# thepochynsons/MCRay-Tracing

Hardware: AMD Instinct MI355X
Metric: rays/sec (Monte-Carlo sample paths traced + accumulated into whole B-mode frames: PSF, envelope, scan conversion) (higher is better)
Workload: dtype f32; 1 GPU; 1M random triangles (8 meshes, PCG64 12345): 128x1024 rays/GPU, depth 10, 465 rows; scan_lines_total=128, triangles=1000000, parallelism=scanline-shard x1, frames_in_flight=128, last_pass_gather_and_post_exposed=False, gather=none (one GPU), slowest_repeat=0, overlap_gather_psf_with_next_trace=True, bvh_builder=sah, warmup_steps_run=3978

## Files before the change

mcray-tracing_amd/api.py:

```python
import contextlib
import ctypes as C
import math
import numpy as np

from . import _lib
from ._lib import Params, MeshRec, Stats, Bvh, Bvh4, BmodeParams, Focus, Compound, Sweep, VolumeGrid, CompoundOpts, LabelOpts, RenderView, RenderOpts, SpeckleOpts, ReconOpts, NODE_DTYPE, SEGMENT_DTYPE, check, ptr, load_library

DEFAULT_ANGLE = 1.0471975511965976


def host_build_bvh(tri, tri_mesh):
    L = load_library()
    tri = np.ascontiguousarray(tri, np.float32).reshape(-1, 9)
    tm = np.ascontiguousarray(tri_mesh, np.uint32)
    b = Bvh()
    check(L.mcrt_build_bvh(ptr(tri), ptr(tm), tri.shape[0], C.byref(b)))
    try:
        nodes = np.frombuffer(C.string_at(b.nodes, 64 * b.n_nodes), dtype=NODE_DTYPE).copy()
        btri = np.frombuffer(C.string_at(b.tri, 48 * b.n_tri), dtype=np.float32).reshape(-1, 12).copy()
        depth = int(b.max_depth)
    finally:
        L.mcrt_free_bvh(C.byref(b))
    return nodes, btri, depth


def host_build_bvh4(tri, tri_mesh):
    L = load_library()
    tri = np.ascontiguousarray(tri, np.float32).reshape(-1, 9)
    tm = np.ascontiguousarray(tri_mesh, np.uint32)
    b = Bvh(); b4 = Bvh4()
    check(L.mcrt_build_bvh(ptr(tri), ptr(tm), tri.shape[0], C.byref(b)))
    try:
        check(L.mcrt_build_bvh4(C.byref(b), C.byref(b4)))
        nodes = np.frombuffer(C.string_at(b.nodes, 64 * b.n_nodes), dtype=NODE_DTYPE).copy()
        btri = np.frombuffer(C.string_at(b.tri, 48 * b.n_tri), dtype=np.float32).reshape(-1, 12).copy()
        n4 = np.frombuffer(C.string_at(b4.nodes, 128 * b4.n_nodes), dtype=np.uint8).reshape(-1, 128).copy()
        ms = int(b4.max_stack)
    finally:
        L.mcrt_free_bvh(C.byref(b)); L.mcrt_free_bvh4(C.byref(b4))
    return nodes, btri, n4, ms


def host_row_thresholds(row_dt_us, n_rows):
    thr = np.zeros(n_rows + 1, np.float64)
    check(load_library().mcrt_row_thresholds(row_dt_us, n_rows, ptr(thr)))
    return thr


def host_texture(n=256):
    out = np.empty((n, n, n, 2), np.float32)
    check(load_library().mcrt_generate_texture(ptr(out), n))
    return out


def host_psf(freq=4.5, var_x=0.05, var_y=0.2, res_um=145, n_ax=7, n_lat=13):
    ax = np.zeros(n_ax, np.float32); lat = np.zeros(n_lat, np.float32)
    check(load_library().mcrt_psf_kernels(freq, var_x, var_y, res_um, ptr(ax), n_ax, ptr(lat), n_lat))
    return ax, lat


def focus_struct(focus_mm=(), focal_range_mm=20.0):
    f = Focus()
    fm = [float(x) for x in (focus_mm or ())]
    f.n_focus = len(fm)
    for i, x in enumerate(fm[:8]):
        f.focus_mm[i] = x
    f.focal_range_mm = focal_range_mm
    return f


def host_psf_focus(var_y, res_um, n_rows, row_mm, focus_mm, focal_range_mm=20.0, n_lat=13):
    out = np.zeros((n_rows, n_lat), np.float32)
    f = focus_struct(focus_mm, focal_range_mm)
    check(load_library().mcrt_psf_focus_kernels(var_y, res_um, C.byref(f), n_rows, row_mm, ptr(out), n_lat))
    return out


def row_pitch_mm(frequency):
    res_f = np.float32(np.float32(1.45) / np.float32(frequency))
    return int(np.float32(res_f * np.float32(1000.0))) / 1000.0


def _element_tables(fn, n_elements, radius_cm, sep_mm, position, angles_deg, *how):
    pos = np.zeros((n_elements, 3), np.float32); d = np.zeros((n_elements, 3), np.float32)
    p = np.asarray(position, np.float32); a = np.asarray(angles_deg, np.float32)
    check(getattr(load_library(), fn)(n_elements, radius_cm, sep_mm, ptr(p), ptr(a), *how, ptr(pos), ptr(d)))
    return pos, d


def host_transducer(n_elements, radius_cm, sep_mm, position, angles_deg):
    return _element_tables("mcrt_transducer_elements", n_elements, radius_cm, sep_mm, position, angles_deg)


def host_elevation_axis(angles_deg):
    a = np.asarray(angles_deg, np.float32); out = np.zeros(3, np.float32)
    check(load_library().mcrt_transducer_elevation_axis(ptr(a), ptr(out)))
    return out


def host_elevation_planes(pos, dirs, axis, n_planes, pitch_um):
    pos = np.ascontiguousarray(pos, np.float32).reshape(-1, 3); dirs = np.ascontiguousarray(dirs, np.float32).reshape(-1, 3)
    axis = np.ascontiguousarray(axis, np.float32)
    E, K = pos.shape[0], max(int(n_planes), 0)
    po = np.zeros((K, E, 3), np.float32); do = np.zeros((K, E, 3), np.float32); z = np.zeros(K, np.float32)
    check(load_library().mcrt_elevation_planes(ptr(pos), ptr(dirs), E, ptr(axis), n_planes, pitch_um, ptr(po), ptr(do), ptr(z)))
    return po, do, z


def host_psf_elevation(var_z, pitch_um, n_rows, row_mm, focus_mm=(), focal_range_mm=20.0, n_planes=7, normalize=True):
    out = np.zeros((n_rows, max(int(n_planes), 0)), np.float32)
    f = focus_struct(focus_mm, focal_range_mm)
    check(load_library().mcrt_psf_elevation_kernels(var_z, pitch_um, C.byref(f), n_rows, row_mm, 1 if normalize else 0, ptr(out), n_planes))
    return out


def host_scan_maps(n_elements, n_rows, radius_mm=30.0, total_angle=DEFAULT_ANGLE, max_travel_us=100, speed_of_sound=1500, out_rows=400, out_cols=500):
    return _sector_maps("mcrt_scan_maps", n_elements, n_rows, radius_mm, total_angle, max_travel_us, speed_of_sound, out_rows, out_cols)


def _sector_maps(fn, n_elements, n_rows, radius_mm, total_angle, max_travel_us, speed_of_sound, out_rows, out_cols, *steer):
    mr = np.zeros((out_rows, out_cols), np.float32); mc = np.zeros((out_rows, out_cols), np.float32)
    check(getattr(load_library(), fn)(n_elements, n_rows, radius_mm, total_angle, max_travel_us, speed_of_sound, out_rows, out_cols, *steer, ptr(mr), ptr(mc)))
    return mr, mc


def host_transducer_steered(n_elements, radius_cm, sep_mm, position, angles_deg, steer_rad):
    return _element_tables("mcrt_transducer_steered", n_elements, radius_cm, sep_mm, position, angles_deg, steer_rad)


def host_compound_maps(n_elements, n_rows, steer_rad, radius_mm=30.0, total_angle=DEFAULT_ANGLE, max_travel_us=100, speed_of_sound=1500, out_rows=400,
                       out_cols=500):
    return _sector_maps("mcrt_compound_maps", n_elements, n_rows, radius_mm, total_angle, max_travel_us, speed_of_sound, out_rows, out_cols, steer_rad)


def compound_struct(steer_rad):
    st = [float(x) for x in steer_rad]
    cp = Compound()
    cp.n_views = len(st)
    for i, x in enumerate(st[:16]):
        cp.steer_rad[i] = x
    return cp


COMPOUND_MODES = {"mean": 0, "max": 1, "median": 2}


def compound_opts_struct(mode="mean", view_weights=None, feather_lines=0.0):
    o = CompoundOpts()
    check(load_library().mcrt_default_compound_opts(C.byref(o)))
    o.mode = COMPOUND_MODES[mode] if isinstance(mode, str) else int(mode)
    o.feather_lines = float(feather_lines)
    if view_weights is not None:
        w = [float(x) for x in view_weights]
        if len(w) > 16:
            raise ValueError("at most 16 view weights, got %d" % len(w))
        for i, x in enumerate(w):
            o.view_weight[i] = x
    return o


def _compound_defaults(mode, view_weights, feather_lines):
    return mode in ("mean", 0) and view_weights is None and feather_lines == 0.0


def host_compound_weights(n_elements, n_rows, steer_rad, view_weight=1.0, feather_lines=0.0, radius_mm=30.0, total_angle=DEFAULT_ANGLE,
                          max_travel_us=100, speed_of_sound=1500, out_rows=400, out_cols=500):
    w = np.zeros((out_rows, out_cols), np.float32)
    check(load_library().mcrt_compound_weights(n_elements, n_rows, radius_mm, total_angle, max_travel_us, speed_of_sound, out_rows, out_cols, steer_rad,
                                               view_weight, feather_lines, ptr(w)))
    return w


def host_transducer_swept(n_elements, radius_cm, sep_mm, position, angles_deg, tilt_rad, pivot_mm=0.0):
    return _element_tables("mcrt_transducer_swept", n_elements, radius_cm, sep_mm, position, angles_deg, tilt_rad, pivot_mm)


def sweep_struct(n_planes, step_rad, pivot_mm=0.0):
    sw = Sweep()
    sw.n_planes, sw.step_rad, sw.pivot_mm = int(n_planes), float(step_rad), float(pivot_mm)
    return sw


def _as_sweep(sweep):
    return sweep if isinstance(sweep, Sweep) else sweep_struct(*sweep)


def sweep_tilts(n_planes, step_rad):
    step = float(np.float32(step_rad))
    return np.array([(k - (n_planes - 1) / 2.0) * step for k in range(n_planes)], np.float32)


def volume_grid(origin_mm, du, dv, dw, nu, nv, nw=1):
    g = VolumeGrid()
    for dst, src in ((g.origin_mm, origin_mm), (g.du_mm, du), (g.dv_mm, dv), (g.dw_mm, dw)):
        for i in range(3):
            dst[i] = float(src[i])
    g.nu, g.nv, g.nw, g._pad = int(nu), int(nv), int(nw), 0
    return g


def cplane_grid(depth_mm, nu, nv, pitch_mm, x0_mm=None, z0_mm=None):
    x0 = -(nu - 1) * pitch_mm / 2.0 if x0_mm is None else x0_mm
    z0 = -(nv - 1) * pitch_mm / 2.0 if z0_mm is None else z0_mm
    return volume_grid((x0, depth_mm, z0), (pitch_mm, 0, 0), (0, 0, pitch_mm), (0, 0, 0), nu, nv, 1)


def sagittal_grid(x_mm, nu, nv, pitch_mm, y0_mm, z0_mm=None):
    z0 = -(nu - 1) * pitch_mm / 2.0 if z0_mm is None else z0_mm
    return volume_grid((x_mm, y0_mm, z0), (0, 0, pitch_mm), (0, pitch_mm, 0), (0, 0, 0), nu, nv, 1)


def host_volume_maps(n_elements, n_rows, sweep, grid, radius_mm=30.0, total_angle=DEFAULT_ANGLE, max_travel_us=100, speed_of_sound=1500):
    sw = _as_sweep(sweep)
    shape = (grid.nw, grid.nv, grid.nu)
    mz = np.zeros(shape, np.float32); mr = np.zeros(shape, np.float32); mc = np.zeros(shape, np.float32)
    check(load_library().mcrt_volume_maps(n_elements, n_rows, radius_mm, total_angle, max_travel_us, speed_of_sound, C.byref(sw), C.byref(grid), ptr(mz), ptr(mr), ptr(mc)))
    return mz, mr, mc


BMODE_MODES = {"db": 0, "ref_log": 1}


RENDER_MODES = {"mip": 0, "mean": 1, "surface": 2}


def render_view(grid, direction, up=(0, 0, 1), pixel_mm=0.25, step_mm=0.25, nx=500, ny=400):
    v = RenderView()
    d = (C.c_double * 3)(*[float(x) for x in direction]); u = (C.c_double * 3)(*[float(x) for x in up])
    check(load_library().mcrt_render_view_for_grid(C.byref(grid), d, u, float(pixel_mm), float(step_mm), int(nx), int(ny), C.byref(v)))
    return v


def render_opts_struct(in_u8=False, mode=None, lo=None, hi=None, threshold=None, ramp=None, opacity=None, depth_cue=None, t_cut=None):
    o = RenderOpts()
    check(load_library().mcrt_default_render_opts(C.byref(o), 1 if in_u8 else 0))
    if mode is not None:
        o.mode = RENDER_MODES[mode] if isinstance(mode, str) else int(mode)
    for name, val in (("lo", lo), ("hi", hi), ("threshold", threshold), ("ramp", ramp), ("opacity", opacity), ("depth_cue", depth_cue), ("t_cut", t_cut)):
        if val is not None:
            setattr(o, name, float(val))
    return o


def speckle_opts_struct(n_iter=None, q0=None, rho=None, lambda_=None, **kw):
    o = SpeckleOpts()
    check(load_library().mcrt_default_speckle_opts(C.byref(o)))
    for k in ("lambda", "lam"):
        if k in kw:
            lambda_ = kw.pop(k)
    if kw:
        raise TypeError("unknown speckle options: %s" % ", ".join(sorted(kw)))
    if n_iter is not None:
        o.n_iter = int(n_iter)
    for name, val in (("q0", q0), ("rho", rho), ("lambda_", lambda_)):
        if val is not None:
            setattr(o, name, float(val))
    return o


def host_speckle_tables(opts=None, **kw):
    o = opts if opts is not None else speckle_opts_struct(**kw)
    n = min(int(o.n_iter), 256)
    q0sq = np.zeros(n, np.float32); kq = np.zeros(n, np.float32); lam4 = np.zeros(1, np.float32)
    check(load_library().mcrt_speckle_tables(C.byref(o), ptr(q0sq), ptr(kq), ptr(lam4)))
    return q0sq, kq, np.float32(lam4[0])


RECON_MODES = {"mean": 0, "max": 1}


def recon_opts_struct(mode=None, value_max=None, fill_radius=None, fill_min=None, empty=None):
    o = ReconOpts()
    check(load_library().mcrt_default_recon_opts(C.byref(o)))
    if mode is not None:
        o.mode = RECON_MODES[mode] if isinstance(mode, str) else int(mode)
    for name, val, kind in (("value_max", value_max, float), ("fill_radius", fill_radius, int), ("fill_min", fill_min, int), ("empty", empty, float)):
        if val is not None:
            setattr(o, name, kind(val))
    return o


def host_recon_transform(grid, unit_mm=10.0):
    A = np.zeros((3, 3), np.float32); b = np.zeros(3, np.float32)
    check(load_library().mcrt_recon_transform(C.byref(grid), float(unit_mm), ptr(A), ptr(b)))
    return A, b


def _depth_mm_f(depth_cm, speed_of_sound):
    travel = int((depth_cm / float(speed_of_sound)) * 10000.0)
    return float(np.float32(np.float32((travel * int(speed_of_sound)) & 0xffffffff) * np.float32(0.001)))


LABEL_RULES = {"traced": 0, "geometric": 1}
LABEL_NONE = 255
LABEL_MAX_CROSSINGS = 64
LABEL_CAPPED = 1 << 31


def label_opts_struct(rule="traced", start_offset=None):
    o = LabelOpts()
    check(load_library().mcrt_default_label_opts(C.byref(o)))
    o.rule = LABEL_RULES[rule] if isinstance(rule, str) else int(rule)
    if start_offset is not None:
        o.start_offset = float(start_offset)
    return o


def bmode_params(mode="db", dynamic_range_db=60.0, gain_db=0.0, ref=None, persistence=0.0, reset_state=True, radius_mm=30.0,
                 total_angle=DEFAULT_ANGLE, out_rows=400, out_cols=500):
    p = BmodeParams()
    check(load_library().mcrt_default_bmode(C.byref(p)))
    p.mode = BMODE_MODES[mode] if isinstance(mode, str) else int(mode)
    p.dynamic_range_db, p.gain_db, p.ref, p.persistence = dynamic_range_db, gain_db, 0.0 if ref is None else ref, persistence
    p.reset_state = 1 if reset_state else 0
    p.out_rows, p.out_cols, p.radius_mm, p.total_angle_rad = out_rows, out_cols, radius_mm, total_angle
    return p


class Transducer:

    def __init__(self, n_elements=512, frequency=4.5, radius_cm=3.0, amplitude_deg=60.0, position=(0, 0, 0), angles_deg=(0, 0, 0), separation_mm=None):
        self.n_elements = n_elements
        self.frequency = frequency
        self.radius_cm = radius_cm
        self.amplitude_rad = (amplitude_deg * math.pi * 1.0) / 180.0
        if separation_mm is None:
            separation_mm = ((float(np.float32(self.amplitude_rad)) * radius_cm) / n_elements) * 10.0
        self.separation_mm = separation_mm
        self.position = tuple(float(x) for x in position)
        self.angles = tuple(float(x) for x in angles_deg)
        self.update()

    def update(self):
        self.pos, self.dir = host_transducer(self.n_elements, self.radius_cm, self.separation_mm, self.position, self.angles)

    def element(self, i):
        return self.pos[i], self.dir[i]

    def planes(self, n_planes, pitch_um):
        return host_elevation_planes(self.pos, self.dir, host_elevation_axis(self.angles), n_planes, pitch_um)

    def steered(self, steer_rad_list):
        tabs = [host_transducer_steered(self.n_elements, self.radius_cm, self.separation_mm, self.position, self.angles, float(s)) for s in steer_rad_list]
        return np.stack([t[0] for t in tabs]), np.stack([t[1] for t in tabs])

    def swept(self, n_planes, step_rad, pivot_mm=0.0):
        tabs = [host_transducer_swept(self.n_elements, self.radius_cm, self.separation_mm, self.position, self.angles, float(t), pivot_mm)
                for t in sweep_tilts(n_planes, step_rad)]
        return np.stack([t[0] for t in tabs]), np.stack([t[1] for t in tabs])

    def poses(self, positions, angles_deg):
        positions = np.asarray(positions, np.float32).reshape(-1, 3); angles_deg = np.asarray(angles_deg, np.float32).reshape(-1, 3)
        if positions.shape != angles_deg.shape:
            raise ValueError("poses takes one position and one set of angles per frame")
        tabs = [host_transducer(self.n_elements, self.radius_cm, self.separation_mm, p, a) for p, a in zip(positions, angles_deg)]
        return np.stack([t[0] for t in tabs]), np.stack([t[1] for t in tabs])


class Psf:

    def __init__(self, freq=4.5, var_x=0.05, var_y=0.2, var_z=0.1, axial_size=7, lateral_size=13, resolution_um=145, focus_mm=None, focal_range_mm=20.0,
                 elevation_size=7, elevation_pitch_um=None, elevation_focus_mm=None, elevation_normalize=True):
        self.axial_kernel, self.lateral_kernel = host_psf(freq, var_x, var_y, resolution_um, axial_size, lateral_size)
        self.var_y, self.resolution_um = var_y, resolution_um
        self.focus_mm = tuple(float(x) for x in focus_mm) if focus_mm is not None else ()
        self.focal_range_mm = focal_range_mm
        self._rows = {}
        self.var_z, self.elevation_size = var_z, elevation_size
        self.elevation_pitch_um = resolution_um if elevation_pitch_um is None else elevation_pitch_um
        self.elevation_focus_mm = tuple(float(x) for x in elevation_focus_mm) if elevation_focus_mm is not None else ()
        self.elevation_normalize = bool(elevation_normalize)
        self.elevation_kernel = (host_psf_elevation(var_z, self.elevation_pitch_um, 1, 1.0, (), focal_range_mm, elevation_size, False)[0]
                                 if var_z > 0 and math.isfinite(var_z) else np.zeros(elevation_size, np.float32))
        self._elev_rows = {}

    def elevation_rows(self, n_rows, row_mm):
        key = (n_rows, row_mm)
        if key not in self._elev_rows:
            self._elev_rows[key] = host_psf_elevation(self.var_z, self.elevation_pitch_um, n_rows, row_mm, self.elevation_focus_mm, self.focal_range_mm,
                                                      self.elevation_size, self.elevation_normalize)
        return self._elev_rows[key]

    @property
    def has_focus(self):
        return len(self.focus_mm) > 0

    def lateral_rows(self, n_rows, row_mm):
        key = (n_rows, row_mm)
        if key not in self._rows:
            self._rows[key] = host_psf_focus(self.var_y, self.resolution_um, n_rows, row_mm, self.focus_mm, self.focal_range_mm, self.lateral_kernel.size)
        return self._rows[key]


def _scene_tables(sd):
    meshes = (MeshRec * len(sd.meshes))(*[MeshRec(a, b, c, 0) for a, b, c in sd.meshes])
    return meshes, len(sd.meshes), np.asarray(sd.spacing, np.float32)


def _tri9(tri):
    if isinstance(tri, np.ndarray):
        tri = np.ascontiguousarray(tri, np.float32).reshape(-1, 9)
        return tri, tri.shape[0]
    return tri, tri.numel() // 9


def _tgc_rows(tgc_db, n_rows):
    if tgc_db is None:
        return None
    tgc = np.ascontiguousarray(tgc_db, np.float32)
    if tgc.shape != (n_rows,):
        raise ValueError("tgc_db needs one value per RF row: %d, got shape %s" % (n_rows, tgc.shape))
    return tgc


def _pose_tables(what, pos, dirs, n_frames, n_elements):
    if isinstance(pos, np.ndarray):
        pos = np.ascontiguousarray(pos, np.float32); dirs = np.ascontiguousarray(dirs, np.float32)
    if n_frames is None:
        if not hasattr(pos, "shape"):
            raise ValueError("%s: n_frames is required with raw device pointers for pos / dirs" % what)
        n_frames = pos.shape[0]
        assert tuple(pos.shape) == (n_frames, n_elements, 3) and tuple(dirs.shape) == tuple(pos.shape)
    return pos, dirs, n_frames


class _SceneCalls:

    def _call(self, name, *args):
        check(getattr(self.L, self.PREFIX + name)(self.h, *args))

    def _assign_params(self, kw):
        for k, v in kw.items():
            if not hasattr(self.params, k):
                raise AttributeError(k)
            setattr(self.params, k, v)

    def set_bvh_builder(self, builder):
        self._call("set_bvh_builder", {"sah": 0, "lbvh": 1}[builder] if isinstance(builder, str) else int(builder))

    def upload_scene(self, sd):
        meshes, n_mesh, sp = _scene_tables(sd)
        self._call("upload_scene", ptr(sd.tri), ptr(sd.tri_mesh), sd.n_tri, C.cast(meshes, C.c_void_p), n_mesh, ptr(sd.materials), sd.materials.shape[0], sd.start_mat, ptr(sp))

    def upload_texture(self, vox=None, n=256):
        if vox is not None:
            vox = np.ascontiguousarray(vox, np.float32)
        self._call("upload_texture", ptr(vox), n)

    def set_transducer(self, pos, d):
        pos = np.ascontiguousarray(pos, np.float32); d = np.ascontiguousarray(d, np.float32)
        self._call("set_transducer", ptr(pos), ptr(d), pos.shape[0])


class Context(_SceneCalls):
    PREFIX = "mcrt_"

    def __init__(self, device=0, _borrowed=None):
        self.L = load_library()
        self.owned = _borrowed is None
        if self.owned:
            h = C.c_void_p()
            check(self.L.mcrt_create(device, C.byref(h)))
        else:
            h = C.c_void_p(_borrowed)
        self.h = h
        self.params = Params()
        check(self.L.mcrt_default_params(C.byref(self.params)))

    def close(self):
        if getattr(self, "h", None):
            if self.owned:
                self.L.mcrt_destroy(self.h)
            self.h = None

    def __del__(self):
        try:
            self.close()
        except Exception:
            pass

    def set_params(self, **kw):
        self._assign_params(kw)
        check(self.L.mcrt_set_params(self.h, C.byref(self.params)))

    def set_stream(self, stream_ptr):
        check(self.L.mcrt_set_stream(self.h, C.c_void_p(stream_ptr) if stream_ptr else None))

    def synchronize(self):
        check(self.L.mcrt_synchronize(self.h))

    def debug_fast_paths(self):
        out = (C.c_uint32 * 4)()
        check(self.L.mcrt_debug_fast_paths(self.h, out))
        return bool(out[0]), bool(out[1]), int(out[2])

    def debug_set_error(self, bits):
        check(self.L.mcrt_debug_set_error(self.h, int(bits)))

    def update_triangles(self, tri):
        tri, n = _tri9(tri)
        check(self.L.mcrt_update_triangles(self.h, ptr(tri), n))

    def refit_triangles(self, tri):
        tri, n = _tri9(tri)
        check(self.L.mcrt_refit_triangles(self.h, ptr(tri), n))

    def get_bvh(self):
        b = Bvh()
        check(self.L.mcrt_get_bvh(self.h, C.byref(b)))
        nodes = np.frombuffer(C.string_at(b.nodes, 64 * b.n_nodes), dtype=NODE_DTYPE).copy() if b.n_nodes else np.zeros(0, NODE_DTYPE)
        btri = np.frombuffer(C.string_at(b.tri, 48 * b.n_tri), dtype=np.float32).reshape(-1, 12).copy()
        return nodes, btri, int(b.max_depth)

    def get_bvh4(self):
        b = Bvh4()
        check(self.L.mcrt_get_bvh4(self.h, C.byref(b)))
        return np.frombuffer(C.string_at(b.nodes, 128 * b.n_nodes), dtype=np.uint8).reshape(-1, 128).copy(), int(b.max_stack)

    def alloc(self, nbytes):
        p = C.c_void_p()
        check(self.L.mcrt_alloc(self.h, nbytes, C.byref(p)))
        return p.value

    def free(self, dev):
        check(self.L.mcrt_free(self.h, C.c_void_p(dev)))

    @contextlib.contextmanager
    def temp(self, nbytes):
        p = self.alloc(nbytes)
        try:
            yield p
        finally:
            self.free(p)

    def d2h(self, dev, shape, dtype=np.float32):
        out = np.empty(shape, dtype)
        check(self.L.mcrt_memcpy_d2h(self.h, ptr(out), ptr(dev), out.nbytes))
        return out

    def h2d(self, dev, arr):
        arr = np.ascontiguousarray(arr)
        check(self.L.mcrt_memcpy_h2d(self.h, ptr(dev), ptr(arr), arr.nbytes))

    def trace_frame(self, frame_id, rf_dev, e_begin=0, e_end=None):
        e_end = self.params.n_elements if e_end is None else e_end
        check(self.L.mcrt_trace_frame(self.h, frame_id, e_begin, e_end, ptr(rf_dev)))

    def trace_frames(self, frame_id, n_frames, rf_dev, e_begin=0, e_end=None):
        e_end = self.params.n_elements if e_end is None else e_end
        check(self.L.mcrt_trace_frames(self.h, frame_id, n_frames, e_begin, e_end, ptr(rf_dev)))

    def trace_frames_poses(self, frame_id, pos, dirs, rf_dev, e_begin=0, e_end=None, n_frames=None):
        e_end = self.params.n_elements if e_end is None else e_end
        pos, dirs, n_frames = _pose_tables("trace_frames_poses", pos, dirs, n_frames, self.params.n_elements)
        check(self.L.mcrt_trace_frames_poses(self.h, frame_id, n_frames, e_begin, e_end, ptr(pos), ptr(dirs), ptr(rf_dev)))

    def trace_frame_debug(self, frame_id, rf_dev, e_begin=0, e_end=None, want_hits=True, want_segs=False):
        e_end = self.params.n_elements if e_end is None else e_end
        ne, S, B = e_end - e_begin, self.params.n_samples, self.params.max_depth
        hits = np.full((ne, S, B), -3, np.int32) if want_hits else None
        segs = np.zeros((ne, S, B), SEGMENT_DTYPE) if want_segs else None
        cnt = np.zeros((ne, S), np.uint32) if want_segs else None
        check(self.L.mcrt_trace_frame_debug(self.h, frame_id, e_begin, e_end, ptr(rf_dev), ptr(hits), ptr(segs), ptr(cnt)))
        return hits, segs, cnt

    def cast_rays(self, frame_id, e_begin=0, e_end=None, want_hits=True):
        e_end = self.params.n_elements if e_end is None else e_end
        ne, S, B = e_end - e_begin, self.params.n_samples, self.params.max_depth
        segs = np.zeros((ne, S, B), SEGMENT_DTYPE); cnt = np.zeros((ne, S), np.uint32)
        hits = np.full((ne, S, B), -3, np.int32) if want_hits else None
        check(self.L.mcrt_cast_rays(self.h, frame_id, e_begin, e_end, ptr(segs), ptr(cnt), ptr(hits)))
        return segs, cnt, hits

    def convolve_frames(self, rf_dev, n_frames, n_elements, n_rows, axial, lateral):
        ax = np.ascontiguousarray(axial, np.float32); lat = np.ascontiguousarray(lateral, np.float32)
        check(self.L.mcrt_convolve_frames(self.h, ptr(rf_dev), n_frames, n_elements, n_rows, ptr(ax), ax.size, ptr(lat), lat.size))

    def convolve_frames_depth(self, rf_dev, n_frames, n_elements, n_rows, axial, lat_rows):
        ax = np.ascontiguousarray(axial, np.float32); lat = np.ascontiguousarray(lat_rows, np.float32)
        if lat.ndim != 2 or lat.shape[0] != n_rows:
            raise ValueError("lat_rows needs one row of taps per RF row: (%d, n_lat), got shape %s" % (n_rows, lat.shape))
        check(self.L.mcrt_convolve_frames_depth(self.h, ptr(rf_dev), n_frames, n_elements, n_rows, ptr(ax), ax.size, ptr(lat), lat.shape[1]))

    def elevation_frames(self, planes_dev, n_frames, n_planes, n_elements, n_rows, w_rows, rf_dev):
        w = np.ascontiguousarray(w_rows, np.float32)
        if w.shape != (n_rows, n_planes):
            raise ValueError("w_rows needs one row of weights per RF row: (%d, %d), got shape %s" % (n_rows, n_planes, w.shape))
        check(self.L.mcrt_elevation_frames(self.h, ptr(planes_dev), n_frames, n_planes, n_elements, n_rows, ptr(w), ptr(rf_dev)))

    def convolve(self, rf_dev, n_elements, n_rows, axial, lateral):
        ax =np.ascontiguousarray(axial, np.float32); lat = np.ascontiguousarray(lateral, np.float32)
        check(self.L.mcrt_convolve(self.h, ptr(rf_dev), n_elements, n_rows, ptr(ax), ax.size, ptr(lat), lat.size))

    def envelope(self, rf_dev, n_elements, n_rows):
        check(self.L.mcrt_envelope(self.h, ptr(rf_dev), n_elements, n_rows))

    def envelope_frames(self, rf_dev, n_frames, n_elements, n_rows):
        check(self.L.mcrt_envelope_frames(self.h, ptr(rf_dev), n_frames, n_elements, n_rows))

    def scan_convert_frames(self, rf_dev, n_frames, n_elements, n_rows, out_dev, radius_mm=30.0, total_angle=DEFAULT_ANGLE, out_rows=400, out_cols=500):
        check(self.L.mcrt_scan_convert_frames(self.h, ptr(rf_dev), n_frames, n_elements, n_rows, radius_mm, total_angle, ptr(out_dev), out_rows, out_cols))

    def scan_convert(self, rf_dev, n_elements, n_rows, out_dev, radius_mm=30.0, total_angle=DEFAULT_ANGLE, out_rows=400, out_cols=500):
        check(self.L.mcrt_scan_convert(self.h, ptr(rf_dev), n_elements, n_rows, radius_mm, total_angle, ptr(out_dev), out_rows, out_cols))

    def bmode_frames(self, rf_dev, n_frames, n_elements, n_rows, out_dev, *, mode="db", dynamic_range_db=60.0, gain_db=0.0, ref=None, tgc_db=None,
                     persistence=0.0, state_dev=None, reset_state=True, peak_dev=None, radius_mm=30.0, total_angle=DEFAULT_ANGLE,
                     out_rows=400, out_cols=500):
        p = bmode_params(mode=mode, dynamic_range_db=dynamic_range_db, gain_db=gain_db, ref=ref, persistence=persistence, reset_state=reset_state,
                         radius_mm=radius_mm, total_angle=total_angle, out_rows=out_rows, out_cols=out_cols)
        tgc = _tgc_rows(tgc_db, n_rows)
        check(self.L.mcrt_bmode_frames(self.h, ptr(rf_dev), n_frames, n_elements, n_rows, C.byref(p), ptr(tgc), ptr(state_dev), ptr(peak_dev), ptr(out_dev)))

    def compound_frames(self, rf_dev, n_frames, n_elements, n_rows, steer_rad, out_dev, radius_mm=30.0, total_angle=DEFAULT_ANGLE, out_rows=400, out_cols=500,
                        mode="mean", view_weights=None, feather_lines=0.0):
        cp = compound_struct(steer_rad)
        if _compound_defaults(mode, view_weights, feather_lines):
            check(self.L.mcrt_compound_frames(self.h, ptr(rf_dev), n_frames, n_elements, n_rows, radius_mm, total_angle, C.byref(cp), ptr(out_dev), out_rows, out_cols))
            return
        o = compound_opts_struct(mode, view_weights, feather_lines)
        check(self.L.mcrt_compound_frames_opts(self.h, ptr(rf_dev), n_frames, n_elements, n_rows, radius_mm, total_angle, C.byref(cp), ptr(out_dev), out_rows, out_cols,
                                               C.byref(o)))

    def bmode_compound_frames(self, rf_dev, n_frames, n_elements, n_rows, steer_rad, out_dev, *, mode="db", dynamic_range_db=60.0, gain_db=0.0, ref=None,
                              tgc_db=None, persistence=0.0, state_dev=None, reset_state=True, peak_dev=None, radius_mm=30.0,
                              total_angle=DEFAULT_ANGLE, out_rows=400, out_cols=500, compound_mode="mean", view_weights=None, feather_lines=0.0):
        p = bmode_params(mode=mode, dynamic_range_db=dynamic_range_db, gain_db=gain_db, ref=ref, persistence=persistence, reset_state=reset_state,
                         radius_mm=radius_mm, total_angle=total_angle, out_rows=out_rows, out_cols=out_cols)
        cp = compound_struct(steer_rad)
        tgc = _tgc_rows(tgc_db, n_rows)
        if _compound_defaults(compound_mode, view_weights, feather_lines):
            check(self.L.mcrt_bmode_compound_frames(self.h, ptr(rf_dev), n_frames, n_elements, n_rows, C.byref(p), C.byref(cp), ptr(tgc), ptr(state_dev),
                                                    ptr(peak_dev), ptr(out_dev)))
            return
        o = compound_opts_struct(compound_mode, view_weights, feather_lines)
        check(self.L.mcrt_bmode_compound_frames_opts(self.h, ptr(rf_dev), n_frames, n_elements, n_rows, C.byref(p), C.byref(cp), ptr(tgc), ptr(state_dev),
                                                     ptr(peak_dev), ptr(out_dev), C.byref(o)))

    def volume_frames(self, rf_dev, n_frames, n_elements, n_rows, sweep, grid, out_dev, radius_mm=30.0, total_angle=DEFAULT_ANGLE):
        sw = _as_sweep(sweep)
        check(self.L.mcrt_volume_frames(self.h, ptr(rf_dev), n_frames, n_elements, n_rows, radius_mm, total_angle, C.byref(sw), C.byref(grid), ptr(out_dev)))

    def bmode_volume_frames(self, rf_dev, n_frames, n_elements, n_rows, sweep, grid, out_dev, *, mode="db", dynamic_range_db=60.0, gain_db=0.0, ref=None,
                            tgc_db=None, persistence=0.0, peak_dev=None, radius_mm=30.0, total_angle=DEFAULT_ANGLE):
        p = bmode_params(mode=mode, dynamic_range_db=dynamic_range_db, gain_db=gain_db, ref=ref, persistence=persistence, radius_mm=radius_mm,
                         total_angle=total_angle, out_rows=0, out_cols=0)
        sw = _as_sweep(sweep)
        tgc = _tgc_rows(tgc_db, n_rows)
        check(self.L.mcrt_bmode_volume_frames(self.h, ptr(rf_dev), n_frames, n_elements, n_rows, C.byref(p), C.byref(sw), C.byref(grid), ptr(tgc), ptr(peak_dev),
                                              ptr(out_dev)))

    def render_frames(self, vol_dev, n_frames, shape, view, out_dev=None, out8_dev=None, depth_dev=None, in_u8=False, **opts):
        nw, nv, nu = shape
        o = render_opts_struct(in_u8, **opts)
        check(self.L.mcrt_render_frames(self.h, ptr(vol_dev), 1 if in_u8 else 0, n_frames, nu, nv, nw, C.byref(view), C.byref(o), ptr(out_dev), ptr(out8_dev),
                                        ptr(depth_dev)))

    def speckle_frames(self, in_dev, n_frames, height, width, out_dev=None, **opts):
        o = speckle_opts_struct(**opts)
        check(self.L.mcrt_speckle_frames(self.h, ptr(in_dev), n_frames, height, width, C.byref(o), ptr(in_dev if out_dev is None else out_dev)))

    def recon_frames(self, stack_dev, pos, dirs, n_frames, n_elements, n_rows, grid, out_dev, count_dev=None, stats_dev=None, row_mm=None, unit_mm=10.0,
                     **opts):
        o = recon_opts_struct(**opts)
        if row_mm is None:
            row_mm = _depth_mm_f(self.params.depth_cm, self.params.speed_of_sound) / n_rows
        pos, dirs, n_frames = _pose_tables("recon_frames", pos, dirs, n_frames, n_elements)
        check(self.L.mcrt_recon_frames(self.h, ptr(stack_dev), n_frames, n_elements, n_rows, ptr(pos), ptr(dirs), float(row_mm), float(unit_mm), C.byref(grid),
                                       C.byref(o), ptr(out_dev), ptr(count_dev), ptr(stats_dev)))

    def label_frames(self, pos=None, dirs=None, *, rule="traced", start_offset=None, e_begin=0, e_end=None, n_frames=None, tissue_dev=None,
                     interface_dev=None, crossings_dev=None):
        e_end = self.params.n_elements if e_end is None else e_end
        if pos is None:
            n_frames = 1 if n_frames is None else n_frames
        else:
            pos, dirs, n_frames = _pose_tables("label_frames", pos, dirs, n_frames, self.params.n_elements)
        o = label_opts_struct(rule, start_offset)
        check(self.L.mcrt_label_frames(self.h, n_frames, e_begin, e_end, ptr(pos), ptr(dirs), C.byref(o), ptr(tissue_dev), ptr(interface_dev), ptr(crossings_dev)))

    def label_scan_convert_frames(self, tissue_dev, n_frames, n_elements, n_rows, out_dev, radius_mm=30.0, total_angle=DEFAULT_ANGLE, out_rows=400, out_cols=500):
        check(self.L.mcrt_label_scan_convert_frames(self.h, ptr(tissue_dev), n_frames, n_elements, n_rows, radius_mm, total_angle, ptr(out_dev), out_rows, out_cols))

    def label_volume_frames(self, tissue_dev, n_frames, n_elements, n_rows, sweep, grid, out_dev, radius_mm=30.0, total_angle=DEFAULT_ANGLE):
        sw = _as_sweep(sweep)
        check(self.L.mcrt_label_volume_frames(self.h, ptr(tissue_dev), n_frames, n_elements, n_rows, radius_mm, total_angle, C.byref(sw), C.byref(grid), ptr(out_dev)))

    def export_rf(self, rf_dev, n_elements, n_rows):
        out = np.empty((n_rows, n_elements), np.float32)
        check(self.L.mcrt_export_rf(self.h, ptr(rf_dev), n_elements, n_rows, ptr(out)))
        return out

    def enable_stats(self, on=True):
        check(self.L.mcrt_enable_stats(self.h, int(on)))

    def get_stats(self, reset=True):
        s = Stats()
        check(self.L.mcrt_get_stats(self.h, C.byref(s), int(reset)))
        return s.as_dict()

    def enable_timing(self, on=True):
        check(self.L.mcrt_enable_timing(self.h, int(on)))

    def kernel_times(self, reset=True):
        ms = (C.c_double * 3)(); n = (C.c_uint32 * 3)()
        check(self.L.mcrt_get_kernel_times(self.h, ms, n, int(reset)))
        return {k: (ms[i], n[i]) for i, k in enumerate(("walk", "shade", "march"))}

    def kernel_time(self, reset=True):
        ms = C.c_double(); n = C.c_uint32()
        check(self.L.mcrt_get_kernel_time(self.h, C.byref(ms), C.byref(n), int(reset)))
        return ms.value, n.value

    def debug_math(self, op, x, y=None):
        x = np.ascontiguousarray(x, np.float64); out = np.empty_like(x)
        if y is not None:
            y = np.ascontiguousarray(y, np.float64)
        check(self.L.mcrt_debug_math(self.h, op, ptr(x), ptr(y), ptr(out), x.size))
        return out

    def debug_philox(self, ctr, key):
        c = np.asarray(ctr, np.uint32); k = np.asarray(key, np.uint32); o = np.zeros(4, np.uint32)
        check(self.L.mcrt_debug_philox(self.h, ptr(c), ptr(k), ptr(o)))
        return o


def shard_range(rank, n_ranks, n_elements):
    b = C.c_uint32(); e = C.c_uint32()
    check(load_library().mcrt_group_shard(rank, n_ranks, n_elements, C.byref(b), C.byref(e)))
    return int(b.value), int(e.value)


class Group(_SceneCalls):
    PREFIX = "mcrt_group_"

    def __init__(self, devices):
        self.L = load_library()
        devs = (C.c_int * len(devices))(*devices)
        h = C.c_void_p()
        check(self.L.mcrt_group_create(C.cast(devs, C.c_void_p), len(devices), C.byref(h)))
        self.h = h
        self.size = int(self.L.mcrt_group_size(self.h))
        self.root = Context(_borrowed=self.L.mcrt_group_root(self.h))
        self.members = [Context(_borrowed=self.L.mcrt_group_member(self.h, r)) for r in range(self.size)]
        self.params = Params()
        check(self.L.mcrt_default_params(C.byref(self.params)))

    def close(self):
        if getattr(self, "h", None):
            self.L.mcrt_group_destroy(self.h)
            self.h = None
            self.root.h = None
            for m in self.members:
                m.h = None

    def __del__(self):
        try:
            self.close()
        except Exception:
            pass

    def set_params(self, **kw):
        self._assign_params(kw)
        try:
            check(self.L.mcrt_group_set_params(self.h, C.byref(self.params)))
        finally:
            for c in [self.root] + self.members:
                check(self.L.mcrt_get_params(c.h, C.byref(c.params)))
            check(self.L.mcrt_get_params(self.root.h, C.byref(self.params)))

    def update_triangles(self, tri):
        tri = np.ascontiguousarray(tri, np.float32).reshape(-1, 9)
        check(self.L.mcrt_group_update_triangles(self.h, ptr(tri), tri.shape[0]))

    def refit_triangles(self, tri):
        tri = np.ascontiguousarray(tri, np.float32).reshape(-1, 9)
        check(self.L.mcrt_group_refit_triangles(self.h, ptr(tri), tri.shape[0]))

    def trace_frames(self, frame_id, n_frames, rf_dev):
        check(self.L.mcrt_group_trace_frames(self.h, frame_id, n_frames, ptr(rf_dev)))

    def trace_frames_poses(self, frame_id, pos, dirs, rf_dev):
        pos = np.ascontiguousarray(pos, np.float32); dirs = np.ascontiguousarray(dirs, np.float32)
        assert tuple(pos.shape) == (pos.shape[0], self.params.n_elements, 3) and tuple(dirs.shape) == tuple(pos.shape)
        check(self.L.mcrt_group_trace_frames_poses(self.h, frame_id, pos.shape[0], ptr(pos), ptr(dirs), ptr(rf_dev)))

    def synchronize(self):
        check(self.L.mcrt_group_synchronize(self.h))

    def last_scene_seconds(self):
        b, u = C.c_double(), C.c_double()
        check(self.L.mcrt_group_last_scene_seconds(self.h, C.byref(b), C.byref(u)))
        return b.value, u.value

    def last_pass_ms(self):
        t = np.zeros(self.size, np.float32); c = np.zeros(self.size, np.float32)
        check(self.L.mcrt_group_last_pass_ms(self.h, ptr(t), ptr(c)))
        return t, c


class Simulator:

    def __init__(self, scene_data, transducer, n_samples=5, n_rows=None, device=0, seed=0x5EED, psf=None, texture=None,
                 max_depth=10, sanitize_tir=0, tex_n=256, bvh_builder="sah", elevation=False, compound=None, compound_mode="mean", compound_weights=None,
                 compound_feather=0.0, sweep=None, sweep_pivot_mm=0.0, speckle=None):
        if sweep is not None and (compound is not None or elevation):
            raise ValueError("sweep= does not combine with compound= or elevation=")
        if compound is not None and not 1 <= len(tuple(compound)) <= 16:
            raise ValueError("compound takes 1..16 steering angles, got %d" % len(tuple(compound)))
        self.speckle = None if speckle is None or speckle is False else speckle_opts_struct(**({} if speckle is True else dict(speckle)))
        self.ctx = Context(device)
        self.ctx.set_bvh_builder(bvh_builder)
        self.tr = transducer
        E = transducer.n_elements
        self.ctx.set_params(n_elements=E, n_samples=n_samples, frequency=transducer.frequency, seed=seed, max_depth=max_depth,
                            sanitize_tir=sanitize_tir, tex_n=tex_n, **({"n_rows": n_rows} if n_rows else {}))
        self.E, self.R, self.S = E, self.ctx.params.n_rows, n_samples
        self.ctx.upload_scene(scene_data)
        self.ctx.upload_texture(texture, tex_n)
        self.ctx.set_transducer(transducer.pos, transducer.dir)
        self.psf = psf or Psf(freq=transducer.frequency)
        self.rf_dev = self.ctx.alloc(E * self.R * 4)
        self.elevation, self.planes_dev, self.views_dev, self.sweep, self.sweep_dev = bool(elevation), None, None, None, None
        self.steers = tuple(float(x) for x in compound) if compound is not None else None
        self.N = len(self.steers) if self.steers is not None else 1
        if compound_weights is not None and (self.steers is None or len(tuple(compound_weights)) != len(self.steers)):
            raise ValueError("compound_weights takes one weight per steering angle of compound=")
        if self.steers is None and not _compound_defaults(compound_mode, None, compound_feather):
            raise ValueError("compound_mode and compound_feather need compound=")
        self.compound_opts = dict(mode=compound_mode, view_weights=tuple(float(x) for x in compound_weights) if compound_weights is not None else None,
                                  feather_lines=float(compound_feather))
        self._stack, self._pass = (self.rf_dev, 1), None
        if self.steers is not None:
            self.view_pos, self.view_dir = transducer.steered(self.steers)
            self.views_dev = self.ctx.alloc(self.N * E * self.R * 4)
            self._stack, self._pass = (self.views_dev, self.N), (self.view_pos, self.view_dir, self.views_dev, self.N)
        if sweep is not None:
            self.sweep = sweep_struct(sweep[0], sweep[1], sweep_pivot_mm)
            self.sweep_pos, self.sweep_dir = transducer.swept(self.sweep.n_planes, self.sweep.step_rad, self.sweep.pivot_mm)
            self.sweep_dev = self.ctx.alloc(self.sweep.n_planes * E * self.R * 4)
            self._stack, self._pass = (self.sweep_dev, self.sweep.n_planes), (self.sweep_pos, self.sweep_dir, self.sweep_dev, self.sweep.n_planes)
        if self.elevation:
            self.K = self.psf.elevation_size
            self.plane_pos, self.plane_dir, self.plane_z_mm = transducer.planes(self.K, self.psf.elevation_pitch_um)
            if self.steers is not None:
                axis = host_elevation_axis(transducer.angles)
                tabs = [host_elevation_planes(self.view_pos[n], self.view_dir[n], axis, self.K, self.psf.elevation_pitch_um) for n in range(self.N)]
                self.plane_pos = np.concatenate([t[0] for t in tabs]); self.plane_dir = np.concatenate([t[1] for t in tabs])
            self.planes_dev = self.ctx.alloc(self.N * self.K * E * self.R * 4)
            self._pass = (self.plane_pos, self.plane_dir, self.planes_dev, self.N * self.K)

    def close(self):
        if self.ctx.h:
            for d in (self.rf_dev, self.planes_dev, self.views_dev, self.sweep_dev):
                if d:
                    self.ctx.free(d)
            self.ctx.close()

    def trace(self, frame_id=0):
        if self._pass is None:
            self.ctx.trace_frame(frame_id, self.rf_dev)
            return
        pos, dirs, dest, per_frame = self._pass
        self.ctx.trace_frames_poses(frame_id * per_frame, pos, dirs, dest)
        if self.elevation:
            self.ctx.elevation_frames(self.planes_dev, self._stack[1], self.K, self.E, self.R, self.psf.elevation_rows(self.R, self.row_mm), self._stack[0])

    @property
    def row_mm(self):
        return row_pitch_mm(self.ctx.params.frequency)

    def convolve(self):
        if self.psf.has_focus:
            self.ctx.convolve_frames_depth(*self._stack, self.E, self.R, self.psf.axial_kernel, self.psf.lateral_rows(self.R, self.row_mm))
        else:
            self.ctx.convolve_frames(*self._stack, self.E, self.R, self.psf.axial_kernel, self.psf.lateral_kernel)

    def envelope(self):
        self.ctx.envelope_frames(*self._stack, self.E, self.R)

    def despeckle(self):
        o = self.speckle if self.speckle is not None else speckle_opts_struct()
        self.ctx.speckle_frames(*self._stack, self.E, self.R, n_iter=o.n_iter, q0=o.q0, rho=o.rho, lambda_=o.lambda_)

    def _run(self, frame_id, convolve=True, envelope=True):
        self.trace(frame_id)
        if convolve:
            self.convolve()
        if envelope:
            self.envelope()
            if self.speckle is not None:
                self.despeckle()

    def compound_image(self, frame_id=0, convolve=True, envelope=True, radius_mm=30.0, total_angle=DEFAULT_ANGLE, out_rows=400, out_cols=500):
        if self.steers is None:
            raise RuntimeError("compound_image() needs Simulator(compound=...)")
        self._run(frame_id, convolve, envelope)
        with self.ctx.temp(out_rows * out_cols * 4) as out:
            self.ctx.compound_frames(self.views_dev, 1, self.E, self.R, self.steers, out, radius_mm=radius_mm, total_angle=total_angle, out_rows=out_rows,
                                     out_cols=out_cols, **self.compound_opts)
            return self.ctx.d2h(out, (out_rows, out_cols), np.float32)

    def volume(self, frame_id, grid, convolve=True, envelope=True, radius_mm=30.0, total_angle=DEFAULT_ANGLE):
        if self.sweep is None:
            raise RuntimeError("volume() needs Simulator(sweep=...)")
        self._run(frame_id, convolve, envelope)
        shape = (grid.nw, grid.nv, grid.nu)
        with self.ctx.temp(shape[0] * shape[1] * shape[2] * 4) as out:
            self.ctx.volume_frames(self.sweep_dev, 1, self.E, self.R, self.sweep, grid, out, radius_mm=radius_mm, total_angle=total_angle)
            return self.ctx.d2h(out, shape, np.float32)

    def bmode_volume(self, frame_id, grid, **display):
        if self.sweep is None:
            raise RuntimeError("bmode_volume() needs Simulator(sweep=...)")
        self._run(frame_id)
        shape = (grid.nw, grid.nv, grid.nu)
        with self.ctx.temp(shape[0] * shape[1] * shape[2]) as out:
            self.ctx.bmode_volume_frames(self.sweep_dev, 1, self.E, self.R, self.sweep, grid, out, **display)
            return self.ctx.d2h(out, shape, np.uint8)

    def render(self, frame_id, grid, direction, up=(0, 0, 1), size=(500, 400), pixel_mm=0.25, step_mm=0.25, mode="surface", **opts):
        if self.sweep is None:
            raise RuntimeError("render() needs Simulator(sweep=...)")
        ropts = {k: opts.pop(k) for k in ("lo", "hi", "threshold", "ramp", "opacity", "depth_cue", "t_cut") if k in opts}
        if "bmode_mode" in opts:
            opts["mode"] = opts.pop("bmode_mode")
        view = render_view(grid, direction, up, pixel_mm, step_mm, size[0], size[1])
        self._run(frame_id)
        shape = (grid.nw, grid.nv, grid.nu)
        with self.ctx.temp(shape[0] * shape[1] * shape[2]) as vox, self.ctx.temp(size[0] * size[1]) as out:
            self.ctx.bmode_volume_frames(self.sweep_dev, 1, self.E, self.R, self.sweep, grid, vox, **opts)
            self.ctx.render_frames(vox, 1, shape, view, out8_dev=out, in_u8=True, mode=mode, **ropts)
            return self.ctx.d2h(out, (size[1], size[0]), np.uint8)

    def freehand(self, frame_id, pos, dirs, grid, convolve=True, envelope=True, counts=False, row_mm=None, unit_mm=10.0, **opts):
        if self.steers is not None or self.sweep is not None or self.elevation:
            raise RuntimeError("freehand() does not combine with compound=, sweep= or elevation=")
        pos, dirs, F = _pose_tables("freehand", np.asarray(pos), np.asarray(dirs), None, self.E)
        shape = (grid.nw, grid.nv, grid.nu)
        n = shape[0] * shape[1] * shape[2]
        with self.ctx.temp(F * self.E * self.R * 4) as stack_dev, self.ctx.temp(n * 4) as out, self.ctx.temp(n * 4) as cnt:
            self.ctx.trace_frames_poses(frame_id * F, pos, dirs, stack_dev)
            held, self._stack = self._stack, (stack_dev, F)
            try:
                if convolve:
                    self.convolve()
                if envelope:
                    self.envelope()
                    if self.speckle is not None:
                        self.despeckle()
            finally:
                self._stack = held
            self.ctx.recon_frames(stack_dev, pos, dirs, F, self.E, self.R, grid, out, count_dev=cnt if counts else None, row_mm=row_mm, unit_mm=unit_mm, **opts)
            vox = self.ctx.d2h(out, shape, np.float32)
            return (vox, self.ctx.d2h(cnt, shape, np.uint32)) if counts else vox

    @contextlib.contextmanager
    def _label_pass(self, rule, start_offset, want_rows=True):
        F = self.sweep.n_planes if self.sweep is not None else 1
        n = F * self.E * self.R
        with contextlib.ExitStack() as held:
            sizes = (n, 4 * n, 4 * F * self.E) if want_rows else (n, 0, 0)
            bufs = [held.enter_context(self.ctx.temp(size)) if size else None for size in sizes]
            pos, dirs = (self.sweep_pos, self.sweep_dir) if self.sweep is not None else (None, None)
            self.ctx.label_frames(pos, dirs, rule=rule, start_offset=start_offset, tissue_dev=bufs[0], interface_dev=bufs[1], crossings_dev=bufs[2])
            yield F, bufs

    def labels(self, rule="traced", start_offset=None, picture=True, radius_mm=30.0, total_angle=DEFAULT_ANGLE, out_rows=400, out_cols=500):
        with self._label_pass(rule, start_offset) as (F, bufs):
            lead = (F,) if self.sweep is not None else ()
            out = dict(tissue=self.ctx.d2h(bufs[0], lead + (self.E, self.R), np.uint8), interface=self.ctx.d2h(bufs[1], lead + (self.E, self.R), np.int32),
                       crossings=self.ctx.d2h(bufs[2], lead + (self.E,), np.uint32), picture=None)
            if picture and self.sweep is None:
                with self.ctx.temp(out_rows * out_cols) as pic_dev:
                    self.ctx.label_scan_convert_frames(bufs[0], 1, self.E, self.R, pic_dev, radius_mm=radius_mm, total_angle=total_angle, out_rows=out_rows, out_cols=out_cols)
                    out["picture"] = self.ctx.d2h(pic_dev, (out_rows, out_cols), np.uint8)
            return out

    def label_volume(self, grid, rule="traced", start_offset=None, radius_mm=30.0, total_angle=DEFAULT_ANGLE):
        if self.sweep is None:
            raise RuntimeError("label_volume() needs Simulator(sweep=...)")
        shape = (grid.nw, grid.nv, grid.nu)
        with self._label_pass(rule, start_offset, want_rows=False) as (F, bufs), self.ctx.temp(shape[0] * shape[1] * shape[2]) as out:
            self.ctx.label_volume_frames(bufs[0], 1, self.E, self.R, self.sweep, grid, out, radius_mm=radius_mm, total_angle=total_angle)
            return self.ctx.d2h(out, shape, np.uint8)

    def bmode(self, frame_id=0, **display):
        if self.sweep is not None:
            raise RuntimeError("a swept probe has K planes and meets only at a grid's points: use volume() or bmode_volume()")
        rows, cols = display.get("out_rows", 400), display.get("out_cols", 500)
        self._run(frame_id)
        with self.ctx.temp(rows * cols) as out:
            if self.steers is not None:
                o = self.compound_opts
                self.ctx.bmode_compound_frames(self.views_dev, 1, self.E, self.R, self.steers, out, compound_mode=o["mode"], view_weights=o["view_weights"],
                                               feather_lines=o["feather_lines"], **display)
            else:
                self.ctx.bmode_frames(self.rf_dev, 1, self.E, self.R, out, **display)
            return self.ctx.d2h(out, (rows, cols), np.uint8)

    def frame(self, frame_id=0, convolve=True):
        if self.sweep is not None:
            raise RuntimeError("a swept probe has K planes and meets only at a grid's points: use volume() or bmode_volume()")
        if self.steers is not None:
            raise RuntimeError("frame() returns one RF image; a compounded frame has N views and meets only as a picture: use compound_image() or bmode()")
        self._run(frame_id, convolve, envelope=False)
        return self.ctx.export_rf(self.rf_dev, self.E, self.R)
```

mcray-tracing_amd/csrc/mcrt_api.cpp:

```cpp
#include "mcrt_ctx.h"
#include "mcrt_kernels.h"
#include "mcrt_lbvh.h"

#include <hip/hip_runtime.h>
#include <cmath>
#include <cstdlib>
#include <cstring>
#include <vector>
#include <algorithm>
#include <memory>
#include <utility>

using mcrt::set_error;

static Consts derive_consts(const mcrt_params &p)
{
    Consts c;
    c.axial_res_f = 1.45f / p.frequency;
    c.axial_res_mm = (double)c.axial_res_f;
    c.axial_res_um = (uint32_t)(c.axial_res_f * 1000.0f);
    c.time_step_us = (c.axial_res_mm * 1000.0) / (double)p.speed_of_sound;
    c.row_dt_us = (double)c.axial_res_um / (double)p.speed_of_sound;
    c.max_travel_us = (p.depth_cm / (double)p.speed_of_sound) * 10000.0;
    c.max_rows = (uint32_t)((p.speed_of_sound * (uint32_t)c.max_travel_us) / c.axial_res_um);
    return c;
}

static Knobs read_knobs()
{
    using mcrt::tuning_env;
    Knobs k;
    if (const char *e = tuning_env("MCRT_KSPLIT_LIMIT")) { long v = atol(e); if (v >= 0 && v <= MCRT_KSPLIT_MAX) k.ksplit_limit = (uint32_t)v; }
    if (const char *e = tuning_env("MCRT_TRACE_BLOCKS")) { int v = atoi(e); if (v >= 1) k.trace_blocks = (uint32_t)v; }
    if (const char *e = tuning_env("MCRT_TRACE_BLOCKS_WIDE")) { int v = atoi(e); if (v >= 1) k.trace_blocks_wide = (uint32_t)v; }
    if (const char *e = tuning_env("MCRT_WIDE_MAX_TREE_MB")) { long long v = atoll(e); if (v >= 0 && v <= 0xffffffffll) k.wide_max_tree_mb = (uint32_t)v; }
    if (const char *e = tuning_env("MCRT_WIDE_FROM")) { long long v = atoll(e); if (v >= 1 && v <= 0xffffffffll) k.wide_from = (uint32_t)v; }
    if (const char *e = tuning_env("MCRT_GROUPS")) { int v = atoi(e); if (v >= 1 && v <= 16) k.groups = (uint32_t)v; }
    if (const char *e = tuning_env("MCRT_PACKET_BOUNCES")) { long v = strtol(e, nullptr, 0); if (v >= 0) k.packet_mask = (uint32_t)v; }
    if (const char *e = tuning_env("MCRT_PATH_GROUPS")) { int v = atoi(e); if (v >= 1 && v <= 16) k.path_groups = (uint32_t)v; }
    if (const char *e = tuning_env("MCRT_PATH_MAX")) { long long v = atoll(e); if (v >= 0 && v <= 0xffffffffll) k.path_max = (uint32_t)v; }
    if (const char *e = tuning_env("MCRT_PACKET_FROM")) { long long v = atoll(e); if (v >= 0 && v <= 0xffffffffll) k.packet_from = (uint32_t)v; }
    if (const char *e = tuning_env("MCRT_MARCH_STREAMS")) { int v = atoi(e); if (v >= 1 && v <= MCRT_SIDE_STREAMS) k.march_streams = (uint32_t)v; }
    if (const char *e = tuning_env("MCRT_MARCH_BLOCKS")) { int v = atoi(e); if (v >= 1) k.march_blocks = (uint32_t)v; }
    k.no_overlap = tuning_env("MCRT_NO_OVERLAP") != nullptr; k.no_priority = tuning_env("MCRT_NO_PRIORITY") != nullptr;
    k.no_fast_div = tuning_env("MCRT_NO_FAST_DIV") != nullptr; k.no_lean = tuning_env("MCRT_NO_LEAN") != nullptr;
    k.test_hooks = tuning_env("MCRT_TEST_HOOKS") != nullptr;
    if (const char *e = tuning_env("MCRT_RETIRE_LATE")) k.retire_late = atoi(e) != 0;
    if (const char *e = tuning_env("MCRT_FOLD_B0")) k.fold_b0 = atoi(e) != 0;
    if (const char *e = tuning_env("MCRT_RENDER_ROW_TILE")) k.render_row_tile = atoi(e) != 0;
    if (const char *e = tuning_env("MCRT_SPECKLE_FUSE")) { int v = atoi(e); if (v == 2 || v == 4) k.speckle_fuse = (uint32_t)v; }
    return k;
}

static int prepare_tables(mcrt_ctx *c)
{
    if (c->tab.thr_rows != c->p.n_rows || c->tab.thr_dt != c->c.row_dt_us || !c->tab.d_row_thr) {
        std::vector<double> thr((size_t)c->p.n_rows + 1);
        MCRT_TRY(mcrt_row_thresholds(c->c.row_dt_us, c->p.n_rows, thr.data()));
        HIP_TRY(hipStreamSynchronize(c->stream));
        c->tab.thr_rows = 0;
        HIP_TRY(c->tab.d_row_thr.alloc(thr.size()));
        HIP_TRY(hipMemcpy(c->tab.d_row_thr, thr.data(), thr.size() * 8, hipMemcpyHostToDevice));
        c->tab.thr_rows = c->p.n_rows; c->tab.thr_dt = c->c.row_dt_us; c->tab.thr_end = thr.back();
    }
    if (c->tab.verified_res != c->p.tex_res) {
        Buf<unsigned long long> d_bad; unsigned long long bad = 1;
        HIP_TRY(d_bad.alloc(1));
        HIP_TRY(hipMemsetAsync(d_bad, 0, 8, c->stream));
        HIP_TRY(mcrt::launch_verify_div(c->p.tex_res, 1.0f / c->p.tex_res, d_bad, c->stream));
        HIP_TRY(hipStreamSynchronize(c->stream));
        HIP_TRY(hipMemcpy(&bad, d_bad, 8, hipMemcpyDeviceToHost));
        c->tab.fast_div = (bad == 0) && !c->knobs.no_fast_div;
        c->tab.fast_div_all = c->tab.fast_div && c->p.tex_res > 1e-16f && !c->knobs.no_lean;
        c->tab.verified_res = c->p.tex_res;
    }
    if (c->scene.have && (!c->tab.mtab_valid || c->tab.mtab_key[0] != c->c.axial_res_f || c->tab.mtab_key[1] != c->p.frequency)) {
        c->tab.mtab_valid = false;
        if (c->tab.d_mtab.cap < c->scene.n_mat) {
            HIP_TRY(hipStreamSynchronize(c->stream));
            HIP_TRY(c->tab.d_mtab.alloc(c->scene.n_mat));
        }
        HIP_TRY(mcrt::launch_material_table(c->scene.d_mats, c->scene.n_mat, c->c.axial_res_f, c->p.frequency, c->tab.d_mtab, c->stream));
        c->tab.mtab_key[0] = c->c.axial_res_f; c->tab.mtab_key[1] = c->p.frequency; c->tab.mtab_valid = true;
    }
    return MCRT_OK;
}

extern "C" int mcrt_version(void) { return MCRT_VERSION; }
extern "C" int mcrt_device_count(void)
{
    int n = 0;
    if (hipGetDeviceCount(&n) != hipSuccess) return 0;
    return n;
}

extern "C" int mcrt_default_params(mcrt_params *p)
{
    if (!p) return set_error(MCRT_ERR_INVALID, "null params");
    memset(p, 0, sizeof *p);
    p->n_elements = 512; p->n_samples = 5; p->max_depth = 10; p->n_rows = 465;
    p->frequency = 4.5f; p->intensity_epsilon = 1e-10f; p->initial_intensity = 1.0f; p->ray_start_offset = 0.1f;
    p->speed_of_sound = 1500; p->depth_cm = 15.0; p->seed = 0x5EED; p->sanitize_tir = 0; p->tex_n = 256; p->tex_res = 0.145f;
    return MCRT_OK;
}

extern "C" int mcrt_create(int device, mcrt_ctx **out)
{
    if (!out) return set_error(MCRT_ERR_INVALID, "null out pointer");
    *out = nullptr;
    int n = 0;
    if (hipGetDeviceCount(&n) != hipSuccess || n <= 0)
        return set_error(MCRT_ERR_NO_DEVICE, "no HIP device visible: libmcrt_hip has no CPU fallback");
    if (device < 0 || device >= n) return set_error(MCRT_ERR_INVALID, "device %d out of range (0..%d)", device, n - 1);
    HIP_TRY(hipSetDevice(device));
    hipDeviceProp_t prop;
    HIP_TRY(hipGetDeviceProperties(&prop, device));
    if (!strstr(prop.gcnArchName, "gfx950"))
        return set_error(MCRT_ERR_NO_DEVICE, "device %d is %s; this library carries gfx950 (MI355X) code only", device, prop.gcnArchName);
    std::unique_ptr<mcrt_ctx> c(new (std::nothrow) mcrt_ctx());
    if (!c) return set_error(MCRT_ERR_NOMEM, "out of host memory");
    c->device = device;
    c->knobs = read_knobs();
    if (prop.multiProcessorCount > 0) c->n_cu = (uint32_t)prop.multiProcessorCount;
    HIP_TRY(hipStreamCreateWithFlags(&c->own_stream.h, hipStreamNonBlocking));
    c->stream = c->own_stream;
    HIP_TRY(ensure_event(c->ev_start));
    c->work.reserve(16);
    mcrt_default_params(&c->p);
    c->c = derive_consts(c->p);
    HIP_TRY(c->ins.d_stats.alloc(MCRT_STATS_WORDS));
    HIP_TRY(hipMemsetAsync(c->ins.d_stats, 0, MCRT_STATS_WORDS * sizeof(unsigned long long), c->stream));
    HIP_TRY(c->d_error.alloc(1));
    HIP_TRY(hipMemsetAsync(c->d_error, 0, 4, c->stream));
    HIP_TRY(hipStreamSynchronize(c->stream));
    MCRT_TRY(prepare_tables(c.get()));
    *out = c.release();
    return MCRT_OK;
}

static int refresh_soa(mcrt_ctx *c)
{
    c->scene.walked_stale = true;
    if (c->scene.bvh4.n_nodes == 0) { c->scene.d_nodes_walk.reset(); return MCRT_OK; }
    if (c->scene.d_nodes_walk.cap != 4 * (size_t)c->scene.bvh4.n_nodes) {
        HIP_TRY(hipStreamSynchronize(c->stream));
        HIP_TRY(c->scene.d_nodes_walk.alloc(4 * (size_t)c->scene.bvh4.n_nodes));
    }
    HIP_TRY(mcrt::launch_nodes_walk(c->scene.d_nodes, c->scene.bvh4.n_nodes, c->scene.d_nodes_walk, c->stream));
    if (c->scene.d_tris_id.cap != MCRT_TRI_PIECES * (size_t)c->scene.bvh.n_tri) {
        HIP_TRY(hipStreamSynchronize(c->stream));
        HIP_TRY(c->scene.d_tris_id.alloc(MCRT_TRI_PIECES * (size_t)c->scene.bvh.n_tri));
    }
    HIP_TRY(mcrt::launch_tris_by_id((const float4 *)c->scene.d_tris, c->scene.bvh.n_tri, c->scene.d_tris_id, c->stream));
    HIP_TRY(ensure_event(c->scene.ev_update));
    HIP_TRY(hipEventRecord(c->scene.ev_update, c->stream));
    c->scene.update_stream = c->stream; c->scene.update_pending = true;
    return MCRT_OK;
}

extern "C" int mcrt_destroy(mcrt_ctx *c)
{
    if (!c) return MCRT_OK;
    hipSetDevice(c->device);
    hipDeviceSynchronize();
    delete c;
    return MCRT_OK;
}

namespace mcrt { hipStream_t ctx_stream(mcrt_ctx *c) { return c->stream; } }
extern "C" int mcrt_set_stream(mcrt_ctx *c, void *s) { CTX_TRY(c); c->stream = s ? (hipStream_t)s : c->own_stream; return MCRT_OK; }
int mcrt::check_device_error(mcrt_ctx *c)
{
    uint32_t e = 0;
    HIP_TRY(hipMemcpy(&e, c->d_error, 4, hipMemcpyDeviceToHost));
    if (e) { HIP_TRY(hipMemsetAsync(c->d_error, 0, 4, c->stream)); HIP_TRY(hipStreamSynchronize(c->stream)); return set_error(MCRT_ERR_LIMIT, "device error flag 0x%x:%s%s", e, (e & 1u) ? " BVH traversal stack overflow" : "", (e & 2u) ? " kernel watchdog expired (a persistent kernel ran for more than its time limit and was abandoned)" : ""); }
    return MCRT_OK;
}
extern "C" int mcrt_synchronize(mcrt_ctx *c) { CTX_TRY(c); HIP_TRY(hipStreamSynchronize(c->stream)); return mcrt::check_device_error(c); }

extern "C" int mcrt_set_params(mcrt_ctx *c, const mcrt_params *p)
{
    CTX_TRY(c);
    if (!p) return set_error(MCRT_ERR_INVALID, "null params");
    if (p->n_elements == 0 || p->n_samples == 0) return set_error(MCRT_ERR_INVALID, "n_elements and n_samples must be positive");
    if (p->max_depth == 0 || p->max_depth > MCRT_MAX_BOUNCES) return set_error(MCRT_ERR_LIMIT, "max_depth must be 1..%d", MCRT_MAX_BOUNCES);
    if (p->n_rows == 0 || p->n_rows > MCRT_MAX_ROWS) return set_error(MCRT_ERR_LIMIT, "n_rows must be 1..%d", MCRT_MAX_ROWS);
    if (!(p->frequency > 0.f) || p->speed_of_sound == 0 || !(p->depth_cm > 0.0)) return set_error(MCRT_ERR_INVALID, "frequency, speed_of_sound and depth must be positive");
    if (p->tex_n == 0 || !(p->tex_res > 0.f)) return set_error(MCRT_ERR_INVALID, "texture size/resolution must be positive");
    Consts k = derive_consts(*p);
    if (k.axial_res_um == 0) return set_error(MCRT_ERR_INVALID, "axial resolution rounds to 0 um at %g MHz", (double)p->frequency);
    c->p = *p; c->c = k;
    return prepare_tables(c);
}

extern "C" int mcrt_get_params(mcrt_ctx *c, mcrt_params *out)
{
    if (!c || !out) return set_error(MCRT_ERR_INVALID, "null argument");
    *out = c->p;
    return MCRT_OK;
}

static int copy_tree(const mcrt::HostTree &src, mcrt_bvh *bvh, mcrt_bvh4 *bvh4)
{
    *bvh = *src.bvh; *bvh4 = *src.bvh4;
    bvh->nodes = nullptr; bvh->tri = nullptr; bvh4->nodes = nullptr;
    const size_t nb = sizeof(mcrt_bvh_node) * (size_t)src.bvh->n_nodes, tb = 48 * (size_t)src.bvh->n_tri, n4 = sizeof(mcrt_bvh4_node) * (size_t)src.bvh4->n_nodes;
    bvh->nodes = (mcrt_bvh_node *)malloc(nb ? nb : 1); bvh->tri = (float *)malloc(tb ? tb : 1); bvh4->nodes = (mcrt_bvh4_node *)malloc(n4 ? n4 : 1);
    if (!bvh->nodes || !bvh->tri || !bvh4->nodes) { mcrt_free_bvh(bvh); mcrt_free_bvh4(bvh4); return set_error(MCRT_ERR_NOMEM, "out of host memory"); }
    memcpy(bvh->nodes, src.bvh->nodes, nb); memcpy(bvh->tri, src.bvh->tri, tb); memcpy(bvh4->nodes, src.bvh4->nodes, n4);
    return MCRT_OK;
}

static int index_triangles(mcrt_ctx *c, const float *tri, uint32_t n_tri, const mcrt::HostTree *pre = nullptr)
{
    if (n_tri >= (1u << 25)) return set_error(MCRT_ERR_LIMIT, "%u triangles: the walk addresses at most 2^25 (32-bit byte offsets into 64-byte nodes and records)", n_tri);
    c->scene.d_nodes.reset(); c->scene.d_tris.reset(); c->scene.d_tri_slot.reset();
    mcrt_free_bvh(&c->scene.bvh); mcrt_free_bvh4(&c->scene.bvh4);
    c->scene.host_bvh_stale = false;
    const bool on_device = c->scene.builder == MCRT_BVH_DEVICE_LBVH;
    Buf<float4> leaf;
    if (on_device) {
        mcrt::LbvhResult r;
        {
            Buf<float> d_tri; Buf<uint32_t> d_mesh;
            HIP_TRY(d_tri.alloc(9 * (size_t)n_tri));
            HIP_TRY(d_mesh.alloc(n_tri));
            if (hipMemcpyAsync(d_tri, tri, 36 * (size_t)n_tri, hipMemcpyDefault, c->stream) != hipSuccess ||
                hipMemcpyAsync(d_mesh, c->scene.tri_mesh.data(), 4 * (size_t)n_tri, hipMemcpyHostToDevice, c->stream) != hipSuccess)
                return set_error(MCRT_ERR_HIP, "triangle upload failed");
            MCRT_TRY(mcrt::lbvh_build(d_tri, d_mesh, n_tri, c->stream, &r));
        }
        c->scene.d_nodes = std::move(r.nodes); c->scene.d_tri_slot = std::move(r.tri_slot); leaf = std::move(r.tris);
        c->scene.bvh.n_nodes = 0; c->scene.bvh.n_tri = n_tri; c->scene.bvh.max_depth = r.max_depth; c->scene.bvh.pad_abs = r.pad_abs; c->scene.bvh.nodes = nullptr; c->scene.bvh.tri = nullptr;
        c->scene.bvh4.n_nodes = r.n_nodes4; c->scene.bvh4.max_stack = r.max_stack; c->scene.bvh4.nodes = nullptr;
        c->scene.host_bvh_stale = true;
        for (int i = 0; i < 3; i++) { c->scene.lo[i] = r.lo[i]; c->scene.hi[i] = r.hi[i]; }
    } else if (pre) {
        if (pre->bvh->n_tri != n_tri) return set_error(MCRT_ERR_INVALID, "prebuilt tree has %u triangles, the scene %u", pre->bvh->n_tri, n_tri);
        MCRT_TRY(copy_tree(*pre, &c->scene.bvh, &c->scene.bvh4));
    } else {
        std::vector<float> host_copy;
        if (is_device_pointer(tri)) {
            host_copy.resize((size_t)n_tri * 9);
            HIP_TRY(hipMemcpy(host_copy.data(), tri, 36 * (size_t)n_tri, hipMemcpyDeviceToHost));
            tri = host_copy.data();
        }
        MCRT_TRY(mcrt_build_bvh(tri, c->scene.tri_mesh.data(), n_tri, &c->scene.bvh));
        MCRT_TRY(mcrt_build_bvh4(&c->scene.bvh, &c->scene.bvh4));
    }
    if (c->scene.bvh4.max_stack > MCRT_STACK)
        return set_error(MCRT_ERR_LIMIT, "%sBVH4 needs a %u-entry traversal stack, the kernel has %d", on_device ? "device-built " : "", c->scene.bvh4.max_stack, MCRT_STACK);
    if (c->scene.bvh4.n_nodes >= (1u << 25)) return set_error(MCRT_ERR_LIMIT, "%u BVH4 nodes: the walk addresses at most 2^25", c->scene.bvh4.n_nodes);
    if (!on_device) {
        for (int i = 0; i < 3; i++) { c->scene.lo[i] = INFINITY; c->scene.hi[i] = -INFINITY; }
        for (int k = 0; k < 4; k++) {
            const mcrt_bvh4_child &ch = c->scene.bvh4.nodes[0].c[k];
            if (ch.ref == MCRT_BVH4_EMPTY) continue;
            const float hi[3] = { ch.hi_x, ch.hi_y, ch.hi_z };
            for (int i = 0; i < 3; i++) { c->scene.lo[i] = std::min(c->scene.lo[i], ch.lo[i]); c->scene.hi[i] = std::max(c->scene.hi[i], hi[i]); }
        }
        HIP_TRY(c->scene.d_nodes.alloc(sizeof(mcrt_bvh4_node) / 16 * (size_t)c->scene.bvh4.n_nodes));
        HIP_TRY(hipMemcpy(c->scene.d_nodes, c->scene.bvh4.nodes, sizeof(mcrt_bvh4_node) * (size_t)c->scene.bvh4.n_nodes, hipMemcpyHostToDevice));
        HIP_TRY(leaf.alloc(3 * (size_t)n_tri));
        HIP_TRY(hipMemcpy(leaf, c->scene.bvh.tri, 48 * (size_t)n_tri, hipMemcpyHostToDevice));
        std::vector<uint32_t> slot(n_tri);
        for (uint32_t k = 0; k < n_tri; k++) { uint32_t id; memcpy(&id, &c->scene.bvh.tri[(size_t)k * 12 + 3], 4); slot[id] = k; }
        HIP_TRY(c->scene.d_tri_slot.alloc(n_tri));
        HIP_TRY(hipMemcpy(c->scene.d_tri_slot, slot.data(), 4 * (size_t)n_tri, hipMemcpyHostToDevice));
    }
    HIP_TRY(c->scene.d_tris.alloc(MCRT_TRI_PIECES * (size_t)n_tri));
    HIP_TRY(mcrt::launch_expand_tris(leaf, n_tri, c->scene.d_tris, c->stream));
    HIP_TRY(hipStreamSynchronize(c->stream));
    return MCRT_OK;
}

static int download_bvh(mcrt_ctx *c)
{
    if (!c->scene.host_bvh_stale) return MCRT_OK;
    HIP_TRY(hipStreamSynchronize(c->stream));
    c->scene.bvh.tri = (float *)malloc(48 * (size_t)c->scene.bvh.n_tri);
    c->scene.bvh4.nodes = (mcrt_bvh4_node *)malloc(sizeof(mcrt_bvh4_node) * (size_t)c->scene.bvh4.n_nodes);
    if (!c->scene.bvh.tri || !c->scene.bvh4.nodes) return set_error(MCRT_ERR_NOMEM, "out of memory");
    {
        const size_t W = 4 * MCRT_TRI_PIECES;
        std::vector<float> rec((size_t)c->scene.bvh.n_tri * W);
        HIP_TRY(hipMemcpy(rec.data(), c->scene.d_tris, 4 * W * (size_t)c->scene.bvh.n_tri, hipMemcpyDeviceToHost));
        for (size_t t = 0; t < c->scene.bvh.n_tri; t++) {
            const float *r = &rec[t * W]; float *o = &c->scene.bvh.tri[t * 12];
            memcpy(o, r, 32);
            o[8] = r[8]; o[9] = r[9]; o[10] = r[10]; o[11] = 0.0f;
        }
    }
    HIP_TRY(hipMemcpy(c->scene.bvh4.nodes, c->scene.d_nodes, sizeof(mcrt_bvh4_node) * (size_t)c->scene.bvh4.n_nodes, hipMemcpyDeviceToHost));
    c->scene.host_bvh_stale = false;
    return MCRT_OK;
}

extern "C" int mcrt_set_bvh_builder(mcrt_ctx *c, int builder)
{
    CTX_TRY(c);
    if (builder != MCRT_BVH_HOST_SAH && builder != MCRT_BVH_DEVICE_LBVH) return set_error(MCRT_ERR_INVALID, "unknown BVH builder %d", builder);
    c->scene.builder = builder;
    return MCRT_OK;
}

static int check_new_positions(mcrt_ctx *c, const float *tri, uint32_t n_tri)
{
    CTX_TRY(c);
    if (!c->scene.have) return set_error(MCRT_ERR_INVALID, "no scene uploaded");
    if (!tri) return set_error(MCRT_ERR_INVALID, "null triangles");
    if (n_tri != c->scene.bvh.n_tri || n_tri == 0) return set_error(MCRT_ERR_INVALID, "the scene has %u triangles, the update has %u", c->scene.bvh.n_tri, n_tri);
    HIP_TRY(hipStreamSynchronize(c->stream));
    return MCRT_OK;
}

static int update_triangles(mcrt_ctx *c, const float *tri, uint32_t n_tri, const mcrt::HostTree *pre)
{
    MCRT_TRY(check_new_positions(c, tri, n_tri));
    c->scene.have = false;
    MCRT_TRY(index_triangles(c, tri, n_tri, pre));
    MCRT_TRY(refresh_soa(c));
    c->scene.have = true;
    return MCRT_OK;
}
extern "C" int mcrt_update_triangles(mcrt_ctx *c, const float *tri, uint32_t n_tri) { return update_triangles(c, tri, n_tri, nullptr); }

extern "C" int mcrt_refit_triangles(mcrt_ctx *c, const float *tri, uint32_t n_tri)
{
    MCRT_TRY(check_new_positions(c, tri, n_tri));
    Buf<float> d_tri;
    HIP_TRY(d_tri.alloc(9 * (size_t)n_tri));
    int rc = MCRT_OK;
    if (hipMemcpyAsync(d_tri, tri, 36 * (size_t)n_tri, hipMemcpyDefault, c->stream) != hipSuccess) rc = set_error(MCRT_ERR_HIP, "triangle upload failed");
    float pad = 0.0f, lo[3], hi[3];
    if (!rc) rc = mcrt::bvh_refit(d_tri, n_tri, c->scene.d_nodes, c->scene.bvh4.n_nodes, c->scene.d_tris, c->stream, &pad, lo, hi);
    d_tri.reset();
    if (!rc) rc = refresh_soa(c);
    if (rc) { c->scene.have = false; return rc; }
    c->scene.bvh.pad_abs = pad;
    for (int i = 0; i < 3; i++) { c->scene.lo[i] = lo[i]; c->scene.hi[i] = hi[i]; }
    free(c->scene.bvh.nodes); c->scene.bvh.nodes = nullptr; c->scene.bvh.n_nodes = 0;
    free(c->scene.bvh.tri); c->scene.bvh.tri = nullptr;
    free(c->scene.bvh4.nodes); c->scene.bvh4.nodes = nullptr;
    c->scene.host_bvh_stale = true;
    return MCRT_OK;
}

static int upload_scene(mcrt_ctx *c, const float *tri, const uint32_t *tri_mesh, uint32_t n_tri,
                        const mcrt_mesh *meshes, uint32_t n_mesh, const float *mats, uint32_t n_mat,
                        uint32_t start_mat, const float spacing[3], const mcrt::HostTree *pre)
{
    CTX_TRY(c);
    if (!meshes || !mats || n_mesh == 0 || n_mat == 0 || !spacing) return set_error(MCRT_ERR_INVALID, "mcrt_upload_scene: missing tables");
    if (n_tri && (!tri || !tri_mesh)) return set_error(MCRT_ERR_INVALID, "mcrt_upload_scene: missing triangles");
    if (start_mat >= n_mat) return set_error(MCRT_ERR_INVALID, "startingMaterial index %u out of range", start_mat);
    for (uint32_t i = 0; i < n_mesh; i++)
        if (meshes[i].mat_inside >= n_mat || meshes[i].mat_outside >= n_mat) return set_error(MCRT_ERR_INVALID, "mesh %u references a material out of range", i);
    for (uint32_t i = 0; i < n_tri; i++)
        if (tri_mesh[i] >= n_mesh) return set_error(MCRT_ERR_INVALID, "triangle %u references mesh %u out of range", i, tri_mesh[i]);
    HIP_TRY(hipStreamSynchronize(c->stream));
    free(c->scene.walked_nodes); c->scene.walked_nodes = nullptr; c->scene.walked_stale = true;
    mcrt_free_bvh(&c->scene.bvh); mcrt_free_bvh4(&c->scene.bvh4);
    c->scene.have = false;
    if (n_tri) {
        c->scene.tri_mesh.assign(tri_mesh, tri_mesh + n_tri);
        MCRT_TRY(index_triangles(c, tri, n_tri, pre));
        MCRT_TRY(refresh_soa(c));
    } else {
        c->scene.d_nodes.reset(); c->scene.d_tris.reset(); c->scene.d_tri_slot.reset(); c->scene.d_nodes_walk.reset(); c->scene.d_tris_id.reset();
    }
    HIP_TRY(c->scene.d_mats.alloc(2 * (size_t)n_mat));
    HIP_TRY(hipMemcpy(c->scene.d_mats, mats, 32 * (size_t)n_mat, hipMemcpyHostToDevice));
    HIP_TRY(c->scene.d_meshes.alloc(n_mesh));
    HIP_TRY(hipMemcpy(c->scene.d_meshes, meshes, sizeof(mcrt_mesh) * (size_t)n_mesh, hipMemcpyHostToDevice));
    c->scene.n_mesh = n_mesh; c->scene.n_mat = n_mat; c->scene.start_mat = start_mat;
    c->scene.start_silent = mats[8 * (size_t)start_mat + 2] == 0.0f && mats[8 * (size_t)start_mat + 4] == 0.0f;
    for (int i = 0; i < 3; i++) c->scene.spacing[i] = spacing[i];
    c->scene.have = true; c->tab.mtab_valid = false;
    return prepare_tables(c);
}
extern "C" int mcrt_upload_scene(mcrt_ctx *c, const float *tri, const uint32_t *tri_mesh, uint32_t n_tri,
                                 const mcrt_mesh *meshes, uint32_t n_mesh, const float *mats, uint32_t n_mat,
                                 uint32_t start_mat, const float spacing[3])
{
    return upload_scene(c, tri, tri_mesh, n_tri, meshes, n_mesh, mats, n_mat, start_mat, spacing, nullptr);
}
namespace mcrt {
int ctx_bvh_builder(const mcrt_ctx *c) { return c ? c->scene.builder : MCRT_BVH_HOST_SAH; }
int upload_scene_with_tree(mcrt_ctx *c, const float *tri, const uint32_t *tri_mesh, uint32_t n_tri, const mcrt_mesh *meshes, uint32_t n_mesh,
                           const float *mats, uint32_t n_mat, uint32_t start_mat, const float spacing[3], const HostTree *pre)
{
    return upload_scene(c, tri, tri_mesh, n_tri, meshes, n_mesh, mats, n_mat, start_mat, spacing, pre);
}
int update_triangles_with_tree(mcrt_ctx *c, const float *tri, uint32_t n_tri, const HostTree *pre) { return update_triangles(c, tri, n_tri, pre); }
}

extern "C" int mcrt_get_bvh(mcrt_ctx *c, mcrt_bvh *out)
{
    if (!c || !out) return set_error(MCRT_ERR_INVALID, "null argument");
    if (!c->scene.have) return set_error(MCRT_ERR_INVALID, "no scene uploaded");
    MCRT_TRY(download_bvh(c));
    *out = c->scene.bvh;
    return MCRT_OK;
}

extern "C" int mcrt_get_bvh4(mcrt_ctx *c, mcrt_bvh4 *out)
{
    if (!c || !out) return set_error(MCRT_ERR_INVALID, "null argument");
    if (!c->scene.have) return set_error(MCRT_ERR_INVALID, "no scene uploaded");
    HIP_TRY(hipSetDevice(c->device));
    if (c->scene.d_nodes_walk) {
        if (c->scene.walked_stale || !c->scene.walked_nodes) {
            const size_t bytes = sizeof(mcrt_bvh4_node) * (size_t)c->scene.bvh4.n_nodes;
            Buf<float4> d_tmp;
            HIP_TRY(d_tmp.alloc(bytes / 16));
            hipError_t e = mcrt::launch_nodes_walk_decode(c->scene.d_nodes_walk, c->scene.bvh4.n_nodes, d_tmp, c->stream);
            if (e == hipSuccess) e = hipStreamSynchronize(c->stream);
            free(c->scene.walked_nodes);
            c->scene.walked_nodes = (mcrt_bvh4_node *)malloc(bytes);
            if (e == hipSuccess && c->scene.walked_nodes) e = hipMemcpy(c->scene.walked_nodes, d_tmp, bytes, hipMemcpyDeviceToHost);
            d_tmp.reset();
            if (!c->scene.walked_nodes) return set_error(MCRT_ERR_NOMEM, "out of memory");
            if (e != hipSuccess) return set_error(MCRT_ERR_HIP, "mcrt_get_bvh4: %s", hipGetErrorString(e));
            c->scene.walked_stale = false;
        }
        out->n_nodes = c->scene.bvh4.n_nodes; out->max_stack = c->scene.bvh4.max_stack; out->nodes = c->scene.walked_nodes;
        return MCRT_OK;
    }
    MCRT_TRY(download_bvh(c));
    *out = c->scene.bvh4;
    return MCRT_OK;
}

extern "C" int mcrt_upload_texture(mcrt_ctx *c, const float *vox, uint32_t n)
{
    CTX_TRY(c);
    if (n == 0) return set_error(MCRT_ERR_INVALID, "texture size 0");
    const size_t total = (size_t)n * n * n;
    std::vector<float> gen;
    bool finite = true;
    if (!vox) {
        gen.resize(total * 2);
        MCRT_TRY(mcrt_generate_texture(gen.data(), n));
        vox = gen.data();
    } else {
        for (size_t i = 0; i < total * 2; i++) if (!std::isfinite(vox[i])) { finite = false; break; }
    }
    HIP_TRY(hipStreamSynchronize(c->stream));
    c->tex_n = 0;
    HIP_TRY(c->d_tex.alloc(total));
    HIP_TRY(hipMemcpy(c->d_tex, vox, total * 8, hipMemcpyHostToDevice));
    c->tex_n = n; c->tex_finite = finite;
    return MCRT_OK;
}

extern "C" int mcrt_set_transducer(mcrt_ctx *c, const float *pos, const float *dir, uint32_t n)
{
    CTX_TRY(c);
    if (!pos || !dir || n == 0) return set_error(MCRT_ERR_INVALID, "mcrt_set_transducer: bad arguments");
    if (n != c->n_el) {
        HIP_TRY(hipStreamSynchronize(c->stream));
        c->n_el = 0;
        HIP_TRY(c->d_pos.alloc(3 * (size_t)n));
        HIP_TRY(c->d_dir.alloc(3 * (size_t)n));
        c->n_el = n;
    }
    HIP_TRY(hipMemcpyAsync(c->d_pos, pos, 12 * (size_t)n, hipMemcpyHostToDevice, c->stream));
    HIP_TRY(hipMemcpyAsync(c->d_dir, dir, 12 * (size_t)n, hipMemcpyHostToDevice, c->stream));
    HIP_TRY(hipStreamSynchronize(c->stream));
    return MCRT_OK;
}

extern "C" int mcrt_alloc(mcrt_ctx *c, size_t bytes, void **dev)
{
    CTX_TRY(c);
    if (!dev) return set_error(MCRT_ERR_INVALID, "null out pointer");
    HIP_TRY(hipMalloc(dev, bytes ? bytes : 1));
    return MCRT_OK;
}
extern "C" int mcrt_free(mcrt_ctx *c, void *dev) { CTX_TRY(c); HIP_TRY(hipStreamSynchronize(c->stream)); HIP_TRY(hipFree(dev)); return MCRT_OK; }
extern "C" int mcrt_memcpy_d2h(mcrt_ctx *c, void *host, const void *dev, size_t bytes)
{
    CTX_TRY(c);
    HIP_TRY(hipMemcpyAsync(host, dev, bytes, hipMemcpyDeviceToHost, c->stream));
    HIP_TRY(hipStreamSynchronize(c->stream));
    return MCRT_OK;
}
extern "C" int mcrt_memcpy_h2d(mcrt_ctx *c, void *dev, const void *host, size_t bytes)
{
    CTX_TRY(c);
    HIP_TRY(hipMemcpyAsync(dev, host, bytes, hipMemcpyHostToDevice, c->stream));
    HIP_TRY(hipStreamSynchronize(c->stream));
    return MCRT_OK;
}

extern "C" int mcrt_enable_stats(mcrt_ctx *c, int on) { CTX_TRY(c); c->ins.stats_on = on != 0; return MCRT_OK; }
static int read_stats(mcrt_ctx *c, size_t first, size_t n, void *out, int reset)
{
    CTX_TRY(c);
    HIP_TRY(hipStreamSynchronize(c->stream));
    HIP_TRY(hipMemcpy(out, c->ins.d_stats + first, n * 8, hipMemcpyDeviceToHost));
    if (reset) { HIP_TRY(hipMemsetAsync(c->ins.d_stats + first, 0, n * 8, c->stream)); HIP_TRY(hipStreamSynchronize(c->stream)); }
    return MCRT_OK;
}
extern "C" int mcrt_get_stats(mcrt_ctx *c, mcrt_stats *out, int reset)
{
    unsigned long long v[6];
    MCRT_TRY(read_stats(c, 0, 6, v, reset));
    if (out) { out->queries = v[0]; out->nodes_visited = v[1]; out->tris_tested = v[2]; out->segments = v[3]; out->rf_steps = v[4]; out->hits = v[5]; }
    return MCRT_OK;
}

extern "C" int mcrt_debug_stamps(mcrt_ctx *c, uint64_t out[200], int reset) { return read_stats(c, 8, 200, out, reset); }

extern "C" int mcrt_debug_tail_histograms(mcrt_ctx *c, uint64_t out[2560], int reset)
{
    CTX_TRY(c);
    if (!out) return set_error(MCRT_ERR_INVALID, "null out pointer");
    return read_stats(c, 256, 2560, out, reset);
}

extern "C" int mcrt_debug_fast_paths(mcrt_ctx *c, uint32_t out[4])
{
    CTX_TRY(c);
    if (!out) return set_error(MCRT_ERR_INVALID, "null out pointer");
    out[0] = c->tab.fast_div ? 1u : 0u; out[1] = c->ins.last_lean_bound > 0.0f ? 1u : 0u; out[2] = c->ins.last_march_rows; out[3] = 0u;
    return MCRT_OK;
}

extern "C" int mcrt_debug_set_error(mcrt_ctx *c, uint32_t bits)
{
    CTX_TRY(c);
    if (!c->knobs.test_hooks) return set_error(MCRT_ERR_INVALID, "mcrt_debug_set_error is a test hook: create the context with MCRT_TEST_HOOKS set in the environment");
    uint32_t e = 0;
    HIP_TRY(hipStreamSynchronize(c->stream));
    HIP_TRY(hipMemcpy(&e, c->d_error, 4, hipMemcpyDeviceToHost));
    e |= bits;
    HIP_TRY(hipMemcpy(c->d_error, &e, 4, hipMemcpyHostToDevice));
    return MCRT_OK;
}

extern "C" int mcrt_enable_timing(mcrt_ctx *c, int on) { CTX_TRY(c); c->ins.timing_on = on != 0; c->ins.timing_level = on; return MCRT_OK; }
extern "C" int mcrt_get_kernel_times(mcrt_ctx *c, double avg_ms[3], uint32_t n[3], int reset)
{
    CTX_TRY(c);
    double sum[3] = { 0, 0, 0 }; uint32_t cnt[3] = { 0, 0, 0 };
    for (size_t i = 0; i < c->ins.ev_used; i++) {
        const TimedLaunch &t = c->ins.ev[i];
        float ms = 0;
        HIP_TRY(hipEventSynchronize(t.end));
        HIP_TRY(hipEventElapsedTime(&ms, t.start, t.end));
        sum[t.kind] += ms; cnt[t.kind]++;
    }
    for (int k = 0; k < 3; k++) { if (avg_ms) avg_ms[k] = cnt[k] ? sum[k] / (double)cnt[k] : 0.0; if (n) n[k] = cnt[k]; }
    if (reset) c->ins.ev_used = 0;
    return MCRT_OK;
}
extern "C" int mcrt_get_kernel_time(mcrt_ctx *c, double *avg_ms, uint32_t *n, int reset)
{
    double a[3]; uint32_t k[3];
    MCRT_TRY(mcrt_get_kernel_times(c, a, k, reset));
    if (avg_ms) *avg_ms = a[0];
    if (n) *n = k[0];
    return MCRT_OK;
}

extern "C" int mcrt_debug_math(mcrt_ctx *c, int op, const double *x, const double *y, double *out, uint32_t n)
{
    CTX_TRY(c);
    if (!x || !out || n == 0) return set_error(MCRT_ERR_INVALID, "mcrt_debug_math: bad arguments");
    Buf<double> dx, dy, dout;
    HIP_TRY(dx.alloc(n)); HIP_TRY(dout.alloc(n));
    HIP_TRY(hipMemcpy(dx, x, 8 * (size_t)n, hipMemcpyHostToDevice));
    if (y) { HIP_TRY(dy.alloc(n)); HIP_TRY(hipMemcpy(dy, y, 8 * (size_t)n, hipMemcpyHostToDevice)); }
    HIP_TRY(mcrt::launch_math_probe(op, dx, dy, dout, n, c->stream));
    HIP_TRY(hipStreamSynchronize(c->stream));
    HIP_TRY(hipMemcpy(out, dout, 8 * (size_t)n, hipMemcpyDeviceToHost));
    return MCRT_OK;
}

extern "C" int mcrt_debug_philox(mcrt_ctx *c, const uint32_t ctr[4], const uint32_t key[2], uint32_t out[4])
{
    CTX_TRY(c);
    Buf<uint32_t> d;
    HIP_TRY(d.alloc(4));
    HIP_TRY(mcrt::launch_philox_probe(ctr, key, d, c->stream));
    HIP_TRY(hipStreamSynchronize(c->stream));
    HIP_TRY(hipMemcpy(out, d, 16, hipMemcpyDeviceToHost));
    return MCRT_OK;
}
```

mcray-tracing_amd/csrc/mcrt_ctx.h:

```cpp
#pragma once
#include "../../include/mcrt.h"
#include "mcrt_internal.h"
#include "mcrt_hip.h"

#include <cstdlib>
#include <cstring>
#include <vector>

#define CTX_TRY(ctx) do { if (!(ctx)) return mcrt::set_error(MCRT_ERR_INVALID, "null context"); HIP_TRY(hipSetDevice((ctx)->device)); } while (0)

struct Consts {
    float axial_res_f; double axial_res_mm, time_step_us, row_dt_us, max_travel_us; uint32_t axial_res_um, max_rows;
};

struct PathBufs {
    Buf<float4> st0, st1, st2, mrec;
    Buf<unsigned long long> key0, key1;
    Buf<uint32_t> q, counts, seg_count, cursors;
    size_t paths = 0; uint32_t depth = 0;
};
struct Work {
    Stream stream, side[MCRT_SIDE_STREAMS];
    Event ev_bounce[MCRT_MAX_BOUNCES], ev_join[MCRT_SIDE_STREAMS], ev_done;
    Buf<int> stack_ovf;
    Buf<mcrt_segment> segs;
    Buf<int32_t> hits;
    PathBufs b;
};

#define MCRT_SPECKLE_FUSE_DEFAULT 2u
struct Knobs {
    uint32_t ksplit_limit = MCRT_KSPLIT_DEFAULT, trace_blocks = 0, trace_blocks_wide = 0, wide_from = 0 , wide_max_tree_mb = 128, groups = MCRT_GROUPS_DEFAULT, march_streams = MCRT_SIDE_STREAMS_DEFAULT, march_blocks = 0;
    bool no_overlap = false, no_priority = false, no_fast_div = false, no_lean = false;
    uint32_t path_groups = MCRT_PATH_GROUPS_DEFAULT;
    uint32_t path_max = MCRT_PATH_MAX_DEFAULT;
    uint32_t packet_mask = MCRT_PACKET_MASK_DEFAULT, packet_from = MCRT_PACKET_FROM;
    bool retire_late = true;
    bool fold_b0 = false;
    bool render_row_tile = false;
    uint32_t speckle_fuse = MCRT_SPECKLE_FUSE_DEFAULT;
    bool test_hooks = false;
};

struct StagedTable : Staging {
    std::vector<float> on_dev; uint32_t key[2] = { 0, 0 };
    int put(const float *src, uint32_t R, uint32_t n, size_t room, hipStream_t st)
    {
        const size_t len = (size_t)n * R;
        if (key[0] == R && key[1] == n && !memcmp(src, on_dev.data(), 4 * len)) return MCRT_OK;
        float *h = nullptr;
        MCRT_TRY(begin(room, st, &h));
        on_dev.resize(room);
        for (uint32_t r = 0; r < R; r++)
            for (uint32_t k = 0; k < n; k++) h[(size_t)k * R + r] = src[(size_t)r * n + k];
        key[0] = key[1] = 0;
        MCRT_TRY(commit(len, st));
        memcpy(on_dev.data(), src, 4 * len);
        key[0] = R; key[1] = n;
        return MCRT_OK;
    }
};

struct MapCache {
    struct Key {
        std::vector<unsigned char> bytes;
        template <class T> Key &add(const T &v) { return add(&v, sizeof v); }
        Key &add(const void *p, size_t n) { bytes.insert(bytes.end(), (const unsigned char *)p, (const unsigned char *)p + n); return *this; }
    };
    struct Slot { Buf<float> d; std::vector<unsigned char> key; uint64_t used = 0; };
    std::vector<Slot> slot; uint64_t clock = 0;
    explicit MapCache(size_t slots) : slot(slots) {}
    static size_t pad(size_t n) { return (n + 255u) & ~(size_t)255u; }
    template <class Fill> int get(const Key &key, size_t n, hipStream_t st, Fill fill, const float **maps)
    {
        Slot *lru = &slot[0];
        for (Slot &s : slot) {
            if (s.used && s.key == key.bytes) { s.used = ++clock; *maps = s.d; return MCRT_OK; }
            if (s.used < lru->used) lru = &s;
        }
        std::vector<float> m(n, 0.0f);
        MCRT_TRY(fill(m));
        HIP_TRY(hipStreamSynchronize(st));
        lru->used = 0;
        HIP_TRY(lru->d.grow(n));
        HIP_TRY(hipMemcpy(lru->d, m.data(), n * 4, hipMemcpyHostToDevice));
        lru->key = key.bytes; lru->used = ++clock;
        *maps = lru->d;
        return MCRT_OK;
    }
};

struct TimedLaunch { Event start, end; int kind = 0; };

struct Scene {
    bool have = false;
    mcrt_bvh bvh{};
    mcrt_bvh4 bvh4{};
    Buf<float4> d_nodes, d_tris, d_mats;
    mcrt_bvh4_node *walked_nodes = nullptr; bool walked_stale = true;
    Buf<uint4> d_nodes_walk;
    Buf<uint4> d_meshes;
    Buf<uint32_t> d_tri_slot;
    Buf<float4> d_tris_id;
    uint32_t n_mesh = 0, n_mat = 0, start_mat = 0;
    bool start_silent = false;
    int builder = MCRT_BVH_HOST_SAH; bool host_bvh_stale = false;
    std::vector<uint32_t> tri_mesh;
    float lo[3] = { 0, 0, 0 }, hi[3] = { 0, 0, 0 };
    float spacing[3] = { 1, 1, 1 };
    Event ev_update; hipStream_t update_stream = nullptr; bool update_pending = false;
    ~Scene() { free(walked_nodes); mcrt_free_bvh(&bvh); mcrt_free_bvh4(&bvh4); }
};
struct Tables {
    Buf<double> d_row_thr; uint32_t thr_rows = 0; double thr_dt = 0.0, thr_end = 0.0;
    float verified_res = 0.0f; bool fast_div = false, fast_div_all = false;
    Buf<float4> d_mtab; float mtab_key[2] = { 0.0f, 0.0f }; bool mtab_valid = false;
};
struct Accumulators {
    Buf<long long> d_acc; Buf<uint32_t> d_flags;
    uint32_t clean_ne = 0, clean_rows = 0;
};
struct ImageStages {
    MapCache maps{ 1 }, cmaps{ 1 }, vmaps{ 4 };
    Buf<float> d_tmp;
    Buf<float> d_disp; StagedTable tgc;
    StagedTable lat_rows, elev_rows;
    Buf<unsigned long long> d_recon;
};
struct Instrumentation {
    Buf<unsigned long long> d_stats; bool stats_on = false;
    bool timing_on = false; int timing_level = 0;
    std::vector<TimedLaunch> ev; size_t ev_used = 0;
    float last_lean_bound = 0.0f; uint32_t last_march_rows = 0;
};

struct mcrt_ctx {
    int device = 0; uint32_t n_cu = 256;
    Knobs knobs;
    Stream own_stream; hipStream_t stream = nullptr;
    std::vector<Work> work;
    Event ev_start;
    mcrt_params p{};
    Consts c{};
    Buf<uint32_t> d_error;
    Scene scene;
    Buf<float2> d_tex; uint32_t tex_n = 0; bool tex_finite = false;
    Buf<float> d_pos, d_dir; uint32_t n_el = 0;
    Buf<int> label_ovf;
    Staging pose_stage[2];
    Tables tab;
    Accumulators acc;
    ImageStages img;
    Instrumentation ins;
};

namespace mcrt {
int check_device_error(mcrt_ctx *c);
}
```

mcray-tracing_amd/csrc/mcrt_kernels.h:

```cpp
#pragma once
#include <hip/hip_runtime.h>
#include <stdint.h>
#include "../../include/mcrt.h"
#include "mcrt_internal.h"

namespace mcrt {

struct FrameArgs {
    const uint4 *nodes_walk;
    int *stack_ovf;
    const float4 *tris;
    const float4 *tris_id;
    const uint4 *meshes;
    const float4 *mats;
    const float2 *tex;
    const float *el_pos;
    const float *el_dir;
    const double *row_thr;
    float4 *st0, *st1, *st2;
    uint32_t *queue;
    unsigned long long *key0, *key1;
    const uint32_t *tri_slot;
    uint32_t *counts;
    uint32_t *cursors;
    mcrt_segment *segs;
    int32_t *hits;
    float4 *mrec;
    const float4 *mtab;
    uint32_t *seg_count;
    long long *acc;
    uint32_t *flags;
    unsigned long long *stats;
    uint32_t *error_flag;
    unsigned long long *stamps;
    uint32_t n_nodes, S, B, R, e_begin, ne, ne_frame, pose_stride, acc_stride, acc_off, trace_blocks, trace_blocks_wide, wide_from, packet_mask, march_blocks, ksplit_limit, frame, seed, start_mat, tex_n, tex_mask, sanitize, tex_finite, fast_div, want_segs, tex_shift, march_rows, n_mat, n_mesh;
    float scene_lo[3], scene_hi[3];
    float freq, eps, I0, offs, sx, sy, sz, tex_res, axial_res_f, pad_abs, tex_rcp, lean_bound;
    double axial_res_mm, time_step, row_dt, max_travel, sos_d, inv_row_dt;
    double thr_end;
    uint32_t retire_late;
    uint32_t fold_b0;
};

constexpr uint32_t MCRT_ALL_BOUNCES = 0xffffffffu;

struct ConvTaps { float ax[16]; float lat[32]; uint32_t n_ax, n_lat; };

struct PixelPass { uint32_t n, n_pad, F, frames_per_chunk, vec; };

struct BmodeArgs {
    const float *grey;
    const float *map_col, *map_row;
    float *state;
    uint8_t *out;
    float alpha;
    uint32_t E, R, reset;
    PixelPass pass;
};

struct CompoundArgs {
    const float *src;
    const float *maps;
    float *state;
    void *out;
    float alpha;
    uint32_t E, R;
    PixelPass pass;
    uint32_t N, reset;
    uint32_t mode;
    float feather;
    float weight[16];
};
enum { COMPOUND_PLAIN = 0, COMPOUND_WEIGHTED = 1, COMPOUND_MAX = 2, COMPOUND_MEDIAN = 3 };

struct VolumeArgs {
    const float *src;
    const float *maps;
    void *out;
    uint32_t E, R, K;
    PixelPass pass;
};

struct RenderArgs {
    const void *vol;
    float *out;
    uint8_t *out8;
    float *depth;
    float origin[3], di[3], dj[3], ds[3];
    uint32_t nx, ny, n_steps, F, nu, nv, nw;
    uint32_t mode;
    uint32_t row_tile;
    float lo, inv_range, threshold, inv_ramp, opacity, depth_cue, t_cut, inv_steps;
};

#ifndef SRAD_TH
#define SRAD_TH 16
#endif
#ifndef SRAD_TW
#define SRAD_TW 64
#endif
#define SRAD_FUSE_MAX 4
struct SpeckleArgs {
    const float *src;
    float *dst;
    uint32_t H, W;
    uint32_t n;
    uint32_t first;
    uint32_t tx, ty;
    float lam4;
    float q0sq[SRAD_FUSE_MAX], kq[SRAD_FUSE_MAX];
};

#define RECON_TU 32
#define RECON_TV 8
#define RECON_TW 8
#define RECON_MAX_FILL 3
#define RECON_MAX_TILES (1u << 24)
struct ReconArgs {
    const float *stack;
    const float *pos, *dir;
    unsigned long long *sum;
    uint32_t *count;
    float *out;
    uint32_t *count_out;
    uint32_t *stats;
    uint32_t R, n_samples;
    uint32_t nu, nv, nw;
    uint32_t mode, fill_radius, fill_min;
    uint32_t tu, tv;
    float A[9], b[3];
    float row_u, value_max, empty;
    double qscale;
};

struct LabelArgs {
    uint8_t *tissue;
    int32_t *interface;
    uint32_t *crossings;
    uint32_t rule;
    float Ls;
};

struct LabelGatherArgs {
    const uint8_t *src;
    const float *map_plane, *map_col, *map_row;
    uint8_t *out;
    uint32_t E, R, K;
    PixelPass pass;
};

hipError_t launch_init(const FrameArgs &a, hipStream_t st);
hipError_t launch_trace(const FrameArgs &a, uint32_t b, bool stats, hipStream_t st);
hipError_t launch_nodes_walk(const float4 *nodes, uint32_t n_nodes, uint4 *out, hipStream_t st);
hipError_t launch_nodes_walk_decode(const uint4 *walk, uint32_t n_nodes, float4 *out, hipStream_t st);
uint32_t lane_stack_entries();
uint32_t lane_wide_from();
hipError_t launch_shade(const FrameArgs &a, uint32_t b, bool stats, hipStream_t st);
uint32_t path_blocks(size_t np);
hipError_t launch_path(const FrameArgs &a, hipStream_t st);
hipError_t launch_march(const FrameArgs &a, uint32_t b, bool stats, hipStream_t st);
hipError_t launch_finalize(long long *acc, uint32_t *flags, float *rf, uint32_t ne, uint32_t R, const uint32_t *error_flag, hipStream_t st);
hipError_t launch_convolve(float *img, float *tmp, uint32_t n_img, uint32_t E, uint32_t R, const ConvTaps &taps, hipStream_t st);
hipError_t launch_convolve_depth(float *img, float *tmp, uint32_t n_img, uint32_t E, uint32_t R, const ConvTaps &taps, const float *lat, hipStream_t st);
hipError_t launch_elevation(const float *planes, float *rf, uint32_t F, uint32_t K, uint32_t E, uint32_t R, const float *w, hipStream_t st);
hipError_t launch_envelope(float *img, uint32_t E, uint32_t R, hipStream_t st);
hipError_t launch_remap(const float *img, uint32_t n_img, uint32_t E, uint32_t R, const float *map_col, const float *map_row, float *out, uint32_t n, hipStream_t st);
hipError_t launch_bmode_peak(const float *rf, uint32_t F, uint32_t E, uint32_t R, const float *tgc, float *peak, hipStream_t st);
hipError_t launch_bmode_grey(const float *rf, uint32_t F, uint32_t E, uint32_t R, const float *tgc, const float *peak , float ref,
                             float *peak_out , uint32_t mode, float gain, float dr, float *grey, hipStream_t st);
hipError_t launch_bmode(const BmodeArgs &a, hipStream_t st);
hipError_t launch_compound(const CompoundArgs &a, bool out8, hipStream_t st);
hipError_t launch_volume(const VolumeArgs &a, bool out8, hipStream_t st);
hipError_t launch_render(const RenderArgs &a, bool in8, hipStream_t st);
hipError_t launch_srad(SpeckleArgs a, uint32_t F, uint32_t fuse, hipStream_t st);
hipError_t launch_recon_splat(const ReconArgs &a, hipStream_t st);
hipError_t launch_recon_resolve(ReconArgs a, hipStream_t st);
uint32_t label_blocks(size_t lines);
uint32_t label_stack_entries();
hipError_t launch_label(const FrameArgs &a, const LabelArgs &l, hipStream_t st);
hipError_t launch_label_gather(const LabelGatherArgs &a, hipStream_t st);
hipError_t launch_blocks_to_frames(const float *blocks, float *frames, uint32_t F, uint32_t E, uint32_t R, uint32_t G, const uint32_t *off , hipStream_t st);
hipError_t launch_transpose(const float *in, float *out, uint32_t E, uint32_t R, hipStream_t st);
hipError_t launch_math_probe(int op, const double *x, const double *y, double *out, uint32_t n, hipStream_t st);
hipError_t launch_verify_div(float res, float rcp, unsigned long long *bad, hipStream_t st);
hipError_t launch_tris_by_id(const float4 *tris, uint32_t n_tri, float4 *out, hipStream_t st);
hipError_t launch_expand_tris(const float4 *in48, uint32_t n_tri, float4 *out, hipStream_t st);
hipError_t launch_material_table(const float4 *mats, uint32_t n_mat, float axial_res_f, float freq, float4 *mtab, hipStream_t st);
hipError_t launch_philox_probe(const uint32_t c[4], const uint32_t k[2], uint32_t *out, hipStream_t st);

}
```

mcray-tracing_amd/csrc/mcrt_march.hip:

```cpp
#include "mcrt_device.h"

#ifndef MCRT_MARCH_PAIRS_FROM
#define MCRT_MARCH_PAIRS_FROM 1048576
#endif
#ifndef MCRT_MARCH_WAVES
#define MCRT_MARCH_WAVES 6
#endif
#ifndef MCRT_MARCH_TILE
#define MCRT_MARCH_TILE 256
#endif
#ifndef MCRT_MARCH_MTAB
#define MCRT_MARCH_MTAB 32
#endif

namespace mcrt {

MCRT_DEV uint32_t vox_index(float q, uint32_t n, uint32_t mask)
{
    long long i;
    if (!(fabsf(q) < 9.2233720368547758e18f)) i = (long long)0x8000000000000000ull;
    else if (fabsf(q) < 2147483648.0f) i = (long long)(int)q;
    else i = (long long)q;
    return mask ? ((uint32_t)i & mask) : ((uint32_t)i) % n;
}

template <int CTRL> MCRT_DEV int dpp_i(int v) { return __builtin_amdgcn_mov_dpp(v, CTRL, 0xF, 0xF, true); }

#define QP_BCAST(k) ((k) * 0x55)

struct RowBin { double thr; long long bin; };

MCRT_DEV int row_of(double t, const RowBin *rb, uint32_t R, double inv_dt, double thr_end)
{
    if (!(t < thr_end) || !(t >= 0.0)) return -1;
    int r = (int)(t * inv_dt);
    r = r < 0 ? 0 : (r > (int)R - 1 ? (int)R - 1 : r);
    const double lo = rb[r].thr, hi = rb[r + 1].thr;
    if ((t < lo) | !(t < hi)) {
        while (t < rb[r].thr) r--;
        while (t >= rb[r + 1].thr) r++;
    }
    return r;
}

template <bool PADDED>
MCRT_DEV int row_near(double t, int guess, const RowBin *rb, uint32_t R, double inv_dt, double thr_end)
{
    const int r = PADDED ? guess : (guess < 0 ? 0 : (guess > (int)R - 1 ? (int)R - 1 : guess));
    const double lo = rb[r].thr, hi = rb[r + 1].thr;
    if ((t >= lo) & (t < hi)) return r;
    return row_of(t, rb, R, inv_dt, thr_end);
}

MCRT_DEV float div_res(float x, const FrameArgs &a)
{
    const float ax = fabsf(x);
    if (a.fast_div && ((ax > 1e-18f && ax < 1e18f) || x == 0.0f)) {
        const float q0 = x * a.tex_rcp;
        const float r = fmaf(-q0, a.tex_res, x);
        return fmaf(r, a.tex_rcp, q0);
    }
    return x / a.tex_res;
}

MCRT_DEV size_t vox_cell(f3 p, const FrameArgs &a)
{
    const uint32_t vx = vox_index(div_res(p.x, a), a.tex_n, a.tex_mask), vy = vox_index(div_res(p.y, a), a.tex_n, a.tex_mask), vz = vox_index(div_res(p.z, a), a.tex_n, a.tex_mask);
    return ((size_t)vx * a.tex_n + vy) * a.tex_n + vz;
}
MCRT_DEV uint32_t vox_lean1(float x, const FrameArgs &a)
{
    const float q0 = x * a.tex_rcp;
    const float r = fmaf(-q0, a.tex_res, x);
    return (uint32_t)(int)fmaf(r, a.tex_rcp, q0) & a.tex_mask;
}
MCRT_DEV uint32_t vox_cell_lean(f3 p, const FrameArgs &a)
{
    return (((vox_lean1(p.x, a) << a.tex_shift) | vox_lean1(p.y, a)) << a.tex_shift) | vox_lean1(p.z, a);
}
MCRT_DEV uint32_t vox_q(float x, const FrameArgs &a)
{
    const float q0 = x * a.tex_rcp;
    const float r = fmaf(-q0, a.tex_res, x);
    return (uint32_t)(int)fmaf(r, a.tex_rcp, q0);
}
MCRT_DEV uint32_t vox_cell_lean256(f3 p, const FrameArgs &a)
{
    const uint32_t yz = __builtin_amdgcn_perm(vox_q(p.y, a), vox_q(p.z, a), 0x0c0c0400u);
    return __builtin_amdgcn_perm(vox_q(p.x, a), yz, 0x0c040100u);
}
MCRT_DEV float vgpr(float s) { float v = s; asm volatile("" : "+v"(v)); return v; }
MCRT_DEV uint32_t vox_q_v(float x, float rcp_v, float res_v)
{
    const float q0 = x * rcp_v;
    const float r = fmaf(-q0, res_v, x);
    return (uint32_t)(int)fmaf(r, rcp_v, q0);
}
MCRT_DEV uint32_t vox_cell_lean256_v(f3 p, float rcp_v, float res_v)
{
    const uint32_t yz = __builtin_amdgcn_perm(vox_q_v(p.y, rcp_v, res_v), vox_q_v(p.z, rcp_v, res_v), 0x0c0c0400u);
    return __builtin_amdgcn_perm(vox_q_v(p.x, rcp_v, res_v), yz, 0x0c040100u);
}
MCRT_DEV float abs_sum(f3 p) { return (fabsf(p.x) + fabsf(p.y)) + fabsf(p.z); }

MCRT_DEV void rf_add(RowBin *rb, uint32_t *lflags, int row, float echo)
{
    if (row < 0) return;
    if (!(fabsf(echo) < 1024.0f)) { atomicOr(&lflags[row >> 5], 1u << (row & 31)); return; }
    const long long v = fix40(echo);
    if (v != 0) atomicAdd((unsigned long long *)&rb[row].bin, (unsigned long long)v);
}

template <bool STATS, int G, bool FAST>
__global__ void __launch_bounds__(256, MCRT_MARCH_WAVES) k_march(FrameArgs a, uint32_t b, uint32_t chunks)
{
    constexpr int H = 8 / G;
#ifndef MCRT_MARCH_REFILL_DIV
#define MCRT_MARCH_REFILL_DIV 4
#endif
    constexpr int REFILL = (64 / G) / MCRT_MARCH_REFILL_DIV;
    extern __shared__ __attribute__((aligned(16))) unsigned char smem[];
    const int tid = threadIdx.x, nthr = blockDim.x, lane = tid & 63, wv = tid >> 6, j = tid & (G - 1);
    const uint32_t R = a.R, nf = (R + 31u) >> 5, nrt = FAST ? a.march_rows : R + 1u;
    RowBin *rb = (RowBin *)smem;
    uint32_t *lflags = (uint32_t *)(rb + nrt);
    uint32_t *sort_cnt = lflags + ((nf + 3u) & ~3u) + wv * 64;
    unsigned char *sort_list = (unsigned char *)(lflags + ((nf + 3u) & ~3u) + 4 * 64) + wv * MCRT_MARCH_TILE;
    unsigned char *sort_cls = (unsigned char *)(lflags + ((nf + 3u) & ~3u) + 4 * 64) + 4 * MCRT_MARCH_TILE + wv * MCRT_MARCH_TILE;
    float4 *mtab_l = (float4 *)((unsigned char *)(lflags + ((nf + 3u) & ~3u) + 4 * 64) + 8 * MCRT_MARCH_TILE);
    const bool mtab_in_lds = a.n_mat <= (uint32_t)MCRT_MARCH_MTAB;
    for (uint32_t r = tid; r < nrt; r += nthr) { rb[r].thr = r <= R ? a.row_thr[r] : -__builtin_inf(); rb[r].bin = 0; }
    for (uint32_t r = tid; r < nf; r += nthr) lflags[r] = 0u;
    if (mtab_in_lds) for (uint32_t r = tid; r < a.n_mat; r += nthr) mtab_l[r] = a.mtab[r];
    __syncthreads();
    auto mtab_row = [&](int m) -> float4 { float4 v; if (mtab_in_lds) { v = mtab_l[m]; asm volatile("" : "+v"(v.x), "+v"(v.y), "+v"(v.z), "+v"(v.w)); } else v = a.mtab[m]; return v; };
#define MCRT_MTAB(m) mtab_row(m)

    uint32_t bid = blockIdx.x;
    if (gridDim.x % MCRT_XCDS == 0u) bid = (blockIdx.x % MCRT_XCDS) * (gridDim.x / MCRT_XCDS) + blockIdx.x / MCRT_XCDS;
    const uint32_t F = a.ne / a.ne_frame, ol = bid / chunks, chunk = bid % chunks;
    const uint32_t line = (ol % F) * a.ne_frame + ol / F;
    const uint32_t per = (a.S + chunks * 4u - 1u) / (chunks * 4u);
    const uint32_t s_begin = min(a.S, (chunk * 4u + (uint32_t)wv) * per), s_end = min(a.S, s_begin + per);
    const size_t pid0 = (size_t)line * a.S;
    unsigned long long st_steps = 0;

    uint32_t tile0 = s_begin, list_base = s_begin, list_n = 0, list_pos = 0;
    bool tiles_left = s_begin < s_end;
    const double thr_end = a.row_thr[R];
    bool busy = false;
    f3 point = mk(0, 0, 0), delta = mk(0, 0, 0);
    double t = 0.0, t_start = 0.0;
    float inten = 0.0f, k_att = 0.0f, seg_refl = 0.0f, m_dens = 0.0f, m_sigma = 0.0f, m_mu = 0.0f;
    uint32_t sidx = 0, steps = 0;
    bool more = false;
    const bool all_b = b == MCRT_ALL_BOUNCES;
    uint32_t seg_b = all_b ? 0u : b, seg_n = 0; size_t seg_pid = 0;
    const float rcp_v = vgpr(a.tex_rcp), res_v = vgpr(a.tex_res);
#define MCRT_LOAD_SEGMENT() { \
        const float4 *mr = a.mrec + 3 * ((size_t)seg_b * a.ne * a.S + seg_pid); \
        const float4 g0 = mr[0], g1 = mr[1], g2 = mr[2]; \
        const float4 mt = MCRT_MTAB(__float_as_int(g2.w)); \
        point = mk(g0.x, g0.y, g0.z); seg_refl = g0.w; \
        delta = mk(g1.x, g1.y, g1.z); inten = g1.w; \
        t_start = __hiloint2double(__float_as_int(g2.y), __float_as_int(g2.x)); \
        steps = __float_as_uint(g2.z); \
        m_mu = mt.x; m_dens = mt.y; m_sigma = mt.z; k_att = mt.w; \
        t = t_start; sidx = (uint32_t)j; \
         \
        const bool silent = a.tex_finite && m_mu == 0.0f && m_sigma == 0.0f; \
        more = !silent && steps > 0u && t < a.max_travel; \
        _Pragma("unroll") for (int u = 1; u < G; u++) if (j >= u) MCRT_ADVANCE() \
        busy = true; }
#define MCRT_ADVANCE() { point = point + delta; t = t + a.time_step; inten *= k_att; }
    for (;;) {
        const bool fin = busy && !more;
        if (popc_mask(__ballot((!busy || fin) && j == 0)) >= (uint32_t)REFILL || !__any(busy && more)) {
            if (fin) {
                if (j == 0) {
                    const double te = t_start + a.time_step * (double)(uint32_t)(steps - 1u);
                    rf_add(rb, lflags, row_of(te, rb, R, a.inv_row_dt, thr_end), seg_refl / (float)a.S);
                }
                busy = false;
                if (all_b && seg_b + 1u < seg_n) { seg_b++; MCRT_LOAD_SEGMENT() }
            }
            while (list_pos < list_n || tiles_left) {
                if (list_pos >= list_n) {
                    const uint32_t t1 = min(s_end, tile0 + (uint32_t)MCRT_MARCH_TILE);
                    sort_cnt[lane] = 0u;
                    __builtin_amdgcn_fence(__ATOMIC_RELEASE, "wavefront"); __builtin_amdgcn_wave_barrier();
                    auto slot_class = [&](uint32_t slot) -> uint32_t {
                        if (slot >= t1) return 0xffffffffu;
                        const uint32_t sn = a.seg_count[pid0 + slot], sb0 = all_b ? 0u : b;
                        if (sb0 >= sn) return 0xffffffffu;
                        uint32_t its = 0u;
                        if (!all_b) {
                            const float4 g2 = a.mrec[3 * ((size_t)sb0 * a.ne * a.S + pid0 + slot) + 2];
                            const float4 mt = MCRT_MTAB(__float_as_int(g2.w));
                            const bool silent = a.tex_finite && mt.x == 0.0f && mt.z == 0.0f;
                            its = silent ? 0u : (__float_as_uint(g2.z) + 7u) >> 3;
                        }
                        return 63u - (its < 63u ? its : 63u);
                    };
                    for (int k = 0; k < MCRT_MARCH_TILE / 64; k++) {
                        const uint32_t c = slot_class(tile0 + (uint32_t)(k * 64 + lane));
                        sort_cls[k * 64 + lane] = (unsigned char)c;
                        if (c != 0xffffffffu) atomicAdd(&sort_cnt[c], 1u);
                    }
                    __builtin_amdgcn_fence(__ATOMIC_ACQ_REL, "wavefront"); __builtin_amdgcn_wave_barrier();
                    const uint32_t mine_cnt = sort_cnt[lane];
                    uint32_t incl = mine_cnt;
#pragma unroll
                    for (int d = 1; d < 64; d <<= 1) { const uint32_t o = (uint32_t)__shfl_up((int)incl, d, 64); if (lane >= d) incl += o; }
                    __builtin_amdgcn_fence(__ATOMIC_ACQ_REL, "wavefront"); __builtin_amdgcn_wave_barrier();
                    sort_cnt[lane] = incl - mine_cnt;
                    __builtin_amdgcn_fence(__ATOMIC_ACQ_REL, "wavefront"); __builtin_amdgcn_wave_barrier();
                    for (int k = 0; k < MCRT_MARCH_TILE / 64; k++) {
                        const uint32_t c = (uint32_t)sort_cls[k * 64 + lane];
                        if (c != 0xffu) sort_list[atomicAdd(&sort_cnt[c], 1u)] = (unsigned char)(k * 64 + lane);
                    }
                    __builtin_amdgcn_fence(__ATOMIC_ACQ_REL, "wavefront"); __builtin_amdgcn_wave_barrier();
                    list_n = (uint32_t)__shfl((int)incl, 63, 64); list_pos = 0u;
                    list_base = tile0; tile0 = t1; tiles_left = t1 < s_end;
                    continue;
                }
                const unsigned long long want = __ballot(!busy && j == 0);
                if (popc_mask(want) < (uint32_t)REFILL) break;
                const uint32_t mine = list_pos + (uint32_t)__popcll(want & ((1ull << (lane & ~(G - 1))) - 1ull));
                if (!busy && mine < list_n) {
                    seg_pid = pid0 + list_base + (uint32_t)sort_list[mine];
                    seg_b = all_b ? 0u : b;
                    seg_n = all_b ? a.seg_count[seg_pid] : b + 1u;
                    if (seg_b < seg_n) MCRT_LOAD_SEGMENT()
                }
                const uint32_t nw = (uint32_t)__popcll(want);
                list_pos = (list_pos + nw < list_n) ? list_pos + nw : list_n;
            }
        }
        if (!__any(busy)) { if (list_pos >= list_n && !tiles_left) break; else continue; }

        if (busy && more) {
            f3 myp[H]; double myt[H]; float myin[H]; bool myv[H];
            float reach = 0.0f;
#pragma unroll
            for (int h = 0; h < H; h++) {
                myp[h] = point; myt[h] = t; myin[h] = inten; myv[h] = sidx < steps && t < a.max_travel;
                if (h == 0 || h == H - 1) reach += abs_sum(point);
#pragma unroll
                for (int u = 0; u < G; u++) MCRT_ADVANCE()
                sidx += (uint32_t)G;
            }
            more = dpp_i<G == 4 ? QP_BCAST(0) : 0xA0>((sidx < steps && t < a.max_travel) ? 1 : 0) != 0;
            float2 vox[H];
            if (reach < a.lean_bound) {
#pragma unroll
                for (int h = 0; h < H; h++) vox[h] = a.tex[FAST ? vox_cell_lean256_v(myp[h], rcp_v, res_v) : vox_cell_lean(myp[h], a)];
            } else {
#pragma unroll
                for (int h = 0; h < H; h++) vox[h] = myv[h] ? a.tex[vox_cell(myp[h], a)] : make_float2(0.0f, 0.0f);
            }
            int rows[H];
#pragma unroll
            for (int h = 0; h < H; h++)
                rows[h] = myv[h] ? row_near<FAST>(myt[h], (int)(myt[h] * a.inv_row_dt), rb, R, a.inv_row_dt, thr_end) : -1;
#pragma unroll
            for (int h = 0; h < H; h++) {
                if (myv[h]) {
                    const float scattering = vox[h].y >= m_dens ? vox[h].x * m_sigma + m_mu : 0.0f;
                    rf_add(rb, lflags, rows[h], myin[h] * scattering);
                    if (STATS) st_steps++;
                }
            }
        }
    }
#undef MCRT_ADVANCE
#undef MCRT_LOAD_SEGMENT
#undef MCRT_MTAB
    if (STATS) {
        long long x = wave_sum_i64((long long)st_steps);
        if (lane == 0 && x) atomicAdd(&a.stats[4], (unsigned long long)x);
    }
    __syncthreads();
    const size_t row = (size_t)(line / a.ne_frame) * a.acc_stride + a.acc_off + line % a.ne_frame;
    for (uint32_t r = tid; r < R; r += nthr) {
        const long long v = rb[r].bin;
        if (v != 0) atomicAdd((unsigned long long *)&a.acc[row * R + r], (unsigned long long)v);
    }
    for (uint32_t r = tid; r < nf; r += nthr) { const uint32_t f = lflags[r]; if (f) atomicOr(&a.flags[row * nf + r], f); }
}

__global__ void k_material_table(const float4 *mats, uint32_t n_mat, float axial_res_f, float freq, float4 *mtab)
{
    const uint32_t m = blockIdx.x * blockDim.x + threadIdx.x;
    if (m >= n_mat) return;
    const float4 s0 = mats[2 * m], s1 = mats[2 * m + 1];
    mtab[m] = make_float4(s0.z, s0.w, s1.x, det_expf(-s0.y * axial_res_f * 0.01f * freq * 1.0f));
}

size_t march_lds_bytes(uint32_t R, uint32_t rows)
{
    const size_t img = (size_t)rows * 16, flg = (size_t)((((R + 31u) >> 5) + 3u) & ~3u) * 4;
    return img + flg + 4 * (64 * 4 + 2 * MCRT_MARCH_TILE) + 16 * MCRT_MARCH_MTAB;
}

hipError_t launch_march(const FrameArgs &a, uint32_t b, bool stats, hipStream_t st)
{
    uint32_t target = a.march_blocks;
    if (!target) { target = (uint32_t)(1024.0 * sqrt((double)a.ne * a.S / 131072.0)); if (target < 1024u) target = 1024u; }
    uint32_t chunks = a.ne >= target ? 1u : (a.march_blocks ? (target + a.ne - 1u) / a.ne : target / a.ne);
    const uint32_t max_chunks = (a.S + 63u) / 64u;
    if (chunks > max_chunks) chunks = max_chunks;
    if (chunks < 1u) chunks = 1u;
    const dim3 grid(a.ne * chunks), blk(256);
    const bool fast = !stats && a.march_rows != 0u;
    const size_t lds = march_lds_bytes(a.R, fast ? a.march_rows : a.R + 1u);
    const bool pairs = (size_t)a.ne * a.S >= (size_t)MCRT_MARCH_PAIRS_FROM;
    if (stats) { if (pairs) hipLaunchKernelGGL((k_march<true, 2, false>), grid, blk, lds, st, a, b, chunks); else hipLaunchKernelGGL((k_march<true, 4, false>), grid, blk, lds, st, a, b, chunks); }
    else if (fast) { if (pairs) hipLaunchKernelGGL((k_march<false, 2, true>), grid, blk, lds, st, a, b, chunks); else hipLaunchKernelGGL((k_march<false, 4, true>), grid, blk, lds, st, a, b, chunks); }
    else { if (pairs) hipLaunchKernelGGL((k_march<false, 2, false>), grid, blk, lds, st, a, b, chunks); else hipLaunchKernelGGL((k_march<false, 4, false>), grid, blk, lds, st, a, b, chunks); }
    return hipGetLastError();
}

hipError_t launch_material_table(const float4 *mats, uint32_t n_mat, float axial_res_f, float freq, float4 *mtab, hipStream_t st)
{
    hipLaunchKernelGGL(k_material_table, dim3((n_mat + 63u) / 64u), dim3(64), 0, st, mats, n_mat, axial_res_f, freq, mtab);
    return hipGetLastError();
}

}
```

mcray-tracing_amd/csrc/mcrt_path.hip:

```cpp
#include "mcrt_device.h"
#include "mcrt_walk.h"
#include "mcrt_shade.h"

namespace mcrt {

#ifndef MCRT_PATH_WAVES
#define MCRT_PATH_WAVES 4
#endif
#ifndef MCRT_PATH_ADOPT_STEPS
#define MCRT_PATH_ADOPT_STEPS 1
#endif
#ifndef MCRT_PATH_LEAF_BATCH
#define MCRT_PATH_LEAF_BATCH MCRT_LANE_LEAF_BATCH
#endif
#ifndef MCRT_PATH_LEAF_GATE
#define MCRT_PATH_LEAF_GATE 16
#endif
static_assert(MCRT_PATH_LEAF_GATE <= MCRT_PATH_LEAF_BATCH, "k_path: with more parked lanes than MCRT_PATH_LEAF_BATCH the inner-node phase stops stepping, so the leaf phase must have started by then");
#ifndef MCRT_PATH_OWNERS
#define MCRT_PATH_OWNERS 32
#endif
__global__ void __launch_bounds__(256, MCRT_PATH_WAVES) k_path(FrameArgs a)
{
    __shared__ int stack[MCRT_LANE_STACK * 256];
    __shared__ unsigned long long wbest[256];
    __shared__ unsigned char donor_of[256];
    __shared__ float4 mats_l[2 * MCRT_SHADE_TABLE];
    __shared__ uint4 meshes_l[MCRT_SHADE_TABLE];
    const int tid = threadIdx.x, lane = tid & 63;
    const uint32_t np = a.ne * a.S, pos = (blockIdx.x * 4u + (uint32_t)(tid >> 6)) * (uint32_t)MCRT_PATH_OWNERS + (uint32_t)lane;
    const bool tables_in_lds = a.n_mat <= (uint32_t)MCRT_SHADE_TABLE && a.n_mesh <= (uint32_t)MCRT_SHADE_TABLE;
    if (tables_in_lds) {
        for (uint32_t r = tid; r < 2u * a.n_mat; r += blockDim.x) mats_l[r] = a.mats[r];
        for (uint32_t r = tid; r < a.n_mesh; r += blockDim.x) meshes_l[r] = a.meshes[r];
        __syncthreads();
    }
    const ShadeTables tb = { a.mats, a.meshes, mats_l, meshes_l, tables_in_lds };
    const LaneStackT<MCRT_LANE_STACK> S = { stack, a.stack_ovf + ((size_t)blockIdx.x * 256 + tid), (size_t)gridDim.x * 256, tid };
    bool alive = lane < MCRT_PATH_OWNERS && pos < np;
    uint32_t pid = 0; float Ls = 0.0f;
    PathState ps; ps.from = mk(0, 0, 0); ps.dir = mk(0, 0, 1); ps.intensity = 0.0f; ps.media = 0; ps.outside = OUT_NONE; ps.dist_mm = 0.0;
    if (alive) {
        pid = a.queue[pos];
        const uint32_t p0 = MCRT_STATE0_AT(pos, a.S);
        const float4 s0 = a.st0[p0], s1 = a.st1[p0], s2 = a.st2[p0];
        ps.from = mk(s0.x, s0.y, s0.z); Ls = s0.w; ps.dir = mk(s1.x, s1.y, s1.z); ps.media = __float_as_int(s1.w);
        ps.dist_mm = __hiloint2double(__float_as_int(s2.y), __float_as_int(s2.x)); ps.outside = __float_as_int(s2.z); ps.intensity = s2.w;
    }
#define MCRT_WORD(bst) (((unsigned long long)__float_as_uint((bst).frac) << 32) | (unsigned long long)(uint32_t)(bst).tri)
    MCRT_WATCHDOG_DECL()
    bool abandoned = false;
    for (uint32_t b = 0; b < a.B && !abandoned; b++) {
        if (!__any(alive)) break;
        f3 f2 = mk(0, 0, 0), to = mk(1, 1, 1), inv = mk(1, 1, 1);
        float t_lo = 0.0f;
        Best best; best.frac = 1.0f; best.tri = -1;
        int sp = 0, sb = 0, cur = CUR_IDLE, owner = tid;
        bool fresh = true, shared = false, helper = false;
        unsigned long long poll_old = 0; int poll_owner = -1; bool poll_pending = false;
        wbest[tid] = MCRT_KEY_MISS;
        const bool leads = b != 0u || lane == 0 || pos % a.S == 0u;
        const unsigned long long lead_mask = __ballot(alive && leads);
        if (alive && leads) {
            const Ray ry = ray_of(ps.from, ps.dir, Ls, a);
            f2 = ry.f2; to = ry.to;
            const f3 d = to - f2;
            inv = mk(rcp_dir(d.x), rcp_dir(d.y), rcp_dir(d.z));
            cur = a.n_nodes != 0u ? 0 : CUR_IDLE; fresh = false;
        }
        __builtin_amdgcn_fence(__ATOMIC_RELEASE, "wavefront"); __builtin_amdgcn_wave_barrier();
        for (;;) {
            { if ((++wd_iter & 4095u) == 0u && wall_clock64() - wd_start > (unsigned long long)MCRT_WATCHDOG_SECONDS * 100000000ull) { if (lane == 0) atomicOr(a.error_flag, 2u); abandoned = true; break; } }
            if (cur == CUR_IDLE && !fresh) {
                if (best.tri >= 0) atomicMin(&wbest[owner], MCRT_WORD(best));
                fresh = true; shared = false; helper = false;
            }
            if (MCRT_WALKING(cur) == 0ull) break;
            {
                const bool thief = cur == CUR_IDLE && fresh;
                const bool donor = cur != CUR_IDLE && sp > sb && sb < MCRT_LANE_STACK;
                const unsigned long long tm = __ballot(thief), dm = __ballot(donor);
                if (tm != 0ull && dm != 0ull) {
                    const unsigned long long below = (1ull << lane) - 1ull;
                    const uint32_t pairs = (uint32_t)min(__popcll(tm), __popcll(dm));
                    const uint32_t trank = (uint32_t)__popcll(tm & below), drank = (uint32_t)__popcll(dm & below);
                    const bool take = thief && trank < pairs, give = donor && drank < pairs;
                    if (give) donor_of[(tid & ~63) + (int)drank] = (unsigned char)lane;
                    __builtin_amdgcn_fence(__ATOMIC_ACQ_REL, "wavefront"); __builtin_amdgcn_wave_barrier();
                    const int src = take ? (int)donor_of[(tid & ~63) + (int)trank] : lane;
                    const int d_sb = __shfl(sb, src, 64);
                    const float c0 = __shfl(f2.x, src, 64), c1 = __shfl(f2.y, src, 64), c2 = __shfl(f2.z, src, 64);
                    const float c3 = __shfl(to.x, src, 64), c4 = __shfl(to.y, src, 64), c5 = __shfl(to.z, src, 64);
                    const float c6 = __shfl(inv.x, src, 64), c7 = __shfl(inv.y, src, 64), c8 = __shfl(inv.z, src, 64);
                    const float c10 = __shfl(best.frac, src, 64);
                    const int c11 = __shfl(owner, src, 64);
                    const int c12 = __shfl(best.tri, src, 64), c13 = __shfl((int)helper, src, 64);
                    if (take) {
                        cur = stack[d_sb * 256 + (tid & ~63) + src];
                        f2 = mk(c0, c1, c2); to = mk(c3, c4, c5); inv = mk(c6, c7, c8);
                        best.frac = c10; best.tri = -1; owner = c11;
                        sp = 0; sb = 0; fresh = false; shared = true;
                        helper = c12 >= 0 || c13 != 0;
                    }
                    if (give) { sb++; shared = true; }
                }
            }
            const float tcap = fminf(1.0f, best.frac);
            const int thieves_wait = __builtin_amdgcn_readfirstlane(__any(cur == CUR_IDLE && fresh) ? 1 : 0);
            int steps_left = thieves_wait ? MCRT_PATH_ADOPT_STEPS : 0x7fffffff;
            const f3 rc = ray_c(f2, inv);
            const LaneRay lr = { rc.x, rc.y, rc.z, inv.x, inv.y, inv.z, inv.x < 0.0f, inv.y < 0.0f, inv.z < 0.0f };
            for (;;) {
                const unsigned long long inner = MCRT_ON_INNER(cur);
                if (inner == 0ull) break;
                if (popc_mask(MCRT_ON_LEAF(cur)) >= (uint32_t)MCRT_PATH_LEAF_BATCH) break;
                if (--steps_left < 0) break;
                if (cur >= 0) lane_node_step(a, S, lr, t_lo, tcap, cur, sp, sb);
            }
            if (popc_mask(MCRT_ON_LEAF(cur)) >= (uint32_t)MCRT_PATH_LEAF_GATE || MCRT_ON_INNER(cur) == 0ull)
            if ((uint32_t)cur > 0x80000000u) lane_leaf_test(a, S, f2, to, inv, rc, t_lo, helper, best, cur, sp, sb);
            if (poll_pending) {
                poll_pending = false;
                const unsigned long long mine = MCRT_WORD(best);
                if (poll_owner == owner && cur != CUR_IDLE && poll_old < mine) {
                    best.frac = __uint_as_float((uint32_t)(poll_old >> 32)); best.tri = (int)(uint32_t)poll_old; helper = false;
                }
            }
            if (shared && cur != CUR_IDLE) {
                const unsigned long long word = (best.tri >= 0) ? MCRT_WORD(best) : ~0ull;
                poll_old = atomicMin(&wbest[owner], word); poll_owner = owner; poll_pending = true;
            }
        }
        __builtin_amdgcn_fence(__ATOMIC_ACQ_REL, "wavefront"); __builtin_amdgcn_wave_barrier();
        if (abandoned) break;
        if (alive) {
            const int leader = 63 - __clzll((long long)(lead_mask & ((2ull << lane) - 1ull)));
            const unsigned long long key = wbest[(tid & ~63) + leader];
            const Ray ry = ray_of(ps.from, ps.dir, Ls, a);
            bool reflected = false; unsigned long long st_seg = 0, st_hits = 0;
            alive = shade_path<false>(a, tb, b, pid, ps, ry.f2, ry.to, key, reflected, st_seg, st_hits);
            if (alive) Ls = ray_len(ps.intensity, tb.mat(2 * ps.media).y, a);
        }
    }
#undef MCRT_WORD
}

uint32_t path_blocks(size_t np) { return (uint32_t)((np + 4u * MCRT_PATH_OWNERS - 1u) / (4u * MCRT_PATH_OWNERS)); }
hipError_t launch_path(const FrameArgs &a, hipStream_t st)
{
    hipLaunchKernelGGL(k_path, dim3(path_blocks((size_t)a.ne * a.S)), dim3(256), 0, st, a);
    return hipGetLastError();
}

}
```

mcray-tracing_amd/csrc/mcrt_shade.h:

```cpp
#pragma once
#include "mcrt_device.h"

namespace mcrt {

struct Hit { float frac; int tri; int mesh; f3 n; float da; };

struct PathState { f3 from, dir; float intensity; int media, outside; double dist_mm; };

struct ShadeTables {
    const float4 *mats_g; const uint4 *meshes_g; const float4 *mats_l; const uint4 *meshes_l; bool lds;
    MCRT_DEV float4 mat(uint32_t r) const { float4 v; if (lds) { v = mats_l[r]; asm volatile("" : "+v"(v.x), "+v"(v.y), "+v"(v.z), "+v"(v.w)); } else v = mats_g[r]; return v; }
    MCRT_DEV uint4 mesh(uint32_t r) const { uint4 v; if (lds) { v = meshes_l[r]; asm volatile("" : "+v"(v.x), "+v"(v.y), "+v"(v.z), "+v"(v.w)); } else v = meshes_g[r]; return v; }
};
struct FoldEcho { float refl; uint32_t steps; double t_start; };
template <bool STATS, bool FOLD = false>
MCRT_DEV bool shade_path(const FrameArgs &a, const ShadeTables &tb, uint32_t b, uint32_t pid, PathState &ps, f3 f2, f3 to, unsigned long long key, bool &reflected,
                         unsigned long long &st_seg, unsigned long long &st_hits, FoldEcho *fo = nullptr)
{
    bool alive = false;
    f3 from = ps.from, dir = ps.dir;
    float intensity = ps.intensity; int media = ps.media, outside = ps.outside; double dist_mm = ps.dist_mm;
    reflected = false;
    {
        Hit best; best.frac = __uint_as_float((uint32_t)(key >> 32)); best.tri = (int)(uint32_t)key; best.da = 0.0f; best.mesh = 0; best.n = mk(0, 0, 0);
        if (best.tri >= 0) {
            const float4 *T = a.tris_id + MCRT_TRI_PIECES * (size_t)best.tri;
            const float4 t2 = T[1];
            const float4 P = tri_plane(xyz(T[0]), xyz(t2), xyz(T[2]));
            best.n = xyz(P);
            best.da = dot(best.n, f2) - P.w;
            best.mesh = __float_as_int(t2.w);
        }
        const uint32_t line = pid / a.S, fr = line / a.ne_frame;
        const uint32_t e_abs = a.e_begin + (line - fr * a.ne_frame);
        Rng g; g.k0 = a.seed; g.k1 = a.frame + fr; g.element = e_abs; g.sample = pid - line * a.S; g.bounce = b;
        const float4 m0 = tb.mat(2 * media);
        const float att = m0.y;

        f3 seg_to = to;
        float seg_refl = 0.0f; const float seg_init = intensity; const double seg_dist = dist_mm;
        const f3 seg_from = from, seg_dir = dir; const int seg_media = media; int seg_tri = -1;
        if (best.tri >= 0) {
            if (STATS) st_hits++;
            f3 nn = normalized(best.n);
            if (best.da <= 0.0f) nn = neg(nn);
            const float sfr = 1.0f - best.frac;
            const f3 hp = mk(sfr * f2.x + best.frac * to.x, sfr * f2.y + best.frac * to.y, sfr * f2.z + best.frac * to.z);
            const uint4 organ = tb.mesh(best.mesh);
            const float sigma_t = tb.mat(2 * organ.x + 1).w;
            float qpen = 0.0f;
            if (sigma_t != 0.0f) {
                double n1, n2, sn, cs;
                rng_block(g, 0u, n1, n2);
                det_sincos(n2 * 2 * PI_D, sn, cs);
                const double z = sqrt(-2.0 * det_log(1.0 - n1)) * cs;
                qpen = (float)fabs(z * (double)sigma_t + 0.0);
            }
            const f3 inside = mk(qpen * dir.x + hp.x, qpen * dir.y + hp.y, qpen * dir.z + hp.z);
            const float xd = fabsf(from.x - inside.x) * a.sx, yd = fabsf(from.y - inside.y) * a.sy, zd = fabsf(from.z - inside.z) * a.sz;
            const double mm = sqrt((double)xd * (double)xd + (double)yd * (double)yd + (double)zd * (double)zd) * 10;
            dist_mm = dist_mm + mm;
            intensity = intensity * det_expf(-att * ((float)mm * 0.01f) * a.freq);

            int after_vasc, mat_after;
            if (outside != OUT_NONE) {
                if (organ.z) { after_vasc = OUT_NONE; mat_after = (outside == OUT_SELF) ? media : outside; }
                else { after_vasc = (outside == (int)organ.x) ? (int)organ.y : (int)organ.x; mat_after = media; }
            } else {
                if (organ.z) { after_vasc = OUT_SELF; mat_after = (int)organ.x; }
                else { after_vasc = OUT_NONE; mat_after = (int)organ.x; }
            }
            const float4 a0 = tb.mat(2 * mat_after), a1 = tb.mat(2 * mat_after + 1);
            double u_pc, u_x;
            rng_block(g, 1u, u_pc, u_x);
            const int indice = (int)a1.z + 1;
            const float exponente = (float)((double)1.0 / indice);
            const float random_angle = (float)det_pow_pos(u_pc, (double)exponente);
            const f3 rn = random_unit_vector(nn, random_angle, g);

            float inc = dot(dir, neg(rn));
            if (inc < 0) inc = dot(dir, rn);
            const float rr = m0.x / a0.x;
            float refa = 1 - rr * rr * (1 - inc * inc);
            const bool tir = refa < 0;
            refa = sqrtf(refa);
            const float kk = rr * inc - refa;
            f3 refr = mk(rr * dir.x + kk * rn.x, rr * dir.y + kk * rn.y, rr * dir.z + kk * rn.z);
            refr = normalized(refr);
            const float two_c = 2 * inc;
            f3 refl = mk(dir.x + two_c * rn.x, dir.y + two_c * rn.y, dir.z + two_c * rn.z);
            refl = normalized(refl);

            float i_refl;
            if (tir) i_refl = intensity;
            else {
                const float num = m0.x * inc - a0.x * refa;
                const float den = m0.x * inc + a0.x * refa;
                const float qq = num / den;
                i_refl = (float)((double)intensity * ((double)qq * (double)qq));
            }
            const float i_refr = intensity - i_refl;

            const float ra = dot(dir, refr);
            float refraction_factor = det_powf(ra, a1.y);
            const float rb = dot(dir, refl);
            const float reflection_factor = det_powf(rb, a1.y);
            if (a.sanitize && tir) refraction_factor = 0.0f;
            seg_refl = (std_max(refraction_factor, 0.0f) + std_max(reflection_factor, 0.0f)) * random_angle;
            seg_to = inside;
            seg_tri = best.tri;

            const float x = (float)u_x;
            const float prob = i_refl / intensity;
            float i_new;
            from = hp;
            if (prob > x) { dir = refl; i_new = i_refl > a.eps ? i_refl : 0.0f; reflected = true; }
            else { dir = refr; media = mat_after; outside = after_vasc; i_new = i_refr > a.eps ? i_refr : 0.0f; }
            if (i_new > a.eps) { intensity = i_new; alive = true; }
        }
        if (STATS) st_seg++;

        {
            const f3 df = seg_to - seg_from;
            const float dist_f = sqrtf(dot(df, df)) * 10.0f;
            const uint32_t steps = steps_from((double)dist_f / a.axial_res_mm);
            const double t_start = (seg_dist * 1000.0) / a.sos_d;
            if (FOLD) { fo->refl = seg_refl; fo->steps = steps; fo->t_start = t_start; }
            else {
                float4 *mr = a.mrec + 3 * ((size_t)b * a.ne * a.S + pid);
                mr[0] = make_float4(seg_from.x, seg_from.y, seg_from.z, seg_refl);
                mr[1] = make_float4(a.axial_res_f * seg_dir.x, a.axial_res_f * seg_dir.y, a.axial_res_f * seg_dir.z, seg_init);
                mr[2] = make_float4(__int_as_float(__double2loint(t_start)), __int_as_float(__double2hiint(t_start)), __uint_as_float(steps), __int_as_float(seg_media));
            }
        }
        if (a.want_segs) {
            mcrt_segment sg;
            sg.from[0] = seg_from.x; sg.from[1] = seg_from.y; sg.from[2] = seg_from.z;
            sg.to[0] = seg_to.x; sg.to[1] = seg_to.y; sg.to[2] = seg_to.z;
            sg.dir[0] = seg_dir.x; sg.dir[1] = seg_dir.y; sg.dir[2] = seg_dir.z;
            sg.reflected_intensity = seg_refl; sg.initial_intensity = seg_init; sg.attenuation = att;
            sg.distance_traveled = seg_dist; sg.media = seg_media; sg.tri = seg_tri;
            a.segs[(size_t)pid * a.B + b] = sg;
        }
        if (a.hits) a.hits[(size_t)pid * a.B + b] = seg_tri;
        a.seg_count[pid] = b + 1u;
        alive = alive && (b + 1u < a.B);
        if (alive && a.retire_late) {
            const double t_next = (dist_mm * 1000.0) / a.sos_d;
            if (!(t_next < a.max_travel) && !(t_next < a.thr_end) && t_next == t_next) alive = false;
        }
    }
    ps.from = from; ps.dir = dir; ps.intensity = intensity; ps.media = media; ps.outside = outside; ps.dist_mm = dist_mm;
    return alive;
}

}
```

mcray-tracing_amd/csrc/mcrt_shade.hip:

```cpp
#include "mcrt_device.h"
#include "mcrt_shade.h"

#ifndef MCRT_SHADE_WAVES
#define MCRT_SHADE_WAVES 5
#endif

namespace mcrt {


__global__ void __launch_bounds__(256) k_init(FrameArgs a)
{
    const uint32_t pos = blockIdx.x * blockDim.x + threadIdx.x;
    const uint32_t np = a.ne * a.S;
    if (pos == 0) { a.counts[0] = np; for (uint32_t b = 1; b <= a.B; b++) a.counts[b] = 0u; }
    if (pos < MCRT_MAX_BOUNCES * MCRT_XCDS) a.cursors[(size_t)pos * MCRT_CURSOR_STRIDE] = 0u;
    if (pos >= np) return;
    const uint32_t F = a.ne / a.ne_frame;
    const uint32_t qline = pos / a.S, sample = pos % a.S;
    const uint32_t scan = qline / F, fr = qline % F;
    const uint32_t pid = (fr * a.ne_frame + scan) * a.S + sample;
    const size_t pe = (size_t)fr * a.pose_stride + a.e_begin + scan;
    const f3 from = mk(a.el_pos[3 * pe], a.el_pos[3 * pe + 1], a.el_pos[3 * pe + 2]);
    const f3 dir = mk(a.el_dir[3 * pe], a.el_dir[3 * pe + 1], a.el_dir[3 * pe + 2]);
    const float intensity = a.I0 / (float)a.S;
    if (sample == 0u) {
        a.st0[pos] = make_float4(from.x, from.y, from.z, ray_len(intensity, a.mats[2 * a.start_mat].y, a));
        a.st1[pos] = make_float4(dir.x, dir.y, dir.z, __int_as_float((int)a.start_mat));
        a.st2[pos] = make_float4(0.0f, 0.0f, __int_as_float(OUT_NONE), intensity);
    }
    a.queue[pos] = pid;
    a.seg_count[pid] = 0u;
    if (pos < a.ne) a.key0[pos] = MCRT_KEY_MISS;
}

template <bool STATS, bool FOLD>
MCRT_DEV void shade_bounce(const FrameArgs &a, uint32_t b)
{
    const uint32_t n = a.counts[b];
    const uint32_t i = blockIdx.x * blockDim.x + threadIdx.x;
    if (blockIdx.x * blockDim.x >= n) return;
    const int lane = threadIdx.x & 63;
    __shared__ float4 mats_l[2 * MCRT_SHADE_TABLE];
    __shared__ uint4 meshes_l[MCRT_SHADE_TABLE];
    const bool tables_in_lds = a.n_mat <= (uint32_t)MCRT_SHADE_TABLE && a.n_mesh <= (uint32_t)MCRT_SHADE_TABLE;
    if (tables_in_lds) {
        for (uint32_t r = threadIdx.x; r < 2u * a.n_mat; r += blockDim.x) mats_l[r] = a.mats[r];
        for (uint32_t r = threadIdx.x; r < a.n_mesh; r += blockDim.x) meshes_l[r] = a.meshes[r];
        __syncthreads();
    }
    __shared__ long long fold_bin[FOLD ? MCRT_MAX_ROWS : 1];
    __shared__ uint32_t fold_flag[FOLD ? MCRT_MAX_ROWS / 32 : 1];
    if (FOLD) {
        for (uint32_t r = threadIdx.x; r < a.R; r += blockDim.x) fold_bin[r] = 0;
        for (uint32_t r = threadIdx.x; r < (a.R + 31u) >> 5; r += blockDim.x) fold_flag[r] = 0u;
        __syncthreads();
    }
    const ShadeTables tb = { a.mats, a.meshes, mats_l, meshes_l, tables_in_lds };
    const uint32_t *q_in = a.queue + (size_t)(b & 1u) * a.ne * a.S;
    uint32_t *q_out = a.queue + (size_t)((b + 1u) & 1u) * a.ne * a.S;
    const bool valid = i < n;
    bool alive = false, reflected = false;
    uint32_t pid = 0;
    PathState ps; ps.from = mk(0, 0, 0); ps.dir = mk(0, 0, 1); ps.intensity = 0.0f; ps.media = 0; ps.outside = OUT_NONE; ps.dist_mm = 0.0;
    unsigned long long st_seg = 0, st_hits = 0;
    if (valid) {
        pid = q_in[i];
        const size_t sin = (size_t)(b & 1u) * a.ne * a.S + (b == 0u ? MCRT_STATE0_AT(i, a.S) : i);
        const float4 s0 = a.st0[sin], s1 = a.st1[sin], s2 = a.st2[sin];
        ps.from = mk(s0.x, s0.y, s0.z); ps.intensity = s2.w;
        ps.dir = mk(s1.x, s1.y, s1.z); ps.media = __float_as_int(s1.w);
        ps.dist_mm = __hiloint2double(__float_as_int(s2.y), __float_as_int(s2.x));
        ps.outside = __float_as_int(s2.z);
        const Ray ry = ray_of(ps.from, ps.dir, s0.w, a);
        const f3 f2 = ry.f2, to = ry.to;
        const size_t hi = (b == 0u) ? (size_t)(i / a.S) : (size_t)i;
        const unsigned long long key = ((b & 1u) ? a.key1 : a.key0)[hi];
        FoldEcho fo;
        alive = shade_path<STATS, FOLD>(a, tb, b, pid, ps, f2, to, key, reflected, st_seg, st_hits, &fo);
        if (FOLD) {
            const double te = fo.t_start + a.time_step * (double)(uint32_t)(fo.steps - 1u);
            const int row = row_of_thr(te, a.row_thr, a.R, a.inv_row_dt, a.thr_end);
            if (row >= 0) {
                const float echo = fo.refl / (float)a.S;
                if (!(fabsf(echo) < 1024.0f)) atomicOr(&fold_flag[row >> 5], 1u << (row & 31));
                else { const long long v = fix40(echo); if (v != 0) atomicAdd((unsigned long long *)&fold_bin[row], (unsigned long long)v); }
            }
        }
    }
    const f3 from = ps.from, dir = ps.dir; const float intensity = ps.intensity; const int media = ps.media, outside = ps.outside; const double dist_mm = ps.dist_mm;

    __shared__ uint32_t wave_live[4], wave_refl[4], block_base;
    const unsigned long long live = __ballot(alive);
    const unsigned long long live_refl = __ballot(alive && reflected);
    const int wv = threadIdx.x >> 6;
    if (lane == 0) { wave_live[wv] = (uint32_t)__popcll(live); wave_refl[wv] = (uint32_t)__popcll(live_refl); }
    __syncthreads();
    if (threadIdx.x == 0) {
        const uint32_t total = wave_live[0] + wave_live[1] + wave_live[2] + wave_live[3];
        block_base = total ? atomicAdd(&a.counts[b + 1u], total) : 0u;
    }
    __syncthreads();
    if (live) {
        const uint32_t refl_all = wave_refl[0] + wave_refl[1] + wave_refl[2] + wave_refl[3];
        uint32_t refl_before = 0, refr_before = 0;
        for (int w = 0; w < wv; w++) { refl_before += wave_refl[w]; refr_before += wave_live[w] - wave_refl[w]; }
        if (alive) {
            const unsigned long long below = (1ull << lane) - 1ull;
            const uint32_t pos = block_base + (reflected ? refl_before + (uint32_t)__popcll(live_refl & below)
                                                         : refl_all + refr_before + (uint32_t)__popcll(live & ~live_refl & below));
            q_out[pos] = pid;
            ((b & 1u) ? a.key0 : a.key1)[pos] = MCRT_KEY_MISS;
            const size_t so = (size_t)((b + 1u) & 1u) * a.ne * a.S + pos;
            a.st0[so] = make_float4(from.x, from.y, from.z, ray_len(intensity, tb.mat(2 * media).y, a));
            a.st1[so] = make_float4(dir.x, dir.y, dir.z, __int_as_float(media));
            a.st2[so] = make_float4(__int_as_float(__double2loint(dist_mm)), __int_as_float(__double2hiint(dist_mm)), __int_as_float(outside), intensity);
        }
    }
    if (STATS) {
        long long x = wave_sum_i64((long long)st_seg), y = wave_sum_i64((long long)st_hits);
        if (lane == 0) { if (x) atomicAdd(&a.stats[3], (unsigned long long)x); if (y) atomicAdd(&a.stats[5], (unsigned long long)y); }
    }
    if (FOLD) {
        const uint32_t F = a.ne / a.ne_frame, ql = (blockIdx.x * blockDim.x) / a.S;
        const uint32_t line = (ql % F) * a.ne_frame + ql / F;
        const size_t row = (size_t)(line / a.ne_frame) * a.acc_stride + a.acc_off + line % a.ne_frame;
        const uint32_t nf = (a.R + 31u) >> 5;
        for (uint32_t r = threadIdx.x; r < a.R; r += blockDim.x) {
            const long long v = fold_bin[r];
            if (v != 0) atomicAdd((unsigned long long *)&a.acc[row * a.R + r], (unsigned long long)v);
        }
        for (uint32_t r = threadIdx.x; r < nf; r += blockDim.x) { const uint32_t f = fold_flag[r]; if (f) atomicOr(&a.flags[row * nf + r], f); }
    }
}

template <bool STATS>
__global__ void __launch_bounds__(256, MCRT_SHADE_WAVES) k_shade(FrameArgs a, uint32_t b) { shade_bounce<STATS, false>(a, b); }
__global__ void __launch_bounds__(256, MCRT_SHADE_WAVES) k_shade_fold(FrameArgs a) { shade_bounce<false, true>(a, 0u); }

hipError_t launch_init(const FrameArgs &a, hipStream_t st)
{
    const uint32_t np = a.ne * a.S;
    hipLaunchKernelGGL(k_init, dim3((np + 255u) / 256u), dim3(256), 0, st, a);
    return hipGetLastError();
}

hipError_t launch_shade(const FrameArgs &a, uint32_t b, bool stats, hipStream_t st)
{
    const uint32_t np = a.ne * a.S;
    const dim3 grid((np + 255u) / 256u), blk(256);
    if (stats) hipLaunchKernelGGL((k_shade<true>), grid, blk, 0, st, a, b);
    else if (a.fold_b0 && b == 0u) hipLaunchKernelGGL(k_shade_fold, grid, blk, 0, st, a);
    else hipLaunchKernelGGL((k_shade<false>), grid, blk, 0, st, a, b);
    return hipGetLastError();
}

}
```

mcray-tracing_amd/csrc/mcrt_trace.cpp:

```cpp
#include "mcrt_ctx.h"
#include "mcrt_kernels.h"

#include <hip/hip_runtime.h>
#include <cmath>
#include <cstring>
#include <vector>
#include <algorithm>
#include <utility>

using mcrt::set_error;

static int get_work(mcrt_ctx *c, size_t g, Work **out)
{
    while (c->work.size() <= g) {
        Work w;
        for (Event &e : w.ev_join) HIP_TRY(ensure_event(e));
        for (Event &e : w.ev_bounce) HIP_TRY(ensure_event(e));
        HIP_TRY(ensure_event(w.ev_done));
        c->work.push_back(std::move(w));
    }
    *out = &c->work[g];
    return MCRT_OK;
}

static int work_stream(Work &w, hipStream_t *out)
{
    if (!w.stream) HIP_TRY(hipStreamCreateWithFlags(&w.stream.h, hipStreamNonBlocking));
    *out = w.stream;
    return MCRT_OK;
}
static int side_stream(mcrt_ctx *c, Work &w, uint32_t i, hipStream_t *out)
{
    if (!w.side[i]) {
        int prio_low = 0, prio_high = 0;
        HIP_TRY(hipDeviceGetStreamPriorityRange(&prio_low, &prio_high));
        if (c->knobs.no_priority) prio_low = 0;
        HIP_TRY(hipStreamCreateWithPriority(&w.side[i].h, hipStreamNonBlocking, prio_low));
    }
    *out = w.side[i];
    return MCRT_OK;
}

static int ensure_acc(mcrt_ctx *c, uint32_t ne)
{
    const size_t need = (size_t)ne * c->p.n_rows, needf = (size_t)ne * ((c->p.n_rows + 31u) >> 5);
    if (need > c->acc.d_acc.cap || needf > c->acc.d_flags.cap) {
        HIP_TRY(hipStreamSynchronize(c->stream));
        c->acc.clean_ne = 0;
        HIP_TRY(c->acc.d_acc.grow(need)); HIP_TRY(c->acc.d_flags.grow(needf));
    }
    if (c->acc.clean_ne != ne || c->acc.clean_rows != c->p.n_rows) {
        HIP_TRY(hipMemsetAsync(c->acc.d_acc, 0, need * 8, c->stream));
        HIP_TRY(hipMemsetAsync(c->acc.d_flags, 0, needf * 4, c->stream));
    }
    c->acc.clean_ne = 0; c->acc.clean_rows = 0;
    return MCRT_OK;
}

static int check_ready(mcrt_ctx *c, uint32_t e0, uint32_t e1, const float *pose_pos = nullptr)
{
    if (!c->scene.have) return set_error(MCRT_ERR_INVALID, "no scene uploaded");
    if (!c->d_tex) return set_error(MCRT_ERR_INVALID, "no texture uploaded");
    if (c->tex_n != c->p.tex_n) return set_error(MCRT_ERR_INVALID, "texture is %u^3 but params say %u^3", c->tex_n, c->p.tex_n);
    if (!pose_pos) {
        if (!c->d_pos) return set_error(MCRT_ERR_INVALID, "no transducer set");
        if (c->n_el != c->p.n_elements) return set_error(MCRT_ERR_INVALID, "transducer has %u elements but params say %u", c->n_el, c->p.n_elements);
    }
    if (e0 >= e1 || e1 > c->p.n_elements) return set_error(MCRT_ERR_INVALID, "scan-line range [%u,%u) invalid for %u elements", e0, e1, c->p.n_elements);
    return MCRT_OK;
}

struct Plan {
    bool latency = false;
    uint32_t groups = 1;
    uint32_t trace_blocks = 0, trace_blocks_wide = 0;
    uint32_t e[17] = {};
    uint32_t sides[16] = {};
    size_t ovf[16] = {};
};

static Plan plan_pass(const mcrt_ctx *c, uint32_t e0, uint32_t e1, uint32_t n_frames, bool one_group)
{
    Plan P;
    const uint32_t ne = e1 - e0, S = c->p.n_samples;
    P.latency = !c->ins.stats_on && (uint64_t)ne * n_frames * S <= c->knobs.path_max;
    uint32_t groups = (one_group || c->ins.stats_on) ? 1u : c->knobs.groups;
    if (!one_group && groups == 1u && P.latency) groups = c->knobs.path_groups;
    P.groups = std::max(1u, std::min({ groups, ne, 16u }));
    for (uint32_t g = 0; g <= P.groups; g++) P.e[g] = e0 + (uint32_t)(((uint64_t)ne * g) / P.groups);
    P.trace_blocks = c->knobs.trace_blocks ? c->knobs.trace_blocks : c->n_cu * 4u;
    P.trace_blocks_wide = c->knobs.trace_blocks_wide ? c->knobs.trace_blocks_wide : c->n_cu * 5u;
    if ((uint64_t)c->scene.bvh4.n_nodes * 64ull > (uint64_t)c->knobs.wide_max_tree_mb * 1048576ull) P.trace_blocks_wide = 0;
    const uint32_t lds_part = mcrt::lane_stack_entries();
    const size_t deep = c->scene.bvh4.max_stack > lds_part ? c->scene.bvh4.max_stack - lds_part : 0;
    for (uint32_t g = 0; g < P.groups; g++) {
        const uint64_t np = (uint64_t)(P.e[g + 1] - P.e[g]) * n_frames * S;
        if (!P.latency) P.sides[g] = c->knobs.march_streams ? c->knobs.march_streams : (P.trace_blocks_wide != 0u && np >= (uint64_t)MCRT_SIDE_STREAMS_TWO_FROM) ? 2u : 1u;
        uint32_t blocks = std::max({ c->knobs.trace_blocks, c->knobs.trace_blocks_wide, c->n_cu * 5u });
        if (P.latency) blocks = std::max(blocks, mcrt::path_blocks(np));
        P.ovf[g] = deep * blocks * 256;
    }
    return P;
}

static int ensure_work(Work &w, size_t np, uint32_t B, size_t ovf, int out)
{
    if (out >= 2 && w.segs.cap < np * B) { HIP_TRY(hipDeviceSynchronize()); HIP_TRY(w.segs.alloc(np * B)); }
    if (out >= 1 && w.hits.cap < np * B) { HIP_TRY(hipDeviceSynchronize()); HIP_TRY(w.hits.alloc(np * B)); }
    if (ovf > w.stack_ovf.cap) { HIP_TRY(hipDeviceSynchronize()); HIP_TRY(w.stack_ovf.alloc(ovf)); }
    if (np <= w.b.paths && B <= w.b.depth) return MCRT_OK;
    HIP_TRY(hipDeviceSynchronize());
    w.b = PathBufs();
    PathBufs &b = w.b;
    HIP_TRY(b.st0.alloc(2 * np)); HIP_TRY(b.st1.alloc(2 * np)); HIP_TRY(b.st2.alloc(2 * np));
    HIP_TRY(b.key0.alloc(np)); HIP_TRY(b.key1.alloc(np));
    HIP_TRY(b.q.alloc(2 * np)); HIP_TRY(b.seg_count.alloc(np));
    HIP_TRY(b.counts.alloc(MCRT_MAX_BOUNCES + 1));
    HIP_TRY(b.cursors.alloc((size_t)MCRT_MAX_BOUNCES * MCRT_XCDS * MCRT_CURSOR_STRIDE));
    HIP_TRY(b.mrec.alloc(3 * np * B));
    b.paths = np; b.depth = B;
    return MCRT_OK;
}

static void fill_pass(mcrt_ctx *c, const Plan &P, mcrt::FrameArgs &a, uint32_t frame, uint32_t acc_ne, bool accumulate, int out, const float *pose_pos, const float *pose_dir)
{
    memset(&a, 0, sizeof a);
    a.nodes_walk = c->scene.d_nodes_walk; a.tris = c->scene.d_tris; a.meshes = c->scene.d_meshes; a.mats = c->scene.d_mats; a.tex = c->d_tex;
    a.el_pos = pose_pos ? pose_pos : c->d_pos; a.el_dir = pose_pos ? pose_dir : c->d_dir; a.pose_stride = pose_pos ? c->p.n_elements : 0u;
    a.row_thr = c->tab.d_row_thr;
    a.acc = c->acc.d_acc; a.flags = c->acc.d_flags; a.acc_stride = acc_ne;
    a.tri_slot = c->scene.d_tri_slot; a.tris_id = c->scene.d_tris_id; a.mtab = c->tab.d_mtab;
    a.stats = c->ins.d_stats; a.error_flag = c->d_error; a.stamps = c->ins.d_stats + 8;
    a.n_mat = c->scene.n_mat; a.n_mesh = c->scene.n_mesh; a.n_nodes = c->scene.bvh4.n_nodes; a.S = c->p.n_samples; a.B = c->p.max_depth; a.R = c->p.n_rows;
    a.ksplit_limit = c->knobs.ksplit_limit;
    if (c->ins.stats_on) a.ksplit_limit = 0;
    for (int i = 0; i < 3; i++) { a.scene_lo[i] = c->scene.lo[i]; a.scene_hi[i] = c->scene.hi[i]; }
    a.trace_blocks = P.trace_blocks; a.trace_blocks_wide = P.trace_blocks_wide;
    a.wide_from = c->knobs.wide_from ? c->knobs.wide_from : mcrt::lane_wide_from();
    a.march_blocks = c->knobs.march_blocks;
    a.want_segs = out >= 2 ? 1u : 0u;
    a.frame = frame; a.seed = c->p.seed; a.start_mat = c->scene.start_mat; a.tex_n = c->tex_n; a.tex_mask = (c->tex_n & (c->tex_n - 1u)) == 0u ? c->tex_n - 1u : 0u;
    a.sanitize = c->p.sanitize_tir; a.tex_finite = c->tex_finite ? 1u : 0u;
    a.freq = c->p.frequency; a.eps = c->p.intensity_epsilon; a.I0 = c->p.initial_intensity; a.offs = c->p.ray_start_offset;
    a.sx = c->scene.spacing[0]; a.sy = c->scene.spacing[1]; a.sz = c->scene.spacing[2]; a.tex_res = c->p.tex_res; a.axial_res_f = c->c.axial_res_f; a.pad_abs = c->scene.bvh.pad_abs; a.tex_rcp = 1.0f / c->p.tex_res; a.fast_div = c->tab.fast_div ? 1u : 0u;
    a.tex_shift = 0; while ((1u << a.tex_shift) < c->tex_n) a.tex_shift++;
    a.lean_bound = 0.0f;
    if (c->tab.fast_div_all && a.tex_mask && a.tex_shift <= 10u) {
        const float lim = 2147483648.0f * c->p.tex_res * (1.0f - 0x1p-20f);
        a.lean_bound = lim < 1e18f ? lim : 1e18f;
        if (!(a.lean_bound > 0.0f)) a.lean_bound = 0.0f;
    }
    a.axial_res_mm = c->c.axial_res_mm; a.time_step = c->c.time_step_us; a.row_dt = c->c.row_dt_us;
    a.max_travel = c->c.max_travel_us; a.sos_d = (double)c->p.speed_of_sound; a.inv_row_dt = 1.0 / c->c.row_dt_us;
    a.march_rows = 0u;
    {
        const double g = a.max_travel * a.inv_row_dt;
        if (a.lean_bound > 0.0f && c->tex_n == 256u && g >= 0.0 && g < (double)(MCRT_MAX_ROWS + 1)) {
            const uint32_t gmax = (uint32_t)g;
            a.march_rows = (gmax + 2u > c->p.n_rows + 1u) ? gmax + 2u : c->p.n_rows + 1u;
        }
    }
    c->ins.last_lean_bound = a.lean_bound; c->ins.last_march_rows = a.march_rows;
    const bool image_only = !c->ins.stats_on && out == 0;
    a.thr_end = c->tab.thr_end;
    a.retire_late = image_only && c->knobs.retire_late ? 1u : 0u;
    a.fold_b0 = image_only && c->knobs.fold_b0 && !P.latency && accumulate && c->tex_finite && c->scene.start_silent && c->p.n_samples % 256u == 0u ? 1u : 0u;
}

static void fill_group(const mcrt_ctx *c, const Work &w, mcrt::FrameArgs &a, uint32_t n_frames, uint32_t b0, uint32_t b1, uint32_t acc_e0, int out)
{
    a.stack_ovf = w.stack_ovf; a.segs = w.segs; a.hits = out >= 1 ? (int32_t *)w.hits : nullptr;
    a.st0 = w.b.st0; a.st1 = w.b.st1; a.st2 = w.b.st2; a.queue = w.b.q; a.key0 = w.b.key0; a.key1 = w.b.key1;
    a.counts = w.b.counts; a.cursors = w.b.cursors; a.mrec = w.b.mrec; a.seg_count = w.b.seg_count;
    a.acc_off = b0 - acc_e0;
    a.e_begin = b0; a.ne_frame = b1 - b0; a.ne = (b1 - b0) * n_frames;
    a.packet_mask = (c->ins.stats_on || (uint64_t)a.ne * a.S < c->knobs.packet_from) ? 0u : c->knobs.packet_mask;
}

static int check_overflow(const mcrt_ctx *c, const Plan &P, const mcrt::FrameArgs &a, const Work &w)
{
    const uint32_t lds_part = mcrt::lane_stack_entries();
    if (c->scene.bvh4.max_stack <= lds_part) return MCRT_OK;
    const uint32_t blocks = P.latency ? mcrt::path_blocks((size_t)a.ne * a.S) : std::max(a.trace_blocks, a.trace_blocks_wide);
    const size_t need = (size_t)(c->scene.bvh4.max_stack - lds_part) * blocks * 256;
    if (need > w.stack_ovf.cap) return set_error(MCRT_ERR_LIMIT, "traversal-stack overflow: %zu entries needed, the work set holds %zu", need, w.stack_ovf.cap);
    return MCRT_OK;
}

template <class Launch> static int timed_launch(mcrt_ctx *c, int kind, hipStream_t st, Launch launch)
{
    if (!c->ins.timing_on || (kind != 0 && c->ins.timing_level < 2)) { HIP_TRY(launch()); return MCRT_OK; }
    if (c->ins.ev_used == c->ins.ev.size()) {
        if (c->ins.ev.size() >= 65536) return set_error(MCRT_ERR_LIMIT, "timing buffer full: call mcrt_get_kernel_time(reset=1)");
        TimedLaunch t;
        HIP_TRY(hipEventCreate(&t.start.h)); HIP_TRY(hipEventCreate(&t.end.h));
        c->ins.ev.push_back(std::move(t));
    }
    TimedLaunch &t = c->ins.ev[c->ins.ev_used];
    HIP_TRY(hipEventRecord(t.start, st));
    HIP_TRY(launch());
    HIP_TRY(hipEventRecord(t.end, st));
    t.kind = kind; c->ins.ev_used++;
    return MCRT_OK;
}

static int run_bounce(mcrt_ctx *c, Work &w, hipStream_t st, const mcrt::FrameArgs &a, uint32_t b, uint32_t sides, bool accumulate, bool overlap)
{
    MCRT_TRY(timed_launch(c, 0, st, [&] { return mcrt::launch_trace(a, b, c->ins.stats_on, st); }));
    MCRT_TRY(timed_launch(c, 1, st, [&] { return mcrt::launch_shade(a, b, c->ins.stats_on, st); }));
    if (!accumulate || (a.fold_b0 && b == 0u)) return MCRT_OK;
    hipStream_t ms = st;
    if (overlap) {
        HIP_TRY(hipEventRecord(w.ev_bounce[b], st));
        MCRT_TRY(side_stream(c, w, b % sides, &ms));
        HIP_TRY(hipStreamWaitEvent(ms, w.ev_bounce[b], 0));
    }
    return timed_launch(c, 2, ms, [&] { return mcrt::launch_march(a, b, c->ins.stats_on, ms); });
}

static int enqueue_pass(mcrt_ctx *c, const Plan &P, const mcrt::FrameArgs *args, Work *const *ws, bool accumulate)
{
    const bool overlap = !c->knobs.no_overlap;
    hipStream_t gst[16] = { c->stream };
    for (uint32_t g = 1; g < P.groups; g++) MCRT_TRY(work_stream(*ws[g], &gst[g]));
    if (c->scene.update_pending && c->scene.update_stream != c->stream) HIP_TRY(hipStreamWaitEvent(c->stream, c->scene.ev_update, 0));
    HIP_TRY(hipEventRecord(c->ev_start, c->stream));
    for (uint32_t g = 0; g < P.groups; g++) {
        if (gst[g] != c->stream) HIP_TRY(hipStreamWaitEvent(gst[g], c->ev_start, 0));
        HIP_TRY(mcrt::launch_init(args[g], gst[g]));
    }
    if (P.latency) {
        for (uint32_t g = 0; g < P.groups; g++) {
            MCRT_TRY(timed_launch(c, 0, gst[g], [&] { return mcrt::launch_path(args[g], gst[g]); }));
        }
        for (uint32_t g = 0; g < P.groups && accumulate; g++) {
            MCRT_TRY(timed_launch(c, 2, gst[g], [&] { return mcrt::launch_march(args[g], mcrt::MCRT_ALL_BOUNCES, false, gst[g]); }));
        }
    } else {
        for (uint32_t b = 0; b < c->p.max_depth; b++)
            for (uint32_t g = 0; g < P.groups; g++) {
                MCRT_TRY(run_bounce(c, *ws[g], gst[g], args[g], b, P.sides[g], accumulate, overlap));
            }
    }
    for (uint32_t g = 0; g < P.groups; g++) {
        for (uint32_t i = 0; i < P.sides[g] && accumulate && overlap; i++) {
            if (!ws[g]->side[i]) continue;
            HIP_TRY(hipEventRecord(ws[g]->ev_join[i], ws[g]->side[i]));
            HIP_TRY(hipStreamWaitEvent(gst[g], ws[g]->ev_join[i], 0));
        }
        if (gst[g] != c->stream) {
            HIP_TRY(hipEventRecord(ws[g]->ev_done, gst[g]));
            HIP_TRY(hipStreamWaitEvent(c->stream, ws[g]->ev_done, 0));
        }
    }
    return MCRT_OK;
}

static int run_pass(mcrt_ctx *c, uint32_t frame, uint32_t n_frames, uint32_t e0, uint32_t e1, bool accumulate, bool one_group, int out, const float *pose_pos = nullptr, const float *pose_dir = nullptr)
{
    const Plan P = plan_pass(c, e0, e1, n_frames, one_group);
    mcrt::FrameArgs pass, args[16];
    Work *ws[16];
    fill_pass(c, P, pass, frame, e1 - e0, accumulate, out, pose_pos, pose_dir);
    for (uint32_t g = 0; g < P.groups; g++) {
        MCRT_TRY(get_work(c, g, &ws[g]));
        MCRT_TRY(ensure_work(*ws[g], (size_t)(P.e[g + 1] - P.e[g]) * n_frames * c->p.n_samples, c->p.max_depth, P.ovf[g], out));
        args[g] = pass;
        fill_group(c, *ws[g], args[g], n_frames, P.e[g], P.e[g + 1], e0, out);
        MCRT_TRY(check_overflow(c, P, args[g], *ws[g]));
    }
    return enqueue_pass(c, P, args, ws, accumulate);
}

static int finalize(mcrt_ctx *c, float *rf_dev, uint32_t lines)
{
    HIP_TRY(mcrt::launch_finalize(c->acc.d_acc, c->acc.d_flags, rf_dev, lines, c->p.n_rows, c->d_error, c->stream));
    c->acc.clean_ne = lines; c->acc.clean_rows = c->p.n_rows;
    return MCRT_OK;
}

static int trace_frames(mcrt_ctx *c, uint32_t frame, uint32_t n_frames, uint32_t e0, uint32_t e1, const float *pose_pos, const float *pose_dir, float *rf_dev)
{
    CTX_TRY(c);
    MCRT_TRY(check_ready(c, e0, e1, pose_pos));
    if (!rf_dev) return set_error(MCRT_ERR_INVALID, "null rf_dev");
    if (n_frames == 0 || n_frames > 1024) return set_error(MCRT_ERR_LIMIT, "n_frames must be 1..1024");
    if ((uint64_t)(e1 - e0) * n_frames * c->p.n_samples > (1ull << 27))
        return set_error(MCRT_ERR_LIMIT, "%u frames x %u scan-lines x %u samples: more than 2^27 paths in one pass", n_frames, e1 - e0, c->p.n_samples);
    const uint32_t lines = (e1 - e0) * n_frames;
    MCRT_TRY(ensure_acc(c, lines));
    MCRT_TRY(run_pass(c, frame, n_frames, e0, e1, true, false, 0, pose_pos, pose_dir));
    return finalize(c, rf_dev, lines);
}

extern "C" int mcrt_trace_frames(mcrt_ctx *c, uint32_t frame, uint32_t n_frames, uint32_t e0, uint32_t e1, float *rf_dev)
{
    return trace_frames(c, frame, n_frames, e0, e1, nullptr, nullptr, rf_dev);
}

extern "C" int mcrt_trace_frame(mcrt_ctx *c, uint32_t frame, uint32_t e0, uint32_t e1, float *rf_dev)
{
    return mcrt_trace_frames(c, frame, 1, e0, e1, rf_dev);
}

static int stage_poses(mcrt_ctx *c, uint32_t n_frames, const float *dev[2])
{
    const size_t len = 3 * (size_t)n_frames * c->p.n_elements;
    for (int k = 0; k < 2; k++) {
        if (is_device_pointer(dev[k])) continue;
        float *h = nullptr;
        MCRT_TRY(c->pose_stage[k].begin(len, c->stream, &h));
        memcpy(h, dev[k], 4 * len);
        MCRT_TRY(c->pose_stage[k].commit(len, c->stream));
        dev[k] = c->pose_stage[k].dev;
    }
    return MCRT_OK;
}

extern "C" int mcrt_trace_frames_poses(mcrt_ctx *c, uint32_t frame, uint32_t n_frames, uint32_t e0, uint32_t e1,
                                       const float *pos, const float *dir, float *rf_dev)
{
    CTX_TRY(c);
    if (!pos || !dir) return set_error(MCRT_ERR_INVALID, "mcrt_trace_frames_poses: null pose tables");
    if (n_frames == 0 || n_frames > 1024) return set_error(MCRT_ERR_LIMIT, "n_frames must be 1..1024");
    const float *dev[2] = { pos, dir };
    MCRT_TRY(stage_poses(c, n_frames, dev));
    return trace_frames(c, frame, n_frames, e0, e1, dev[0], dev[1], rf_dev);
}

static int copy_out(mcrt_ctx *c, uint32_t ne, int32_t *hits, mcrt_segment *segs, uint32_t *seg_count)
{
    const size_t np = (size_t)ne * c->p.n_samples, B = c->p.max_depth;
    const Work &w = c->work[0];
    HIP_TRY(hipStreamSynchronize(c->stream));
    MCRT_TRY(mcrt::check_device_error(c));
    std::vector<uint32_t> cnt;
    if (!seg_count && (hits || segs)) { cnt.resize(np); seg_count = cnt.data(); }
    if (seg_count) HIP_TRY(hipMemcpy(seg_count, w.b.seg_count, np * 4, hipMemcpyDeviceToHost));
    if (segs) {
        HIP_TRY(hipMemcpy(segs, w.segs, np * B * sizeof(mcrt_segment), hipMemcpyDeviceToHost));
        for (size_t p = 0; p < np; p++)
            for (size_t b = seg_count[p]; b < B; b++) memset(&segs[p * B + b], 0, sizeof(mcrt_segment));
    }
    if (hits) {
        HIP_TRY(hipMemcpy(hits, w.hits, np * B * 4, hipMemcpyDeviceToHost));
        for (size_t p = 0; p < np; p++)
            for (size_t b = seg_count[p]; b < B; b++) hits[p * B + b] = -2;
    }
    return MCRT_OK;
}

extern "C" int mcrt_trace_frame_debug(mcrt_ctx *c, uint32_t frame, uint32_t e0, uint32_t e1, float *rf_dev,
                                      int32_t *hits, mcrt_segment *segs, uint32_t *seg_count)
{
    CTX_TRY(c);
    MCRT_TRY(check_ready(c, e0, e1));
    if (!rf_dev) return set_error(MCRT_ERR_INVALID, "null rf_dev");
    MCRT_TRY(ensure_acc(c, e1 - e0));
    MCRT_TRY(run_pass(c, frame, 1, e0, e1, true, true, segs ? 2 : 1));
    MCRT_TRY(finalize(c, rf_dev, e1 - e0));
    return copy_out(c, e1 - e0, hits, segs, seg_count);
}

extern "C" int mcrt_cast_rays(mcrt_ctx *c, uint32_t frame, uint32_t e0, uint32_t e1, mcrt_segment *segs, uint32_t *seg_count, int32_t *hits)
{
    CTX_TRY(c);
    MCRT_TRY(check_ready(c, e0, e1));
    MCRT_TRY(run_pass(c, frame, 1, e0, e1, false, true, segs ? 2 : 1));
    return copy_out(c, e1 - e0, hits, segs, seg_count);
}

extern "C" int mcrt_default_label_opts(mcrt_label_opts *o)
{
    if (!o) return set_error(MCRT_ERR_INVALID, "mcrt_default_label_opts: null options");
    o->rule = MCRT_LABEL_TRACED; o->start_offset = -1.0f;
    return MCRT_OK;
}

extern "C" int mcrt_label_frames(mcrt_ctx *c, uint32_t n_frames, uint32_t e0, uint32_t e1, const float *pos, const float *dir, const mcrt_label_opts *o,
                                 uint8_t *tissue_dev, int32_t *interface_dev, uint32_t *crossings_dev)
{
    CTX_TRY(c);
    static const char fn[] = "mcrt_label_frames";
    mcrt_label_opts d;
    mcrt_default_label_opts(&d);
    if (!o) o = &d;
    if (!c->scene.have) return set_error(MCRT_ERR_INVALID, "%s: no scene uploaded", fn);
    if ((pos == nullptr) != (dir == nullptr)) return set_error(MCRT_ERR_INVALID, "%s: pos and dir go together (null %s)", fn, pos ? "dir" : "pos");
    if (!pos) {
        if (!c->d_pos) return set_error(MCRT_ERR_INVALID, "%s: no transducer set", fn);
        if (c->n_el != c->p.n_elements) return set_error(MCRT_ERR_INVALID, "%s: transducer has %u elements but params say %u", fn, c->n_el, c->p.n_elements);
        if (n_frames != 1) return set_error(MCRT_ERR_INVALID, "%s: the context's transducer is one pose: n_frames must be 1 (%u)", fn, n_frames);
    }
    if (e0 >= e1 || e1 > c->p.n_elements) return set_error(MCRT_ERR_INVALID, "%s: scan-line range [%u,%u) invalid for %u elements", fn, e0, e1, c->p.n_elements);
    if (!tissue_dev && !interface_dev && !crossings_dev) return set_error(MCRT_ERR_INVALID, "%s: no output asked for", fn);
    if (o->rule != MCRT_LABEL_TRACED && o->rule != MCRT_LABEL_GEOMETRIC) return set_error(MCRT_ERR_INVALID, "%s: unknown rule %u", fn, o->rule);
    if (!std::isfinite(o->start_offset) || o->start_offset == 0.0f) return set_error(MCRT_ERR_INVALID, "%s: start_offset must be finite and not 0 (%g)", fn, (double)o->start_offset);
    if (n_frames == 0) return set_error(MCRT_ERR_INVALID, "%s: n_frames must be 1..1024", fn);
    if (n_frames > 1024) return set_error(MCRT_ERR_LIMIT, "%s: n_frames must be 1..1024 (%u)", fn, n_frames);
    if (c->scene.n_mat > 254) return set_error(MCRT_ERR_LIMIT, "%s: at most 254 materials fit a tissue byte (%u)", fn, c->scene.n_mat);
    const uint32_t lines = (e1 - e0) * n_frames, blocks = mcrt::label_blocks(lines), lds_part = mcrt::label_stack_entries();
    const size_t ovf = c->scene.bvh4.max_stack > lds_part ? (size_t)(c->scene.bvh4.max_stack - lds_part) * blocks * 64 : 0;
    if (ovf > c->label_ovf.cap) { HIP_TRY(hipDeviceSynchronize()); HIP_TRY(c->label_ovf.alloc(ovf)); }
    const float *dev[2] = { pos, dir };
    if (pos) MCRT_TRY(stage_poses(c, n_frames, dev));
    if (c->scene.update_pending && c->scene.update_stream != c->stream) HIP_TRY(hipStreamWaitEvent(c->stream, c->scene.ev_update, 0));
    mcrt::FrameArgs a;
    memset(&a, 0, sizeof a);
    a.nodes_walk = c->scene.d_nodes_walk; a.tris = c->scene.d_tris; a.tris_id = c->scene.d_tris_id; a.meshes = c->scene.d_meshes; a.n_nodes = c->scene.bvh4.n_nodes;
    a.n_mat = c->scene.n_mat; a.n_mesh = c->scene.n_mesh; a.start_mat = c->scene.start_mat; a.pad_abs = c->scene.bvh.pad_abs;
    a.sx = c->scene.spacing[0]; a.sy = c->scene.spacing[1]; a.sz = c->scene.spacing[2];
    a.el_pos = pos ? dev[0] : c->d_pos; a.el_dir = pos ? dev[1] : c->d_dir; a.pose_stride = pos ? c->p.n_elements : 0u;
    a.e_begin = e0; a.ne_frame = e1 - e0; a.ne = lines;
    a.row_thr = c->tab.d_row_thr; a.R = c->p.n_rows; a.thr_end = c->tab.thr_end; a.inv_row_dt = 1.0 / c->c.row_dt_us;
    a.max_travel = c->c.max_travel_us; a.sos_d = (double)c->p.speed_of_sound;
    a.offs = o->start_offset < 0.0f ? c->p.ray_start_offset : o->start_offset;
    a.stack_ovf = c->label_ovf; a.error_flag = c->d_error;
    mcrt::LabelArgs l;
    l.tissue = tissue_dev; l.interface = interface_dev; l.crossings = crossings_dev; l.rule = o->rule; l.Ls = (float)(2.0 * c->p.depth_cm);
    HIP_TRY(mcrt::launch_label(a, l, c->stream));
    return MCRT_OK;
}
```

Before: 486.9 million rays/s.

## Precompute per-material PCV exponent and add optional persistent shade loop

Precomputes the per-material scattering exponent (1/(index+1)) into a table at material-table build time and folds it into the LDS material rows, removing a double-precision divide per scatter in the shade path. It raises the shade kernel's launch-bounds occupancy target from 5 to 6 waves and merges the LDS-fill barriers. It also adds an opt-in grid-stride persistent variant of the shade kernel sized from CU count, off by default. Overwriting a material row field in LDS could affect other readers of that field, and the tighter launch bounds may increase register spilling.

Result: no change. 485.5 million rays/s (-0.3%).

```diff
diff --git a/mcray-tracing_amd/api.py b/mcray-tracing_amd/api.py
--- a/mcray-tracing_amd/api.py
+++ b/mcray-tracing_amd/api.py
@@ -493,6 +493,11 @@
         out = (C.c_uint32 * 4)()
         check(self.L.mcrt_debug_fast_paths(self.h, out))
         return bool(out[0]), bool(out[1]), int(out[2])
+
+    def debug_shade_blocks(self):
+        out = (C.c_uint32 * 4)()
+        check(self.L.mcrt_debug_fast_paths(self.h, out))
+        return int(out[3])
 
     def debug_set_error(self, bits):
         check(self.L.mcrt_debug_set_error(self.h, int(bits)))
diff --git a/mcray-tracing_amd/csrc/mcrt_api.cpp b/mcray-tracing_amd/csrc/mcrt_api.cpp
--- a/mcray-tracing_amd/csrc/mcrt_api.cpp
+++ b/mcray-tracing_amd/csrc/mcrt_api.cpp
@@ -47,6 +47,8 @@
     k.test_hooks = tuning_env("MCRT_TEST_HOOKS") != nullptr;
     if (const char *e = tuning_env("MCRT_RETIRE_LATE")) k.retire_late = atoi(e) != 0;
     if (const char *e = tuning_env("MCRT_FOLD_B0")) k.fold_b0 = atoi(e) != 0;
+    if (const char *e = tuning_env("MCRT_SHADE_PERSIST")) k.shade_persist = atoi(e) != 0;
+    if (const char *e = tuning_env("MCRT_SHADE_BLOCKS")) { int v = atoi(e); if (v >= 1) k.shade_blocks = (uint32_t)v; }
     if (const char *e = tuning_env("MCRT_RENDER_ROW_TILE")) k.render_row_tile = atoi(e) != 0;
     if (const char *e = tuning_env("MCRT_SPECKLE_FUSE")) { int v = atoi(e); if (v == 2 || v == 4) k.speckle_fuse = (uint32_t)v; }
     return k;
@@ -80,7 +82,11 @@
             HIP_TRY(hipStreamSynchronize(c->stream));
             HIP_TRY(c->tab.d_mtab.alloc(c->scene.n_mat));
         }
-        HIP_TRY(mcrt::launch_material_table(c->scene.d_mats, c->scene.n_mat, c->c.axial_res_f, c->p.frequency, c->tab.d_mtab, c->stream));
+        if (c->tab.d_ptab.cap < c->scene.n_mat) {
+            HIP_TRY(hipStreamSynchronize(c->stream));
+            HIP_TRY(c->tab.d_ptab.alloc(c->scene.n_mat));
+        }
+        HIP_TRY(mcrt::launch_material_table(c->scene.d_mats, c->scene.n_mat, c->c.axial_res_f, c->p.frequency, c->tab.d_mtab, c->tab.d_ptab, c->stream));
         c->tab.mtab_key[0] = c->c.axial_res_f; c->tab.mtab_key[1] = c->p.frequency; c->tab.mtab_valid = true;
     }
     return MCRT_OK;
@@ -524,7 +530,7 @@
 {
     CTX_TRY(c);
     if (!out) return set_error(MCRT_ERR_INVALID, "null out pointer");
-    out[0] = c->tab.fast_div ? 1u : 0u; out[1] = c->ins.last_lean_bound > 0.0f ? 1u : 0u; out[2] = c->ins.last_march_rows; out[3] = 0u;
+    out[0] = c->tab.fast_div ? 1u : 0u; out[1] = c->ins.last_lean_bound > 0.0f ? 1u : 0u; out[2] = c->ins.last_march_rows; out[3] = c->ins.last_shade_blocks;
     return MCRT_OK;
 }
 
diff --git a/mcray-tracing_amd/csrc/mcrt_ctx.h b/mcray-tracing_amd/csrc/mcrt_ctx.h
--- a/mcray-tracing_amd/csrc/mcrt_ctx.h
+++ b/mcray-tracing_amd/csrc/mcrt_ctx.h
@@ -37,6 +37,8 @@
     uint32_t packet_mask = MCRT_PACKET_MASK_DEFAULT, packet_from = MCRT_PACKET_FROM;
     bool retire_late = true;
     bool fold_b0 = false;
+    bool shade_persist = false;
+    uint32_t shade_blocks = 0;
     bool render_row_tile = false;
     uint32_t speckle_fuse = MCRT_SPECKLE_FUSE_DEFAULT;
     bool test_hooks = false;
@@ -114,7 +116,7 @@
 struct Tables {
     Buf<double> d_row_thr; uint32_t thr_rows = 0; double thr_dt = 0.0, thr_end = 0.0;
     float verified_res = 0.0f; bool fast_div = false, fast_div_all = false;
-    Buf<float4> d_mtab; float mtab_key[2] = { 0.0f, 0.0f }; bool mtab_valid = false;
+    Buf<float4> d_mtab; Buf<float> d_ptab; float mtab_key[2] = { 0.0f, 0.0f }; bool mtab_valid = false;
 };
 struct Accumulators {
     Buf<long long> d_acc; Buf<uint32_t> d_flags;
@@ -131,7 +133,7 @@
     Buf<unsigned long long> d_stats; bool stats_on = false;
     bool timing_on = false; int timing_level = 0;
     std::vector<TimedLaunch> ev; size_t ev_used = 0;
-    float last_lean_bound = 0.0f; uint32_t last_march_rows = 0;
+    float last_lean_bound = 0.0f; uint32_t last_march_rows = 0, last_shade_blocks = 0;
 };
 
 struct mcrt_ctx {
diff --git a/mcray-tracing_amd/csrc/mcrt_kernels.h b/mcray-tracing_amd/csrc/mcrt_kernels.h
--- a/mcray-tracing_amd/csrc/mcrt_kernels.h
+++ b/mcray-tracing_amd/csrc/mcrt_kernels.h
@@ -27,6 +27,7 @@
     int32_t *hits;
     float4 *mrec;
     const float4 *mtab;
+    const float *ptab;
     uint32_t *seg_count;
     long long *acc;
     uint32_t *flags;
@@ -39,6 +40,7 @@
     double axial_res_mm, time_step, row_dt, max_travel, sos_d, inv_row_dt;
     double thr_end;
     uint32_t retire_late;
+    uint32_t shade_blocks;
     uint32_t fold_b0;
 };
 
@@ -156,6 +158,7 @@
 uint32_t lane_stack_entries();
 uint32_t lane_wide_from();
 hipError_t launch_shade(const FrameArgs &a, uint32_t b, bool stats, hipStream_t st);
+uint32_t shade_waves();
 uint32_t path_blocks(size_t np);
 hipError_t launch_path(const FrameArgs &a, hipStream_t st);
 hipError_t launch_march(const FrameArgs &a, uint32_t b, bool stats, hipStream_t st);
@@ -185,7 +188,7 @@
 hipError_t launch_verify_div(float res, float rcp, unsigned long long *bad, hipStream_t st);
 hipError_t launch_tris_by_id(const float4 *tris, uint32_t n_tri, float4 *out, hipStream_t st);
 hipError_t launch_expand_tris(const float4 *in48, uint32_t n_tri, float4 *out, hipStream_t st);
-hipError_t launch_material_table(const float4 *mats, uint32_t n_mat, float axial_res_f, float freq, float4 *mtab, hipStream_t st);
+hipError_t launch_material_table(const float4 *mats, uint32_t n_mat, float axial_res_f, float freq, float4 *mtab, float *ptab, hipStream_t st);
 hipError_t launch_philox_probe(const uint32_t c[4], const uint32_t k[2], uint32_t *out, hipStream_t st);
 
 }
diff --git a/mcray-tracing_amd/csrc/mcrt_march.hip b/mcray-tracing_amd/csrc/mcrt_march.hip
--- a/mcray-tracing_amd/csrc/mcrt_march.hip
+++ b/mcray-tracing_amd/csrc/mcrt_march.hip
@@ -289,12 +289,14 @@
     for (uint32_t r = tid; r < nf; r += nthr) { const uint32_t f = lflags[r]; if (f) atomicOr(&a.flags[row * nf + r], f); }
 }
 
-__global__ void k_material_table(const float4 *mats, uint32_t n_mat, float axial_res_f, float freq, float4 *mtab)
+__global__ void k_material_table(const float4 *mats, uint32_t n_mat, float axial_res_f, float freq, float4 *mtab, float *ptab)
 {
     const uint32_t m = blockIdx.x * blockDim.x + threadIdx.x;
     if (m >= n_mat) return;
     const float4 s0 = mats[2 * m], s1 = mats[2 * m + 1];
     mtab[m] = make_float4(s0.z, s0.w, s1.x, det_expf(-s0.y * axial_res_f * 0.01f * freq * 1.0f));
+    const int indice = (int)s1.z + 1;
+    ptab[m] = (float)((double)1.0 / indice);
 }
 
 size_t march_lds_bytes(uint32_t R, uint32_t rows)
@@ -321,9 +323,9 @@
     return hipGetLastError();
 }
 
-hipError_t launch_material_table(const float4 *mats, uint32_t n_mat, float axial_res_f, float freq, float4 *mtab, hipStream_t st)
-{
-    hipLaunchKernelGGL(k_material_table, dim3((n_mat + 63u) / 64u), dim3(64), 0, st, mats, n_mat, axial_res_f, freq, mtab);
+hipError_t launch_material_table(const float4 *mats, uint32_t n_mat, float axial_res_f, float freq, float4 *mtab, float *ptab, hipStream_t st)
+{
+    hipLaunchKernelGGL(k_material_table, dim3((n_mat + 63u) / 64u), dim3(64), 0, st, mats, n_mat, axial_res_f, freq, mtab, ptab);
     return hipGetLastError();
 }
 
diff --git a/mcray-tracing_amd/csrc/mcrt_path.hip b/mcray-tracing_amd/csrc/mcrt_path.hip
--- a/mcray-tracing_amd/csrc/mcrt_path.hip
+++ b/mcray-tracing_amd/csrc/mcrt_path.hip
@@ -29,13 +29,9 @@
     __shared__ uint4 meshes_l[MCRT_SHADE_TABLE];
     const int tid = threadIdx.x, lane = tid & 63;
     const uint32_t np = a.ne * a.S, pos = (blockIdx.x * 4u + (uint32_t)(tid >> 6)) * (uint32_t)MCRT_PATH_OWNERS + (uint32_t)lane;
-    const bool tables_in_lds = a.n_mat <= (uint32_t)MCRT_SHADE_TABLE && a.n_mesh <= (uint32_t)MCRT_SHADE_TABLE;
-    if (tables_in_lds) {
-        for (uint32_t r = tid; r < 2u * a.n_mat; r += blockDim.x) mats_l[r] = a.mats[r];
-        for (uint32_t r = tid; r < a.n_mesh; r += blockDim.x) meshes_l[r] = a.meshes[r];
-        __syncthreads();
-    }
-    const ShadeTables tb = { a.mats, a.meshes, mats_l, meshes_l, tables_in_lds };
+    const bool tables_in_lds = shade_tables_fill(a, mats_l, meshes_l);
+    if (tables_in_lds) __syncthreads();
+    const ShadeTables tb = { a.mats, a.meshes, a.ptab, mats_l, meshes_l, tables_in_lds };
     const LaneStackT<MCRT_LANE_STACK> S = { stack, a.stack_ovf + ((size_t)blockIdx.x * 256 + tid), (size_t)gridDim.x * 256, tid };
     bool alive = lane < MCRT_PATH_OWNERS && pos < np;
     uint32_t pid = 0; float Ls = 0.0f;
diff --git a/mcray-tracing_amd/csrc/mcrt_shade.h b/mcray-tracing_amd/csrc/mcrt_shade.h
--- a/mcray-tracing_amd/csrc/mcrt_shade.h
+++ b/mcray-tracing_amd/csrc/mcrt_shade.h
@@ -8,10 +8,19 @@
 struct PathState { f3 from, dir; float intensity; int media, outside; double dist_mm; };
 
 struct ShadeTables {
-    const float4 *mats_g; const uint4 *meshes_g; const float4 *mats_l; const uint4 *meshes_l; bool lds;
+    const float4 *mats_g; const uint4 *meshes_g; const float *ptab_g; const float4 *mats_l; const uint4 *meshes_l; bool lds;
     MCRT_DEV float4 mat(uint32_t r) const { float4 v; if (lds) { v = mats_l[r]; asm volatile("" : "+v"(v.x), "+v"(v.y), "+v"(v.z), "+v"(v.w)); } else v = mats_g[r]; return v; }
     MCRT_DEV uint4 mesh(uint32_t r) const { uint4 v; if (lds) { v = meshes_l[r]; asm volatile("" : "+v"(v.x), "+v"(v.y), "+v"(v.z), "+v"(v.w)); } else v = meshes_g[r]; return v; }
+    MCRT_DEV float pcv_exponent(uint32_t m, const float4 &row0) const { return lds ? row0.z : ptab_g[m]; }
 };
+MCRT_DEV bool shade_tables_fill(const FrameArgs &a, float4 *mats_l, uint4 *meshes_l)
+{
+    if (a.n_mat > (uint32_t)MCRT_SHADE_TABLE || a.n_mesh > (uint32_t)MCRT_SHADE_TABLE) return false;
+    for (uint32_t r = threadIdx.x; r < 2u * a.n_mat; r += blockDim.x) { float4 v = a.mats[r]; if (!(r & 1u)) v.z = a.ptab[r >> 1]; mats_l[r] = v; }
+    for (uint32_t r = threadIdx.x; r < a.n_mesh; r += blockDim.x) meshes_l[r] = a.meshes[r];
+    return true;
+}
+
 struct FoldEcho { float refl; uint32_t steps; double t_start; };
 template <bool STATS, bool FOLD = false>
 MCRT_DEV bool shade_path(const FrameArgs &a, const ShadeTables &tb, uint32_t b, uint32_t pid, PathState &ps, f3 f2, f3 to, unsigned long long key, bool &reflected,
@@ -73,8 +82,7 @@
             const float4 a0 = tb.mat(2 * mat_after), a1 = tb.mat(2 * mat_after + 1);
             double u_pc, u_x;
             rng_block(g, 1u, u_pc, u_x);
-            const int indice = (int)a1.z + 1;
-            const float exponente = (float)((double)1.0 / indice);
+            const float exponente = tb.pcv_exponent((uint32_t)mat_after, a0);
             const float random_angle = (float)det_pow_pos(u_pc, (double)exponente);
             const f3 rn = random_unit_vector(nn, random_angle, g);
 
diff --git a/mcray-tracing_amd/csrc/mcrt_shade.hip b/mcray-tracing_amd/csrc/mcrt_shade.hip
--- a/mcray-tracing_amd/csrc/mcrt_shade.hip
+++ b/mcray-tracing_amd/csrc/mcrt_shade.hip
@@ -2,7 +2,7 @@
 #include "mcrt_shade.h"
 
 #ifndef MCRT_SHADE_WAVES
-#define MCRT_SHADE_WAVES 5
+#define MCRT_SHADE_WAVES 6
 #endif
 
 namespace mcrt {
@@ -33,88 +33,92 @@
     if (pos < a.ne) a.key0[pos] = MCRT_KEY_MISS;
 }
 
-template <bool STATS, bool FOLD>
+template <bool STATS, bool FOLD, bool LOOP>
 MCRT_DEV void shade_bounce(const FrameArgs &a, uint32_t b)
 {
     const uint32_t n = a.counts[b];
-    const uint32_t i = blockIdx.x * blockDim.x + threadIdx.x;
-    if (blockIdx.x * blockDim.x >= n) return;
+    uint32_t base = blockIdx.x * 256u;
+    if (base >= n) return;
+    const uint32_t stride = gridDim.x * 256u;
     const int lane = threadIdx.x & 63;
     __shared__ float4 mats_l[2 * MCRT_SHADE_TABLE];
     __shared__ uint4 meshes_l[MCRT_SHADE_TABLE];
-    const bool tables_in_lds = a.n_mat <= (uint32_t)MCRT_SHADE_TABLE && a.n_mesh <= (uint32_t)MCRT_SHADE_TABLE;
-    if (tables_in_lds) {
-        for (uint32_t r = threadIdx.x; r < 2u * a.n_mat; r += blockDim.x) mats_l[r] = a.mats[r];
-        for (uint32_t r = threadIdx.x; r < a.n_mesh; r += blockDim.x) meshes_l[r] = a.meshes[r];
-        __syncthreads();
-    }
+    const bool tables_in_lds = shade_tables_fill(a, mats_l, meshes_l);
     __shared__ long long fold_bin[FOLD ? MCRT_MAX_ROWS : 1];
     __shared__ uint32_t fold_flag[FOLD ? MCRT_MAX_ROWS / 32 : 1];
     if (FOLD) {
         for (uint32_t r = threadIdx.x; r < a.R; r += blockDim.x) fold_bin[r] = 0;
         for (uint32_t r = threadIdx.x; r < (a.R + 31u) >> 5; r += blockDim.x) fold_flag[r] = 0u;
-        __syncthreads();
     }
-    const ShadeTables tb = { a.mats, a.meshes, mats_l, meshes_l, tables_in_lds };
-    const uint32_t *q_in = a.queue + (size_t)(b & 1u) * a.ne * a.S;
-    uint32_t *q_out = a.queue + (size_t)((b + 1u) & 1u) * a.ne * a.S;
-    const bool valid = i < n;
-    bool alive = false, reflected = false;
-    uint32_t pid = 0;
-    PathState ps; ps.from = mk(0, 0, 0); ps.dir = mk(0, 0, 1); ps.intensity = 0.0f; ps.media = 0; ps.outside = OUT_NONE; ps.dist_mm = 0.0;
+    if (tables_in_lds || FOLD) __syncthreads();
+    const ShadeTables tb = { a.mats, a.meshes, a.ptab, mats_l, meshes_l, tables_in_lds };
+    const size_t half_in = (size_t)(b & 1u) * a.ne * a.S, half_out = (size_t)((b + 1u) & 1u) * a.ne * a.S;
+    const uint32_t *q_in = a.queue + half_in;
+    uint32_t *q_out = a.queue + half_out;
+    const unsigned long long *key_in = (b & 1u) ? a.key1 : a.key0;
     unsigned long long st_seg = 0, st_hits = 0;
-    if (valid) {
-        pid = q_in[i];
-        const size_t sin = (size_t)(b & 1u) * a.ne * a.S + (b == 0u ? MCRT_STATE0_AT(i, a.S) : i);
-        const float4 s0 = a.st0[sin], s1 = a.st1[sin], s2 = a.st2[sin];
-        ps.from = mk(s0.x, s0.y, s0.z); ps.intensity = s2.w;
-        ps.dir = mk(s1.x, s1.y, s1.z); ps.media = __float_as_int(s1.w);
-        ps.dist_mm = __hiloint2double(__float_as_int(s2.y), __float_as_int(s2.x));
-        ps.outside = __float_as_int(s2.z);
-        const Ray ry = ray_of(ps.from, ps.dir, s0.w, a);
-        const f3 f2 = ry.f2, to = ry.to;
-        const size_t hi = (b == 0u) ? (size_t)(i / a.S) : (size_t)i;
-        const unsigned long long key = ((b & 1u) ? a.key1 : a.key0)[hi];
-        FoldEcho fo;
-        alive = shade_path<STATS, FOLD>(a, tb, b, pid, ps, f2, to, key, reflected, st_seg, st_hits, &fo);
-        if (FOLD) {
-            const double te = fo.t_start + a.time_step * (double)(uint32_t)(fo.steps - 1u);
-            const int row = row_of_thr(te, a.row_thr, a.R, a.inv_row_dt, a.thr_end);
-            if (row >= 0) {
-                const float echo = fo.refl / (float)a.S;
-                if (!(fabsf(echo) < 1024.0f)) atomicOr(&fold_flag[row >> 5], 1u << (row & 31));
-                else { const long long v = fix40(echo); if (v != 0) atomicAdd((unsigned long long *)&fold_bin[row], (unsigned long long)v); }
+    __shared__ uint32_t wave_live[2][4], wave_refl[2][4], block_base;
+    for (uint32_t it = 0u;; it++) {
+        const uint32_t i = base + threadIdx.x, next = base + stride;
+        const bool valid = i < n, more = LOOP && next < n;
+        bool alive = false, reflected = false;
+        uint32_t pid = 0;
+        PathState ps; ps.from = mk(0, 0, 0); ps.dir = mk(0, 0, 1); ps.intensity = 0.0f; ps.media = 0; ps.outside = OUT_NONE; ps.dist_mm = 0.0;
+        if (valid) {
+            pid = q_in[i];
+            const size_t sin = half_in + (b == 0u ? MCRT_STATE0_AT(i, a.S) : i);
+            const float4 s0 = a.st0[sin], s1 = a.st1[sin], s2 = a.st2[sin];
+            ps.from = mk(s0.x, s0.y, s0.z); ps.intensity = s2.w;
+            ps.dir = mk(s1.x, s1.y, s1.z); ps.media = __float_as_int(s1.w);
+            ps.dist_mm = __hiloint2double(__float_as_int(s2.y), __float_as_int(s2.x));
+            ps.outside = __float_as_int(s2.z);
+            const Ray ry = ray_of(ps.from, ps.dir, s0.w, a);
+            const f3 f2 = ry.f2, to = ry.to;
+            const size_t hi = (b == 0u) ? (size_t)(i / a.S) : (size_t)i;
+            const unsigned long long key = key_in[hi];
+            FoldEcho fo;
+            alive = shade_path<STATS, FOLD>(a, tb, b, pid, ps, f2, to, key, reflected, st_seg, st_hits, &fo);
+            if (FOLD) {
+                const double te = fo.t_start + a.time_step * (double)(uint32_t)(fo.steps - 1u);
+                const int row = row_of_thr(te, a.row_thr, a.R, a.inv_row_dt, a.thr_end);
+                if (row >= 0) {
+                    const float echo = fo.refl / (float)a.S;
+                    if (!(fabsf(echo) < 1024.0f)) atomicOr(&fold_flag[row >> 5], 1u << (row & 31));
+                    else { const long long v = fix40(echo); if (v != 0) atomicAdd((unsigned long long *)&fold_bin[row], (unsigned long long)v); }
+                }
             }
         }
-    }
-    const f3 from = ps.from, dir = ps.dir; const float intensity = ps.intensity; const int media = ps.media, outside = ps.outside; const double dist_mm = ps.dist_mm;
+        const f3 from = ps.from, dir = ps.dir; const float intensity = ps.intensity; const int media = ps.media, outside = ps.outside; const double dist_mm = ps.dist_mm;
 
-    __shared__ uint32_t wave_live[4], wave_refl[4], block_base;
-    const unsigned long long live = __ballot(alive);
-    const unsigned long long live_refl = __ballot(alive && reflected);
-    const int wv = threadIdx.x >> 6;
-    if (lane == 0) { wave_live[wv] = (uint32_t)__popcll(live); wave_refl[wv] = (uint32_t)__popcll(live_refl); }
-    __syncthreads();
-    if (threadIdx.x == 0) {
-        const uint32_t total = wave_live[0] + wave_live[1] + wave_live[2] + wave_live[3];
-        block_base = total ? atomicAdd(&a.counts[b + 1u], total) : 0u;
-    }
-    __syncthreads();
-    if (live) {
-        const uint32_t refl_all = wave_refl[0] + wave_refl[1] + wave_refl[2] + wave_refl[3];
-        uint32_t refl_before = 0, refr_before = 0;
-        for (int w = 0; w < wv; w++) { refl_before += wave_refl[w]; refr_before += wave_live[w] - wave_refl[w]; }
-        if (alive) {
-            const unsigned long long below = (1ull << lane) - 1ull;
-            const uint32_t pos = block_base + (reflected ? refl_before + (uint32_t)__popcll(live_refl & below)
-                                                         : refl_all + refr_before + (uint32_t)__popcll(live & ~live_refl & below));
-            q_out[pos] = pid;
-            ((b & 1u) ? a.key0 : a.key1)[pos] = MCRT_KEY_MISS;
-            const size_t so = (size_t)((b + 1u) & 1u) * a.ne * a.S + pos;
-            a.st0[so] = make_float4(from.x, from.y, from.z, ray_len(intensity, tb.mat(2 * media).y, a));
-            a.st1[so] = make_float4(dir.x, dir.y, dir.z, __int_as_float(media));
-            a.st2[so] = make_float4(__int_as_float(__double2loint(dist_mm)), __int_as_float(__double2hiint(dist_mm)), __int_as_float(outside), intensity);
+        uint32_t *w_live = wave_live[it & 1u], *w_refl = wave_refl[it & 1u];
+        const unsigned long long live = __ballot(alive);
+        const unsigned long long live_refl = __ballot(alive && reflected);
+        const int wv = threadIdx.x >> 6;
+        if (lane == 0) { w_live[wv] = (uint32_t)__popcll(live); w_refl[wv] = (uint32_t)__popcll(live_refl); }
+        __syncthreads();
+        if (threadIdx.x == 0) {
+            const uint32_t total = w_live[0] + w_live[1] + w_live[2] + w_live[3];
+            block_base = total ? atomicAdd(&a.counts[b + 1u], total) : 0u;
         }
+        __syncthreads();
+        if (live) {
+            const uint32_t refl_all = w_refl[0] + w_refl[1] + w_refl[2] + w_refl[3];
+            uint32_t refl_before = 0, refr_before = 0;
+            for (int w = 0; w < wv; w++) { refl_before += w_refl[w]; refr_before += w_live[w] - w_refl[w]; }
+            if (alive) {
+                const unsigned long long below = (1ull << lane) - 1ull;
+                const uint32_t pos = block_base + (reflected ? refl_before + (uint32_t)__popcll(live_refl & below)
+                                                             : refl_all + refr_before + (uint32_t)__popcll(live & ~live_refl & below));
+                q_out[pos] = pid;
+                ((b & 1u) ? a.key0 : a.key1)[pos] = MCRT_KEY_MISS;
+                const size_t so = half_out + pos;
+                a.st0[so] = make_float4(from.x, from.y, from.z, ray_len(intensity, tb.mat(2 * media).y, a));
+                a.st1[so] = make_float4(dir.x, dir.y, dir.z, __int_as_float(media));
+                a.st2[so] = make_float4(__int_as_float(__double2loint(dist_mm)), __int_as_float(__double2hiint(dist_mm)), __int_as_float(outside), intensity);
+            }
+        }
+        if (!more) break;
+        base = next;
     }
     if (STATS) {
         long long x = wave_sum_i64((long long)st_seg), y = wave_sum_i64((long long)st_hits);
@@ -134,8 +138,11 @@
 }
 
 template <bool STATS>
-__global__ void __launch_bounds__(256, MCRT_SHADE_WAVES) k_shade(FrameArgs a, uint32_t b) { shade_bounce<STATS, false>(a, b); }
-__global__ void __launch_bounds__(256, MCRT_SHADE_WAVES) k_shade_fold(FrameArgs a) { shade_bounce<false, true>(a, 0u); }
+__global__ void __launch_bounds__(256, MCRT_SHADE_WAVES) k_shade(FrameArgs a, uint32_t b) { shade_bounce<STATS, false, !STATS>(a, b); }
+__global__ void __launch_bounds__(256, MCRT_SHADE_WAVES) k_shade_chunk(FrameArgs a, uint32_t b) { shade_bounce<false, false, false>(a, b); }
+__global__ void __launch_bounds__(256, MCRT_SHADE_WAVES) k_shade_fold(FrameArgs a) { shade_bounce<false, true, false>(a, 0u); }
+
+uint32_t shade_waves() { return MCRT_SHADE_WAVES; }
 
 hipError_t launch_init(const FrameArgs &a, hipStream_t st)
 {
@@ -146,11 +153,12 @@
 
 hipError_t launch_shade(const FrameArgs &a, uint32_t b, bool stats, hipStream_t st)
 {
-    const uint32_t np = a.ne * a.S;
-    const dim3 grid((np + 255u) / 256u), blk(256);
+    const uint32_t np = a.ne * a.S, full = (np + 255u) / 256u;
+    const dim3 grid(full), blk(256);
     if (stats) hipLaunchKernelGGL((k_shade<true>), grid, blk, 0, st, a, b);
     else if (a.fold_b0 && b == 0u) hipLaunchKernelGGL(k_shade_fold, grid, blk, 0, st, a);
-    else hipLaunchKernelGGL((k_shade<false>), grid, blk, 0, st, a, b);
+    else if (a.shade_blocks != 0u) hipLaunchKernelGGL((k_shade<false>), dim3(a.shade_blocks < full ? a.shade_blocks : full), blk, 0, st, a, b);
+    else hipLaunchKernelGGL(k_shade_chunk, grid, blk, 0, st, a, b);
     return hipGetLastError();
 }
 
diff --git a/mcray-tracing_amd/csrc/mcrt_trace.cpp b/mcray-tracing_amd/csrc/mcrt_trace.cpp
--- a/mcray-tracing_amd/csrc/mcrt_trace.cpp
+++ b/mcray-tracing_amd/csrc/mcrt_trace.cpp
@@ -129,7 +129,7 @@
     a.el_pos = pose_pos ? pose_pos : c->d_pos; a.el_dir = pose_pos ? pose_dir : c->d_dir; a.pose_stride = pose_pos ? c->p.n_elements : 0u;
     a.row_thr = c->tab.d_row_thr;
     a.acc = c->acc.d_acc; a.flags = c->acc.d_flags; a.acc_stride = acc_ne;
-    a.tri_slot = c->scene.d_tri_slot; a.tris_id = c->scene.d_tris_id; a.mtab = c->tab.d_mtab;
+    a.tri_slot = c->scene.d_tri_slot; a.tris_id = c->scene.d_tris_id; a.mtab = c->tab.d_mtab; a.ptab = c->tab.d_ptab;
     a.stats = c->ins.d_stats; a.error_flag = c->d_error; a.stamps = c->ins.d_stats + 8;
     a.n_mat = c->scene.n_mat; a.n_mesh = c->scene.n_mesh; a.n_nodes = c->scene.bvh4.n_nodes; a.S = c->p.n_samples; a.B = c->p.max_depth; a.R = c->p.n_rows;
     a.ksplit_limit = c->knobs.ksplit_limit;
@@ -167,13 +167,15 @@
     a.fold_b0 = image_only && c->knobs.fold_b0 && !P.latency && accumulate && c->tex_finite && c->scene.start_silent && c->p.n_samples % 256u == 0u ? 1u : 0u;
 }
 
-static void fill_group(const mcrt_ctx *c, const Work &w, mcrt::FrameArgs &a, uint32_t n_frames, uint32_t b0, uint32_t b1, uint32_t acc_e0, int out)
+static void fill_group(mcrt_ctx *c, const Work &w, mcrt::FrameArgs &a, uint32_t n_frames, uint32_t b0, uint32_t b1, uint32_t acc_e0, int out)
 {
     a.stack_ovf = w.stack_ovf; a.segs = w.segs; a.hits = out >= 1 ? (int32_t *)w.hits : nullptr;
     a.st0 = w.b.st0; a.st1 = w.b.st1; a.st2 = w.b.st2; a.queue = w.b.q; a.key0 = w.b.key0; a.key1 = w.b.key1;
     a.counts = w.b.counts; a.cursors = w.b.cursors; a.mrec = w.b.mrec; a.seg_count = w.b.seg_count;
     a.acc_off = b0 - acc_e0;
     a.e_begin = b0; a.ne_frame = b1 - b0; a.ne = (b1 - b0) * n_frames;
+    a.shade_blocks = !c->knobs.shade_persist ? 0u : c->knobs.shade_blocks ? c->knobs.shade_blocks : c->n_cu * mcrt::shade_waves();
+    c->ins.last_shade_blocks = a.shade_blocks;
     a.packet_mask = (c->ins.stats_on || (uint64_t)a.ne * a.S < c->knobs.packet_from) ? 0u : c->knobs.packet_mask;
 }
 
```
